# C-H-Chien/Trifocal_Pose_Estimation_using_Improved_GPUHC

Hardware: AMD Instinct MI355X
Metric: HC paths/sec (312 tracks x RANSAC samples) (higher is better)
Workload: dtype f32

## Files before the change

### trifocal_pose_estimation_using_improved_gpuhc_amd/_abi.py

```python
from __future__ import annotations

import ctypes as C
import os
from collections import namedtuple

import numpy as np

PKG_DIR = os.path.dirname(os.path.abspath(__file__))
LIB_PATH = os.environ.get("HC_TRIFOCAL_LIB") or os.path.join(PKG_DIR, "lib", "libhc_trifocal.so")

ABI_VERSION = 2

NUM_VARS, NUM_PARAMS, NUM_TRACKS = 30, 33, 312
NPP = NUM_PARAMS + 1
UNIFIED_INDEX_SIZE = 38880

HC_STATUS = {0: "HC_SUCCESS", 1: "HC_ERROR_INVALID_VALUE", 2: "HC_ERROR_WORKSPACE", 3: "HC_ERROR_LAUNCH",
             4: "HC_ERROR_DEVICE", 5: "HC_ERROR_TABLE"}


class HCError(RuntimeError):
    pass


# ... 138 lines not shown
                       "HC_THREEVIEW_NONE": HC_THREEVIEW_NONE, "HC_THREEVIEW_TOO_FEW": HC_THREEVIEW_TOO_FEW,
                       "HC_THREEVIEW_SINGULAR": HC_THREEVIEW_SINGULAR, "HC_THREEVIEW_SKIPPED": HC_THREEVIEW_SKIPPED}


class hcThreeViewReport(C.Structure):
    _fields_ = [("status", C.c_int32), ("iterations_run", C.c_int32), ("best_iteration", C.c_int32),
                ("transfer_history", C.c_int32 * (HC_REFINE_MAX_ITERATIONS + 1)),
                ("joint_history", C.c_int32 * (HC_REFINE_MAX_ITERATIONS + 1)),
                ("fit_set", C.c_int32), ("transfer_inliers", C.c_int32),
                ("scale_in", C.c_float), ("scale_out", C.c_float), ("pad", C.c_int32),
                ("rms_px_in", C.c_double * 2), ("rms_px_out", C.c_double * 2)]


class hcRefineThreeViewSettings(C.Structure):
    _fields_ = [("head", hcRefineSettings), ("scale_reports", C.c_void_p), ("reports", C.c_void_p),
                ("transfer_mask", C.c_void_p), ("iterations3", C.c_int32), ("pad", C.c_int32)]


THREEVIEW_REPORT_BYTES = C.sizeof(hcThreeViewReport)

HC_REFINE_STRUCTURE = 0x53543344
HC_STRUCTURE_ONLY = 1
HC_EDGEL3D_TANGENT, HC_EDGEL3D_ORIENTED = 1, 2
HC_STRUCTURE_NONE = 1
STRUCTURE_CONSTANTS = {"HC_REFINE_STRUCTURE": HC_REFINE_STRUCTURE, "HC_STRUCTURE_ONLY": HC_STRUCTURE_ONLY,
                       "HC_EDGEL3D_TANGENT": HC_EDGEL3D_TANGENT, "HC_EDGEL3D_ORIENTED": HC_EDGEL3D_ORIENTED,
                       "HC_STRUCTURE_NONE": HC_STRUCTURE_NONE}


class hcEdgel3D(C.Structure):
    _fields_ = [("X", C.c_float * 3), ("T", C.c_float * 3), ("err3_px", C.c_float), ("sin_plane", C.c_float),
                ("sin3", C.c_float), ("edgel", C.c_int32), ("flags", C.c_int32), ("pad", C.c_int32)]


class hcStructureReport(C.Structure):
    _fields_ = [("status", C.c_int32), ("count", C.c_int32), ("tangents", C.c_int32), ("oriented", C.c_int32),
                ("scale31", C.c_float), ("pad", C.c_int32 * 3)]


class hcRefineStructureSettings(C.Structure):
    _fields_ = [("tv", hcRefineThreeViewSettings), ("tangents", C.c_void_p), ("edgel_offsets", C.c_void_p),
                ("edgels3d", C.c_void_p), ("reports", C.c_void_p), ("min_sin_plane", C.c_float),
                ("max_sin3", C.c_float)]


EDGEL3D_BYTES = C.sizeof(hcEdgel3D)
STRUCTURE_REPORT_BYTES = C.sizeof(hcStructureReport)
EDGEL3D_DTYPE = np.dtype([("X", "<f4", (3,)), ("T", "<f4", (3,)), ("err3_px", "<f4"), ("sin_plane", "<f4"),
                          ("sin3", "<f4"), ("edgel", "<i4"), ("flags", "<i4"), ("pad", "<i4")])
assert EDGEL3D_DTYPE.itemsize == EDGEL3D_BYTES


Sig = namedtuple("Sig", "name restype argtypes optional", defaults=(False,))

_i, _u, _z, _p, _s, _ST = C.c_int, C.c_uint, C.c_size_t, C.c_void_p, C.c_char_p, C.c_int
_TA = C.POINTER(hcTrackArgs)
_GA = C.POINTER(hcGroupedAbortArgs)
_WS = (_p, _z, _p)
_SUPPORT = (_i, _p, _p, _i, _p, _p, _i, _p, _p, _p)

SIGNATURES = (
    Sig("hc_trifocal_workspace_size", _z, ()),
    Sig("hc_trifocal_workspace_size_for", _z, (_i,)),
    Sig("hc_trifocal_workspace_size_for_steps", _z, (_i, _i)),
    Sig("hc_trifocal_2op1p_30x30_track", _ST, (_TA, *_WS)),
    Sig("hc_trifocal_2op1p_30x30_track_abort", _ST, (_TA, C.POINTER(hcAbortArgs), *_WS)),
    Sig("hc_trifocal_2op1p_30x30_track_abort_grouped", _ST, (_TA, _GA, *_WS), True),
    Sig("hc_trifocal_2op1p_30x30_track_abort_gated", _ST, (_TA, _GA, C.POINTER(hcJointGate), *_WS), True),
    Sig("hc_shared_flag_create", _ST, (C.POINTER(_p), C.POINTER(hcIpcHandle)), True),
    Sig("hc_shared_flag_memory_kind", _i, (_p,), True),
    Sig("hc_shared_flag_open", _ST, (C.POINTER(hcIpcHandle), C.POINTER(_p)), True),
    Sig("hc_shared_flag_reset", _ST, (_p, _p), True),
    Sig("hc_shared_flag_close", _ST, (_p, _i), True),
    Sig("hc_trifocal_2op1p_30x30_track_ph_codeopt", _ST, (_TA, *_WS)),
    Sig("hc_trifocal_2op1p_30x30_track_ph", _ST, (_TA, *_WS)),
    Sig("hc_trifocal_workspace_status", _ST, (_p,)),
    Sig("hc_trifocal_read_timings", _ST, (_p, C.POINTER(C.c_double))),
    Sig("hc_trifocal_read_timestamps", _ST, (_p, C.POINTER(C.c_uint64), C.POINTER(C.c_uint64),
                                             C.POINTER(C.c_double))),
    Sig("hc_cgesv_30x30_batched", _ST, (_i, _p, _p, _p, _p)),
    Sig("hc_trifocal_eval_batched", _ST, (_i, _p, _p, _p, _p, _p, _p, _p, *_WS)),
    Sig("hc_last_error_string", _s, ()),
    Sig("hc_trifocal_version", _s, ()),
    Sig("hc_trifocal_abi_version", _i, ()),
    Sig("hc_trifocal_set_ring_test", None, (_i,)),
    Sig("hc_trifocal_set_small_launch", None, (_i,), True),
    Sig("hc_trifocal_set_retry_reuse", None, (_i,), True),
    Sig("hc_trifocal_ring_check_test", _ST, (_p, _z, _u, _u, _u, _p), True),
    Sig("hc_lu_struct_pattern", _u, (_i,), True),
    Sig("hc_lu_group_class", _i, (_i, _i), True),
    Sig("hc_lu_candidates", _u, (_i,), True),
    Sig("hc_lu_search_span", _i, (_i,), True),
    Sig("hc_trifocal_pose_support", _ST, _SUPPORT),
    Sig("hc_trifocal_pose_support_grouped", _ST, _SUPPORT, True),
    Sig("hc_pose_merge", None, (_i, _p, _p, _i, C.POINTER(hcPoseSelection))),
    Sig("hc_trifocal_pose_support_joint", _ST, _SUPPORT),
    Sig("hc_trifocal_pose_support_joint_grouped", _ST, _SUPPORT),
    Sig("hc_trifocal_pose_inlier_mask", _ST, (_p, _i, _p, _p, _p, _p)),
    Sig("hc_pose_merge_joint", None, (_i, _p, _p, C.POINTER(hcTrifocalSelection))),
    Sig("hc_pose_residuals", _i, (_p,) * 7),
    Sig("hc_read_start_sols", _i, (_s, _p)),
    Sig("hc_read_start_params", _i, (_s, _p)),
    Sig("hc_read_int_table", _i, (_s, _p, _i)),
    Sig("hc_read_float_table", _i, (_s, _p, _i)),
    Sig("hc_count_triplet_edgels", _i, (_s,)),
    Sig("hc_read_triplet_edgels", _i, (_s, _p, _p, _i)),
    Sig("hc_split_samples", None, (_i, _i, _p)),
    Sig("hc_prepare_target_params", None, (_u, _i, _p, _p, _p, _i, _p, _p, _p, _p)),
    Sig("hc_count_solutions", None, (_i, _p, _p, _p, _p)),
    Sig("hc_write_converged_sols", _i, (_s, _i, _p, _p)),
    Sig("hc_add_pixel_noise", None, (_i, _p, _p, C.c_double, C.c_uint64, _p)),
    Sig("hc_write_triplet_edgels", _i, (_s, _i, _p, _p)),
)
DECLARED_SYMBOLS = tuple(s.name for s in SIGNATURES)

P2C_SIGNATURES = (
    Sig("hc_trifocal_2op1p_30x30_track_p2c", _ST, (_TA, C.POINTER(hcP2cArgs), *_WS), True),
    Sig("hc_trifocal_p2c_eval_batched", _ST, (_i, _p, _p, _p, _p, _p, _p, _p, _p, _p, *_WS), True),
    Sig("hc_p2c_coefficients", _ST, (_i, _p, _p, _p, _p, _p), True),
)
P2C_DECLARED_SYMBOLS = tuple(s.name for s in P2C_SIGNATURES)

_RS = C.POINTER(hcRefineSettings)
REFINE_SIGNATURES = (
    Sig("hc_trifocal_pose_refine", _ST, (_p, _i, _p, _p, _RS, _p, _p, _p), True),
    Sig("hc_trifocal_pose_refine_grouped", _ST, (_i, _p, _p, _RS, _p, _p, _p), True),
)
REFINE_DECLARED_SYMBOLS = tuple(s.name for s in REFINE_SIGNATURES)

HC_TOPK_MAX = 32
TOPK_SIGNATURES = (
    Sig("hc_trifocal_pose_topk_joint", _ST, (_i, _p, _p, _i, _p, _p), True),
    Sig("hc_trifocal_pose_topk_joint_grouped", _ST, (_i, _p, _p, _i, _p, _i, _p, _p), True),
    Sig("hc_trifocal_pose_refine_topk", _ST, (_i, _p, _i, _p, _p, _RS, _p, _p, _p, _p, _p), True),
    Sig("hc_trifocal_pose_refine_topk_grouped", _ST, (_i, _p, _i, _p, _RS, _p, _p, _p, _p, _p), True),
    Sig("hc_pose_merge_topk", None, (_i, _i, _p, _p, _p), True),
)
TOPK_DECLARED_SYMBOLS = tuple(s.name for s in TOPK_SIGNATURES)

LU_SIGNATURES = (
    Sig("hc_lu_step_level", _i, (_i,), True),
    Sig("hc_cgesv_30x30_struct_batched", _ST, (_i, _p, _p, _p, _p), True),
    Sig("hc_cgesv_30x30_variant_batched", _ST, (_i, _i, _p, _p, _p, _p), True),
)
LU_VARIANTS = ("throughput", "throughput_twin", "abort", "abort_twin", "small", "small_twin", "archived",
               "archived_twin")
LU_DECLARED_SYMBOLS = tuple(s.name for s in LU_SIGNATURES)

LU_ROWTABLE_SIGNATURES = (
    Sig("hc_lu_row_field", _i, (_i, _i, _i), True),
)
LU_ROW_FIELDS = ("member", "bound", "window", "partner", "place", "chain")

EVAL_SIGNATURES = (
    Sig("hc_trifocal_eval_variant_batched", _ST, (_i, _u, _i, _p, _p, _p, _p, _p, _p, _p, _p, _p, _p, *_WS), True),
)
EVAL_VARIANTS = ("packed", "abs")
HC_EVAL_REDO = 1
EVAL_DECLARED_SYMBOLS = tuple(s.name for s in EVAL_SIGNATURES)

ADAPTIVE_SIGNATURES = (
    Sig("hc_ransac_need_table", _ST, (_i, C.c_double, _i, _i, _p), True),
)
ADAPTIVE_DECLARED_SYMBOLS = tuple(s.name for s in ADAPTIVE_SIGNATURES)

_lib = None


def lib() -> C.CDLL:
    global _lib
    if _lib is None:
        if not os.path.exists(LIB_PATH):
            raise HCError(f"native library missing: {LIB_PATH} (run `python -c 'import __graft_entry__ as g; g.build()'`)")
        import torch
        L = C.CDLL(LIB_PATH)
        for s in SIGNATURES + P2C_SIGNATURES + REFINE_SIGNATURES + TOPK_SIGNATURES + LU_SIGNATURES + \
                LU_ROWTABLE_SIGNATURES + EVAL_SIGNATURES + ADAPTIVE_SIGNATURES:
            fn = getattr(L, s.name, None)
            if fn is None:
                if s.optional:
                    continue
                raise HCError(f"{LIB_PATH} does not export {s.name}")
            fn.restype, fn.argtypes = s.restype, list(s.argtypes)
        if L.hc_trifocal_abi_version() != ABI_VERSION:
            raise HCError(f"{LIB_PATH}: ABI {L.hc_trifocal_abi_version()}, this binding expects {ABI_VERSION}")
        _lib = L
    return _lib


def check(status: int, what: str) -> None:
    if status != 0:
        detail = lib().hc_last_error_string().decode(errors="replace")
        raise HCError(f"{what} failed: {HC_STATUS.get(status, status)} ({detail})")


def call(name: str, *args) -> None:
    fn = getattr(lib(), name, None)
    if fn is None:
        raise HCError(f"{LIB_PATH} does not export {name}")
    check(fn(*args), name)


def ptr(x):
    if x is None:
        return C.c_void_p()
    if hasattr(x, "data_ptr"):
        return C.c_void_p(x.data_ptr())
    if hasattr(x, "cuda_stream"):
        return C.c_void_p(x.cuda_stream)
    return x.ctypes.data_as(C.c_void_p)


def _fatbin_digest(path: str) -> str | None:
    import hashlib
    import struct
    with open(path, "rb") as fh:
        elf = fh.read()
    if elf[:4] != b"\x7fELF" or elf[4] != 2:
        return None
    shoff, = struct.unpack_from("<Q", elf, 0x28)
    shentsize, shnum, shstrndx = struct.unpack_from("<HHH", elf, 0x3A)
    def sec(i):
        name, _typ, _flags, _addr, off, size = struct.unpack_from("<IIQQQQ", elf, shoff + i * shentsize)
        return name, off, size
    _, stroff, _ = sec(shstrndx)
    for i in range(shnum):
        name, off, size = sec(i)
        end = elf.index(b"\0", stroff + name)
        if elf[stroff + name:end] == b".hip_fatbin":
            return hashlib.sha256(elf[off:off + size]).hexdigest()
    return None


def build_id(path: str | None = None) -> str:
    import re
    path = path or LIB_PATH
    with open(path, "rb") as fh:
        m = re.search(rb"hc_trifocal gfx950 (v[0-9.]+)", fh.read())
    ver = m.group(1).decode() if m else "v?"
    d = _fatbin_digest(path)
    return f"{ver}+{d[:12] if d else 'nofatbin'}"


PRODUCT_LIB_PATH = os.path.join(PKG_DIR, "lib", "libhc_trifocal.so")
```

### trifocal_pose_estimation_using_improved_gpuhc_amd/csrc/hc_components.hpp

```cpp
#pragma once

#include "hc_layout.hpp"

namespace hc {


__global__ void __launch_bounds__(WG_THREADS) k_cgesv(int n, const cf *__restrict__ A, const cf *__restrict__ B,
                                                      cf *__restrict__ X) {
    __shared__ LUBuf s_lu[2 * WAVES_PER_WG];
    __shared__ __attribute__((aligned(16))) cf s_scr[2 * WAVES_PER_WG][LU_SCRATCH_CF];
    const int lane = lane_id();
    const int r = lane & 31;
    const int sys = (blockIdx.x * WAVES_PER_WG + threadIdx.x / WAVE) * 2 + (lane >> 5);
    const bool ok = sys < n && r < NV;
    cf rA[NV];
    uint32_t pat = 0;
#pragma unroll
    for (int c = 0; c < NV; c++) {
        rA[c] = ok ? A[((size_t)sys * NV + r) * NV + c] : cmk(0.0f, 0.0f);
        if (rA[c].x != 0.0f || rA[c].y != 0.0f) pat |= 1u << c;
    }
    const cf rB = ok ? B[(size_t)sys * NV + r] : cmk(0.0f, 0.0f);
    LUBuf &LB = s_lu[(threadIdx.x / WAVE) * 2 + (lane >> 5)];
    cf *scr = s_scr[(threadIdx.x / WAVE) * 2 + (lane >> 5)];
    bool redo;
    cf x = lu_solve<false>(rA, rB, lane, pat, LB, scr, redo, __ballot(sys < n));
    if (__builtin_expect(redo, 0)) {
#pragma unroll
        for (int c = 0; c < NV; c++) rA[c] = ok ? A[((size_t)sys * NV + r) * NV + c] : cmk(0.0f, 0.0f);
        x = lu_solve<true>(rA, rB, lane, pat, LB, scr, redo);
    }
    if (ok) X[(size_t)sys * NV + r] = x;
}

__global__ void __launch_bounds__(WG_THREADS) k_cgesv_struct_check(int n, const cf *__restrict__ A,
                                                                   unsigned *__restrict__ bad) {
    const size_t i = (size_t)blockIdx.x * WG_THREADS + threadIdx.x;
    if (i >= (size_t)n * NV) return;
    const uint32_t pat = LU_STRUCT_PAT[i % NV];
    bool out = false;
    for (int c = 0; c < NV; c++) {
        const cf a = A[i * NV + c];
        if (!((pat >> c) & 1u) && (a.x != 0.0f || a.y != 0.0f)) out = true;
    }
    if (out) *bad = 1u;
}
template <int LAT, bool STRUCT, bool ENTCHK, bool FUSE>
__global__ void __launch_bounds__(WG_THREADS) k_cgesv_variant(int n, const cf *__restrict__ A,
                                                              const cf *__restrict__ B, cf *__restrict__ X) {
    __shared__ LUBuf s_lu[2 * WAVES_PER_WG];
    __shared__ __attribute__((aligned(16))) cf s_scr[2 * WAVES_PER_WG][FUSE ? LU_SCRATCH_FUSED_CF : LU_SCRATCH_CF];
    if constexpr (FUSE) {
        lu_rowtab_fill(threadIdx.x);
        __syncthreads();
    }
    const int lane = lane_id();
    const int r = lane & 31;
    const int sys = (blockIdx.x * WAVES_PER_WG + threadIdx.x / WAVE) * 2 + (lane >> 5);
    const bool ok = sys < n && r < NV;
    cf rA[NV];
    uint32_t nz = 0;
    pf2 sq = {0.0f, 0.0f};
#pragma unroll
    for (int c = 0; c < NV; c++) {
        rA[c] = ok ? A[((size_t)sys * NV + r) * NV + c] : cmk(0.0f, 0.0f);
        if constexpr (!STRUCT) {
            if (rA[c].x != 0.0f || rA[c].y != 0.0f) nz |= 1u << c;
        }
        if constexpr (ENTCHK) {
            sq.x = __builtin_fmaf(rA[c].x, rA[c].x, sq.x);
            sq.y = __builtin_fmaf(rA[c].y, rA[c].y, sq.y);
        }
    }
    bool ent_bad = false;
    if constexpr (ENTCHK) ent_bad = __ballot(!(sq.x + sq.y < __builtin_inff())) != 0ull;
    const uint32_t pat = STRUCT ? (r < NV ? LU_STRUCT_PAT[r] : 0u) : nz;
    const cf rB = ok ? B[(size_t)sys * NV + r] : cmk(0.0f, 0.0f);
    LUBuf &LB = s_lu[(threadIdx.x / WAVE) * 2 + (lane >> 5)];
    cf *scr = s_scr[(threadIdx.x / WAVE) * 2 + (lane >> 5)];
    bool redo;
    cf x = lu_solve<false, LAT, STRUCT, ENTCHK, FUSE>(rA, rB, lane, pat, LB, scr, redo, __ballot(sys < n), ent_bad);
    if (__builtin_expect(redo, 0)) {
#pragma unroll
        for (int c = 0; c < NV; c++) rA[c] = ok ? A[((size_t)sys * NV + r) * NV + c] : cmk(0.0f, 0.0f);
        x = lu_solve<true>(rA, rB, lane, pat, LB, scr, redo);
    }
    if (ok) X[(size_t)sys * NV + r] = x;
}


__global__ void __launch_bounds__(WG_THREADS) k_eval(int n, const Workspace *ws, const cf *__restrict__ X,
                                                     const cf *__restrict__ P, const cf *__restrict__ D,
                                                     cf *__restrict__ HX, cf *__restrict__ HT, cf *__restrict__ H) {
    __shared__ uint32_t s_hx[HX_SLOT_CAP * 32];
    __shared__ uint2 s_ht[HT_TERMS * 32];
    __shared__ uint32_t s_hxd[HX_NSLOT / 2 * 32];
    __shared__ SlotLDS s_slot[2 * WAVES_PER_WG];
    const EvalTables *T = &ws->tab;
    if (ws->status != 0u) return;
    for (int i = threadIdx.x; i < HX_SLOT_CAP * 32; i += WG_THREADS) s_hx[i] = T->hx[i];
    for (int i = threadIdx.x; i < HT_TERMS * 32; i += WG_THREADS) s_ht[i] = T->ht[i];
    for (int i = threadIdx.x; i < HX_NSLOT / 2 * 32; i += WG_THREADS) s_hxd[i] = (&T->hxd[0][0])[i];
    {
        float *z = reinterpret_cast<float *>(s_slot);
        for (int i = threadIdx.x; i < (int)(sizeof(s_slot) / 4); i += WG_THREADS) z[i] = 0.0f;
    }
    __syncthreads();
    const int lane = lane_id();
    const int r = lane & 31;
    const int sys = (blockIdx.x * WAVES_PER_WG + threadIdx.x / WAVE) * 2 + (lane >> 5);
    SlotLDS &S = s_slot[(threadIdx.x / WAVE) * 2 + (lane >> 5)];
    const bool ok = sys < n;
    if (ok && r < 31) S.x[r] = X[(size_t)sys * 31 + r];
    if (ok) {
        S.ent[r] = P[(size_t)sys * NPP + r];
        S.ent[NPP + r] = D[(size_t)sys * NPP + r];
        if (r < NPP - 32) {
            S.ent[r + 32] = P[(size_t)sys * NPP + r + 32];
            S.ent[NPP + r + 32] = D[(size_t)sys * NPP + r + 32];
        }
    }
    __shared__ uint32_t s_gm[GM_WORDS][32];
    if (threadIdx.x < 32)
        for (int q = 0; q < GM_WORDS; q++) s_gm[q][threadIdx.x] = T->gm[q][threadIdx.x];
    __syncthreads();
    build_prefix_rounds(S, r, &T->pre[0][0]);
    cf rA[NV];
    eval_hx(rA, s_hx, s_hxd, &s_gm[0][0], S, r);
    const cf ht = eval_rhs<RHS_HT>(s_ht, S, r, true, rhs_masks(T));
    const cf h = eval_rhs<RHS_H>(s_ht, S, r, false, rhs_masks(T));
    if (ok && r < NV) {
#pragma unroll
        for (int c = 0; c < NV; c++) HX[((size_t)sys * NV + r) * NV + c] = rA[c];
        HT[(size_t)sys * NV + r] = ht;
        H[(size_t)sys * NV + r] = h;
    }
}

template <bool ABSTAB>
__global__ void __launch_bounds__(WG_THREADS) k_eval_variant(int n, int redo_vals, const Workspace *ws,
                                                             const cf *__restrict__ X, const cf *__restrict__ TGT,
                                                             const cf *__restrict__ DIF, const cf *__restrict__ SP,
                                                             const float *__restrict__ T0,
                                                             const uint8_t *__restrict__ KIND, cf *__restrict__ HX,
                                                             cf *__restrict__ RHS, uint8_t *__restrict__ ENT_OK) {
    __shared__ cf s_sp[NPP];
    __shared__ SlotLDS s_slot[2 * WAVES_PER_WG];
    const EvalTables *T = &ws->tab;
    if (ws->status != 0u) return;
    const uint2 *s_ht = T->ht;
    const uint32_t *s_hx = T->hx;
    const uint32_t *s_hxd = &T->hxd[0][0];
    if (threadIdx.x < NPP) s_sp[threadIdx.x] = SP[threadIdx.x];
    {
        float *z = reinterpret_cast<float *>(s_slot);
        for (int i = threadIdx.x; i < (int)(sizeof(s_slot) / 4); i += WG_THREADS) z[i] = 0.0f;
    }
    __syncthreads();
    const int lane = lane_id();
    const int r = lane & 31, hb = lane & 32;
    const int wid = threadIdx.x / WAVE;
    SlotLDS &S = s_slot[wid * 2 + (hb >> 5)];
    if (r == 30) S.x[30] = cmk(1.0f, 0.0f);
    __shared__ uint32_t s_rowc[GM_WORDS + 1][32];
    if (threadIdx.x < 32) {
        for (int q = 0; q < GM_WORDS; q++) s_rowc[q][threadIdx.x] = T->gm[q][threadIdx.x];
        s_rowc[GM_WORDS][threadIdx.x] = T->pat[threadIdx.x];
    }
    __syncthreads();
    const bool rl = r < NV;
    wave_lds_sync();
    const AbsTables *AT = &ws->abs;
    const int wv = ABSTAB ? __builtin_amdgcn_readfirstlane(wid) : 0;
    char *const l0 = reinterpret_cast<char *>(s_slot);

    const int pt = (blockIdx.x * WAVES_PER_WG + wid) * 2 + (hb >> 5);
    const size_t pi = (size_t)(pt < n ? pt : n - 1);
    const unsigned kd = KIND[pi];
    const bool act = pt < n && kd < 2u;
    const bool pred = act && kd == 0u;
    if (act && rl) S.x[r] = X[pi * (NV + 1) + r];
    build_prefixes(S, r, &T->pre[0][0], TGT + pi * NPP, DIF + pi * NPP, s_sp, T0[pi]);
    wave_lds_sync();
    const int lane_v = lane_fresh();
    const int r_v = lane_v & 31;
    const uint32_t l16 = (uint32_t)lane_v << 4;
    cf rB = cmk(0.0f, 0.0f);
    {
        const bool any_p = __ballot(pred) != 0ull, any_c = __ballot(act && !pred) != 0ull;
        const RhsMasks mk = rhs_masks(T);
        if (any_p && any_c) {
            if constexpr (ABSTAB) rB = eval_rhs_abs<RHS_MIXED>(AT->ht[wv], AT->htq[wv], l0, l16, pred, mk);
            else rB = eval_rhs<RHS_MIXED>(s_ht, S, r_v, pred, mk);
        } else if (any_p) {
            const cf t = ABSTAB ? eval_rhs_abs<RHS_HT>(AT->ht[wv], AT->htq[wv], l0, l16, true, mk)
                                : eval_rhs<RHS_HT>(s_ht, S, r_v, true, mk);
            if (pred) rB = t;
        } else if (any_c) {
            const cf t = ABSTAB ? eval_rhs_abs<RHS_H>(AT->ht[wv], AT->htq[wv], l0, l16, false, mk)
                                : eval_rhs<RHS_H>(s_ht, S, r_v, false, mk);
            if (!pred) rB = t;
        }
    }
    cf rA[NV];
    if constexpr (ABSTAB) {
        uint4 gmv[ABS_GM_Q];
        const bool ent_ok = eval_hx_terms_abs(AT->hx[wv], l0, l16, AT->gm[wv], gmv);
        if (act) ENT_OK[pi * 32 + r] = ent_ok ? 1 : 0;
        wave_lds_sync();
        gather_hx_abs(rA, l0, gmv);
    } else {
        eval_hx(rA, s_hx, s_hxd, &s_rowc[0][0], S, r_v);
    }
    wave_lds_sync();
    if (redo_vals) {
        for (int k = r; k < ENT_CAP - 1; k += 32) S.ent[k] = cmk(__builtin_nanf(""), __builtin_nanf(""));
        wave_lds_sync();
        const bool act_r = act, pred_r = pred;
        const int l_r = lane_fresh(), r_r = l_r & 31;
        const uint32_t l16_r = (uint32_t)l_r << 4;
        cf rb = cmk(0.0f, 0.0f);
        if (__ballot(pred_r) != 0ull) {
            const cf t = ABSTAB ? eval_rhs_abs<RHS_HT>(AT->ht[wv], AT->htq[wv], l0, l16_r, true, rhs_masks(T))
                                : eval_rhs<RHS_HT>(s_ht, S, r_r, true, rhs_masks(T));
            if (pred_r) rb = t;
        }
        if (__ballot(act_r && !pred_r) != 0ull) {
            const cf t = ABSTAB ? eval_rhs_abs<RHS_H>(AT->ht[wv], AT->htq[wv], l0, l16_r, false, rhs_masks(T))
                                : eval_rhs<RHS_H>(s_ht, S, r_r, false, rhs_masks(T));
            if (!pred_r) rb = t;
        }
        if constexpr (ABSTAB) {
            uint4 gmv[ABS_GM_Q];
            eval_hx_terms_abs(AT->hx[wv], l0, l16_r, AT->gm[wv], gmv);
            wave_lds_sync();
            gather_hx_abs(rA, l0, gmv);
        } else {
            eval_hx_terms(s_hx, s_hxd, reinterpret_cast<char *>(&S), r_r);
            wave_lds_sync();
            gather_hx(rA, &s_rowc[0][0], S, r_r);
        }
        wave_lds_sync();
        rB = rb;
    }
    if (act && rl) {
#pragma unroll
        for (int c = 0; c < NV; c++) HX[(pi * NV + r) * NV + c] = rA[c];
        RHS[pi * NV + r] = rB;
    }
}

}
```

### trifocal_pose_estimation_using_improved_gpuhc_amd/csrc/hc_eval.hpp

```cpp
#pragma once

#include <stddef.h>

#include "hc_slot.hpp"

namespace hc {

typedef float pf2 __attribute__((ext_vector_type(2)));

constexpr int HX_GCAP[6] = {8, 5, 3, 3, 1, 1};
constexpr int HX_SLOT_CAP = 21;
constexpr int HX_NSLOT = 6;
__host__ __device__ constexpr int hx_gend(int s) { return s < 0 ? 0 : hx_gend(s - 1) + HX_GCAP[s]; }
__host__ __device__ constexpr bool hx_is_gend(int k) {
    return k + 1 == hx_gend(0) || k + 1 == hx_gend(1) || k + 1 == hx_gend(2) || k + 1 == hx_gend(3) ||
           k + 1 == hx_gend(4) || k + 1 == hx_gend(5);
}
__host__ __device__ constexpr int hx_gslot(int k) {
    return k < hx_gend(0) ? 0 : k < hx_gend(1) ? 1 : k < hx_gend(2) ? 2 : k < hx_gend(3) ? 3 : k < hx_gend(4) ? 4 : 5;
}
static_assert(hx_gend(5) == HX_SLOT_CAP, "slot capacities");
constexpr int SLOT_OFF_X = (int)offsetof(SlotLDS, x);
constexpr int SLOT_OFF_ENT = (int)offsetof(SlotLDS, ent);
constexpr int SLOT_OFF_ENTZERO = SLOT_OFF_ENT + 8 * (ENT_CAP - 1);
constexpr int SLOT_OFF_STG = SLOT_OFF_ENT;
constexpr int SLOT_STG_DIF_DELTA = 8 * NPP;
constexpr int SLOT_OFF_TP = (int)offsetof(SlotLDS, tp);
constexpr int SLOT_OFF_QP = (int)offsetof(SlotLDS, qp);
constexpr int SLOT_OFF_HXDUMMY = (int)offsetof(SlotLDS, lu) + 8 * 31;
static_assert(SLOT_OFF_QP + 8 * QP_CAP < 65536 && SLOT_OFF_HXDUMMY < 65536, "slot offsets must fit 16 bits");
static_assert(SLOT_OFF_X + 8 * 31 < 256, "x offsets must fit a byte");
static_assert(2 * NPP <= ENT_CAP - 1, "the staging area lies below the structural zero");

constexpr int GM_WORDS = NV / 2;
constexpr int PRE_TP_ROUNDS = (TP_CAP + 31) / 32, PRE_ROUNDS = PRE_TP_ROUNDS + (QP_CAP + 31) / 32;
__device__ __forceinline__ float coef_b2(uint32_t w) {
    float co;
    asm("v_cvt_f32_i32_sdwa %0, sext(%1) dst_sel:DWORD dst_unused:UNUSED_PAD src0_sel:BYTE_2" : "=v"(co) : "v"(w));
    return co;
}
__device__ __forceinline__ float coef_ht(const uint2 &w) { return (float)((int)w.y >> 24); }
struct EvalTables {
    int hx_len;
    int status;
    unsigned magic;
    unsigned lu_struct;
    unsigned long long src_hash;
    unsigned long long pad2;
    uint32_t gm[GM_WORDS][32];
    uint32_t pat[32];
    uint32_t hxd[HX_NSLOT / 2][32];
    uint32_t ht_acc_mask[4];
    uint32_t ht_light_mask[4];
    uint2 pre[PRE_ROUNDS][32];
    uint32_t hx[HX_SLOT_CAP * 32];
    uint2 ht[HT_TERMS * 32];
};

__device__ __forceinline__ pf2 ldp(const char *base, uint32_t off) {
    return *reinterpret_cast<const pf2 *>(base + off);
}
__device__ __forceinline__ pf2 pcmul(pf2 a, pf2 b) {
    pf2 t, r;
    asm("v_pk_mul_f32 %0, %1, %2 op_sel:[1,1] op_sel_hi:[1,0] neg_lo:[1,0]" : "=v"(t) : "v"(a), "v"(b));
    asm("v_pk_fma_f32 %0, %1, %2, %3 op_sel_hi:[0,1,1]" : "=v"(r) : "v"(a), "v"(b), "v"(t));
    return r;
}
__device__ __forceinline__ pf2 pcmadd(pf2 acc, pf2 a, pf2 b) {
    pf2 s, r;
    asm("v_pk_fma_f32 %0, %1, %2, %3 op_sel_hi:[0,1,1]" : "=v"(s) : "v"(a), "v"(b), "v"(acc));
    asm("v_pk_fma_f32 %0, %1, %2, %3 op_sel:[1,1,0] op_sel_hi:[1,0,1] neg_lo:[1,0,0]" : "=v"(r) : "v"(a), "v"(b), "v"(s));
    return r;
}
__device__ __forceinline__ pf2 pcmsub(pf2 acc, pf2 a, pf2 b) {
    pf2 s, r;
    asm("v_pk_fma_f32 %0, %1, %2, %3 op_sel_hi:[0,1,1] neg_lo:[1,0,0] neg_hi:[1,0,0]" : "=v"(s) : "v"(a), "v"(b), "v"(acc));
    asm("v_pk_fma_f32 %0, %1, %2, %3 op_sel:[1,1,0] op_sel_hi:[1,0,1] neg_hi:[1,0,0]" : "=v"(r) : "v"(a), "v"(b), "v"(s));
    return r;
}

#ifndef HC_EV_AHEAD
#define HC_EV_AHEAD 2
#endif
constexpr int EV_AHEAD = HC_EV_AHEAD;
constexpr int EV_WAHEAD = EV_AHEAD + 2;

struct HxOps { pf2 t, xu, xv; };
__device__ __forceinline__ HxOps hx_ops(const char *sb, uint32_t w) {
    return HxOps{ldp(sb, w & 0xFFFFu), ldp(sb, (w >> 16) & 0xFFu), ldp(sb, w >> 24)};
}

__device__ __forceinline__ void eval_hx_terms(const uint32_t *s_hx, const uint32_t *s_hxd, char *sb, int r) {
    uint32_t w[HX_SLOT_CAP];
    uint32_t dst[HX_NSLOT / 2];
#pragma unroll
    for (int q = 0; q < HX_NSLOT / 2; q++) dst[q] = s_hxd[q * 32 + r];
#pragma unroll
    for (int k = 0; k < EV_WAHEAD; k++) w[k] = s_hx[k * 32 + r];
    HxOps o[EV_AHEAD + 1];
#pragma unroll
    for (int k = 0; k < EV_AHEAD; k++) o[k] = hx_ops(sb, w[k]);
    pf2 acc = {0.0f, 0.0f};
#pragma unroll
    for (int k = 0; k < HX_SLOT_CAP; k++) {
        if (k + EV_WAHEAD < HX_SLOT_CAP) w[k + EV_WAHEAD] = s_hx[(k + EV_WAHEAD) * 32 + r];
        if (k + EV_AHEAD < HX_SLOT_CAP) o[(k + EV_AHEAD) % (EV_AHEAD + 1)] = hx_ops(sb, w[k + EV_AHEAD]);
        const HxOps &q = o[k % (EV_AHEAD + 1)];
        const pf2 P = pcmul(q.t, q.xu);
        acc = pcmadd(acc, P, q.xv);
        if (hx_is_gend(k)) {
            const int sl = hx_gslot(k);
            const uint32_t off = (sl & 1) ? (dst[sl >> 1] >> 16) : (dst[sl >> 1] & 0xFFFFu);
            *reinterpret_cast<pf2 *>(sb + off) = acc;
            acc = pf2{0.0f, 0.0f};
        }
        __builtin_amdgcn_sched_barrier(0);
    }
}

__device__ __forceinline__ void gather_hx(cf (&rA)[NV], const uint32_t *gmw, const SlotLDS &S, int r) {
    const char *sb = reinterpret_cast<const char *>(&S);
    uint32_t g[GM_WORDS];
#pragma unroll
    for (int q = 0; q < GM_WORDS; q++) g[q] = gmw[q * 32 + r];
#pragma unroll
    for (int c = 0; c < NV; c++) {
        const pf2 v = ldp(sb, (c & 1) ? (g[c / 2] >> 16) : (g[c / 2] & 0xFFFFu));
        rA[c] = cmk(v.x, v.y);
    }
}

__device__ __forceinline__ void eval_hx(cf (&rA)[NV], const uint32_t *s_hx, const uint32_t *s_hxd,
                                        const uint32_t *gmw, SlotLDS &S, int r) {
    eval_hx_terms(s_hx, s_hxd, reinterpret_cast<char *>(&S), r);
    wave_lds_sync();
    HC_ISA_MARK("ev_gather");
    gather_hx(rA, gmw, S, r);
}

__device__ __forceinline__ void build_prefix_rounds(SlotLDS &S, int r, const uint2 *pre) {
    char *sb = reinterpret_cast<char *>(&S);
    wave_lds_sync();
#pragma unroll
    for (int k = 0; k < PRE_TP_ROUNDS; k++) {
        const uint2 w = pre[k * 32 + r];
        const pf2 pa = ldp(sb, w.x & 0xFFFFu), pb = ldp(sb, w.x >> 16);
        const float co = coef_b2(w.y);
        const pf2 t = pcmul(pa * pf2{co, co}, pb);
        *reinterpret_cast<pf2 *>(sb + (w.y & 0xFFFFu)) = t;
    }
#pragma unroll
    for (int k = PRE_TP_ROUNDS; k < PRE_ROUNDS; k++) {
        const uint2 w = pre[k * 32 + r];
        const uint32_t oa = w.x & 0xFFFFu, ob = w.x >> 16;
        const pf2 pa = ldp(sb, oa), pb = ldp(sb, ob);
        const pf2 da = ldp(sb + SLOT_STG_DIF_DELTA, oa), db = ldp(sb + SLOT_STG_DIF_DELTA, ob);
        const pf2 q = pcmadd(pcmul(da, pb), db, pa);
// ... 6 lines not shown
    cf *stg = S.ent;
    const float omt = (float)(1.0 - (double)t0);
    stg[r] = cadd(cscale(target[r], t0), cscale(sp[r], omt));
    stg[NPP + r] = diff[r];
    if (r == 0) {
        stg[32] = cadd(cscale(target[32], t0), cscale(sp[32], omt));
        stg[33] = cmk(1.0f, 0.0f);
        stg[NPP + 32] = diff[32];
        stg[NPP + 33] = diff[33];
    }
    build_prefix_rounds(S, r, pre);
}

constexpr int P2C_NK = 38;
constexpr int SLOT_STG_P2C_HT_DELTA = 8 * P2C_NK;
static_assert(2 * P2C_NK <= ENT_CAP - 1, "the P2C staging area lies below the structural zero");
__device__ __forceinline__ void p2c_stage(SlotLDS &S, int r, const cf *chx, const cf *cht, float t) {
    cf *stg = S.ent;
#pragma unroll
    for (int q = 0; q < 2; q++) {
        const int k = r + 32 * q;
        if (k < P2C_NK) {
            stg[k] = cadd(cadd(chx[3 * k], cscale(chx[3 * k + 1], t)), cscale(cscale(chx[3 * k + 2], t), t));
            stg[P2C_NK + k] = cadd(cht[2 * k], cscale(cht[2 * k + 1], t));
        }
    }
}
__device__ __forceinline__ void build_prefix_rounds_p2c(SlotLDS &S, int r, const uint2 *pre) {
    char *sb = reinterpret_cast<char *>(&S);
    wave_lds_sync();
#pragma unroll
    for (int k = 0; k < PRE_TP_ROUNDS; k++) {
        const uint2 w = pre[k * 32 + r];
        const pf2 c = ldp(sb, w.x & 0xFFFFu);
        const float co = coef_b2(w.y);
        *reinterpret_cast<pf2 *>(sb + (w.y & 0xFFFFu)) = c * pf2{co, co};
    }
#pragma unroll
    for (int k = PRE_TP_ROUNDS; k < PRE_ROUNDS; k++) {
        const uint2 w = pre[k * 32 + r];
        *reinterpret_cast<pf2 *>(sb + (w.y & 0xFFFFu)) = ldp(sb + SLOT_STG_P2C_HT_DELTA, w.x & 0xFFFFu);
    }
    wave_lds_sync();
}
__device__ __forceinline__ void build_prefixes_p2c(SlotLDS &S, int r, const uint2 *pre, const cf *chx, const cf *cht,
                                                   float t0) {
    p2c_stage(S, r, chx, cht, t0);
    build_prefix_rounds_p2c(S, r, pre);
}

enum : int { RHS_HT = 0, RHS_H = 1, RHS_MIXED = 2 };
constexpr int HT_FULL = 13, HT_HELP = HT_TERMS - HT_FULL;
constexpr int HT_HELP_FIRST = HT_FULL - HT_HELP;

template <bool SUB>
__device__ __forceinline__ pf2 pcmacc_masked(pf2 acc, pf2 a, pf2 b, unsigned long long m) {
    pf2 t;
    unsigned long long sv;
    if constexpr (SUB)
        asm("s_mov_b64 %2, exec\n\ts_mov_b64 exec, %3\n\t"
            "v_pk_fma_f32 %1, %4, %5, %0 op_sel_hi:[0,1,1] neg_lo:[1,0,0] neg_hi:[1,0,0]\n\t"
            "s_nop 0\n\t"
            "v_pk_fma_f32 %0, %4, %5, %1 op_sel:[1,1,0] op_sel_hi:[1,0,1] neg_hi:[1,0,0]\n\t"
            "s_mov_b64 exec, %2"
            : "+v"(acc), "=&v"(t), "=&s"(sv) : "s"(m), "v"(a), "v"(b));
    else
        asm("s_mov_b64 %2, exec\n\ts_mov_b64 exec, %3\n\t"
            "v_pk_fma_f32 %1, %4, %5, %0 op_sel_hi:[0,1,1]\n\t"
            "s_nop 0\n\t"
            "v_pk_fma_f32 %0, %4, %5, %1 op_sel:[1,1,0] op_sel_hi:[1,0,1] neg_lo:[1,0,0]\n\t"
            "s_mov_b64 exec, %2"
            : "+v"(acc), "=&v"(t), "=&s"(sv) : "s"(m), "v"(a), "v"(b));
    return acc;
}
__device__ __forceinline__ pf2 from_partner(pf2 v) {
    asm("v_permlane16_swap_b32 %0, %0\n\tv_permlane16_swap_b32 %1, %1" : "+v"(v.x), "+v"(v.y));
    return v;
}
struct RhsMasks { unsigned long long acc[HT_HELP], light[HT_HELP]; };

__device__ __forceinline__ RhsMasks rhs_masks(const EvalTables *T) {
    RhsMasks m;
#pragma unroll
    for (int q = 0; q < HT_HELP; q++) {
        const unsigned long long a = (uint32_t)__builtin_amdgcn_readfirstlane((int)T->ht_acc_mask[q]),
                                 l = (uint32_t)__builtin_amdgcn_readfirstlane((int)T->ht_light_mask[q]);
        m.acc[q] = a | (a << 32);
        m.light[q] = l | (l << 32);
    }
    return m;
}

template <int KIND>
struct RhsOps { pf2 t, q, xu, xv, xw; };
template <int KIND>
__device__ __forceinline__ RhsOps<KIND> rhs_ops(const char *sb, const uint2 &w) {
    RhsOps<KIND> o;
    if constexpr (KIND != RHS_HT) o.t = ldp(sb, w.x & 0xFFFFu);
    if constexpr (KIND != RHS_H) o.q = ldp(sb, w.x >> 16);
    o.xu = ldp(sb, w.y & 0xFFu);
    o.xv = ldp(sb, (w.y >> 8) & 0xFFu);
    o.xw = ldp(sb, (w.y >> 16) & 0xFFu);
    return o;
}

template <int KIND>
__device__ __forceinline__ cf eval_rhs(const uint2 *s_ht, const SlotLDS &S, int r, bool ht_half, const RhsMasks &mk) {
    const char *sb = reinterpret_cast<const char *>(&S);
    constexpr bool SUB = KIND == RHS_HT;
    uint2 w[HT_TERMS];
#pragma unroll
    for (int j = 0; j < EV_WAHEAD; j++) w[j] = s_ht[j * 32 + r];
    RhsOps<KIND> o[EV_AHEAD + 1];
#pragma unroll
    for (int j = 0; j < EV_AHEAD; j++) o[j] = rhs_ops<KIND>(sb, w[j]);
    pf2 acc = {0.0f, 0.0f};
    pf2 hp[HT_HELP];
#pragma unroll
    for (int j = 0; j < HT_FULL; j++) {
        if (j + EV_WAHEAD < HT_TERMS) w[j + EV_WAHEAD] = s_ht[(j + EV_WAHEAD) * 32 + r];
        if (j + EV_AHEAD < HT_FULL) o[(j + EV_AHEAD) % (EV_AHEAD + 1)] = rhs_ops<KIND>(sb, w[j + EV_AHEAD]);
        const RhsOps<KIND> &q = o[j % (EV_AHEAD + 1)];
        const float co = coef_ht(w[j]);
        pf2 P;
        if constexpr (KIND == RHS_HT) {
            const pf2 s = q.q * pf2{co, co};
            P = pcmul(pcmul(s, q.xu), q.xv);
        } else if constexpr (KIND == RHS_H) {
            P = pcmul(pcmul(q.t, q.xu), q.xv);
        } else {
            const pf2 s = q.q * pf2{-co, -co};
            const pf2 pre = {ht_half ? s.x : q.t.x, ht_half ? s.y : q.t.y};
            P = pcmul(pcmul(pre, q.xu), q.xv);
        }
        if (j < HT_HELP_FIRST) {
            acc = SUB ? pcmsub(acc, P, q.xw) : pcmadd(acc, P, q.xw);
        } else {
            hp[j - HT_HELP_FIRST] = P;
            acc = pcmacc_masked<SUB>(acc, P, q.xw, mk.acc[j - HT_HELP_FIRST]);
        }
        __builtin_amdgcn_sched_barrier(0);
    }
#pragma unroll
    for (int q = 0; q < HT_HELP; q++) {
        const pf2 P = from_partner(hp[q]);
        const pf2 xw = ldp(sb, (w[HT_FULL + q].y >> 16) & 0xFFu);
        acc = pcmacc_masked<SUB>(acc, P, xw, mk.light[q]);
    }
    return cmk(acc.x, acc.y);
}

constexpr int ABS_WAVES = 4;
constexpr int ABS_GM_Q = (NV + 3) / 4;
static_assert(HT_HELP <= 3, "the light terms' x[w] share one word group");
struct AbsTables {
    uint4 hx[ABS_WAVES][HX_SLOT_CAP][WAVE];
    uint4 ht[ABS_WAVES][HT_FULL + 1][WAVE];
    uint2 htq[ABS_WAVES][HT_FULL][WAVE];
    uint4 gm[ABS_WAVES][ABS_GM_Q][WAVE];
};
static_assert(2 * ABS_WAVES * sizeof(SlotLDS) < 65536, "absolute offsets stay in the DS offset range");
constexpr int EV_TAHEAD = 6;
static_assert(EV_TAHEAD > EV_AHEAD, "the words come before the operands they address");

template <typename W>
__device__ __forceinline__ W abs_ld(const W *row, uint32_t lane_off) {
    return *reinterpret_cast<const W *>(reinterpret_cast<const char *>(row) + (size_t)lane_off);
}

__device__ __forceinline__ HxOps hx_ops_abs(const char *l0, const uint4 &w) {
    return HxOps{ldp(l0, w.x), ldp(l0, w.y), ldp(l0, w.z)};
}
__device__ __forceinline__ bool eval_hx_terms_abs(const uint4 (*hxw)[WAVE], char *l0, uint32_t l16,
                                                  const uint4 (*gmw)[WAVE], uint4 (&g)[ABS_GM_Q]) {
    uint4 w[HX_SLOT_CAP];
#pragma unroll
    for (int k = 0; k < EV_TAHEAD; k++) w[k] = abs_ld(hxw[k], l16);
    HxOps o[EV_AHEAD + 1];
#pragma unroll
    for (int k = 0; k < EV_AHEAD; k++) o[k] = hx_ops_abs(l0, w[k]);
    pf2 acc = {0.0f, 0.0f}, sq = {0.0f, 0.0f};
#pragma unroll
    for (int k = 0; k < HX_SLOT_CAP; k++) {
        if (k + EV_TAHEAD < HX_SLOT_CAP) w[k + EV_TAHEAD] = abs_ld(hxw[k + EV_TAHEAD], l16);
        if (k == HX_SLOT_CAP - EV_TAHEAD) {
#pragma unroll
            for (int q = 0; q < ABS_GM_Q; q++) g[q] = abs_ld(gmw[q], l16);
        }
        if (k + EV_AHEAD < HX_SLOT_CAP) o[(k + EV_AHEAD) % (EV_AHEAD + 1)] = hx_ops_abs(l0, w[k + EV_AHEAD]);
        const HxOps &q = o[k % (EV_AHEAD + 1)];
        const pf2 P = pcmul(q.t, q.xu);
        acc = pcmadd(acc, P, q.xv);
        if (hx_is_gend(k)) {
            *reinterpret_cast<pf2 *>(l0 + w[k].w) = acc;
            asm("v_pk_fma_f32 %0, %1, %1, %0" : "+v"(sq) : "v"(acc));
            acc = pf2{0.0f, 0.0f};
        }
        __builtin_amdgcn_sched_barrier(0);
    }
    return sq.x + sq.y < __builtin_inff();
}

__device__ __forceinline__ void gather_hx_abs(cf (&rA)[NV], const char *l0, const uint4 (&g)[ABS_GM_Q]) {
#pragma unroll
    for (int c = 0; c < NV; c++) {
        const uint4 &gw = g[c / 4];
        const pf2 v = ldp(l0, c % 4 == 0 ? gw.x : c % 4 == 1 ? gw.y : c % 4 == 2 ? gw.z : gw.w);
        rA[c] = cmk(v.x, v.y);
    }
}

template <int KIND>
__device__ __forceinline__ RhsOps<KIND> rhs_ops_abs(const char *l0, const uint4 &w, const uint2 &wq) {
    RhsOps<KIND> o;
    if constexpr (KIND != RHS_HT) o.t = ldp(l0, w.w);
    if constexpr (KIND != RHS_H) o.q = ldp(l0, wq.x);
    o.xu = ldp(l0, w.x);
    o.xv = ldp(l0, w.y);
    o.xw = ldp(l0, w.z);
    return o;
}

template <int KIND>
__device__ __forceinline__ cf eval_rhs_abs(const uint4 (*htw)[WAVE], const uint2 (*htqw)[WAVE], const char *l0,
                                           uint32_t l16, bool ht_half, const RhsMasks &mk) {
    constexpr bool SUB = KIND == RHS_HT;
    constexpr bool Q = KIND != RHS_H;
    const uint32_t l8 = l16 >> 1;
    uint4 w[HT_FULL + 1];
    uint2 wq[HT_FULL];
#pragma unroll
    for (int j = 0; j < EV_TAHEAD; j++) {
        w[j] = abs_ld(htw[j], l16);
        if constexpr (Q) wq[j] = abs_ld(htqw[j], l8);
    }
    RhsOps<KIND> o[EV_AHEAD + 1];
#pragma unroll
    for (int j = 0; j < EV_AHEAD; j++) o[j] = rhs_ops_abs<KIND>(l0, w[j], wq[j]);
    pf2 acc = {0.0f, 0.0f};
    pf2 hp[HT_HELP];
#pragma unroll
    for (int j = 0; j < HT_FULL; j++) {
        if (j + EV_TAHEAD < HT_FULL + 1) w[j + EV_TAHEAD] = abs_ld(htw[j + EV_TAHEAD], l16);
        if constexpr (Q)
            if (j + EV_TAHEAD < HT_FULL) wq[j + EV_TAHEAD] = abs_ld(htqw[j + EV_TAHEAD], l8);
        if (j + EV_AHEAD < HT_FULL)
            o[(j + EV_AHEAD) % (EV_AHEAD + 1)] = rhs_ops_abs<KIND>(l0, w[j + EV_AHEAD], wq[j + EV_AHEAD]);
        const RhsOps<KIND> &q = o[j % (EV_AHEAD + 1)];
        pf2 P;
        if constexpr (KIND == RHS_HT) {
            const float co = __uint_as_float(wq[j].y);
            const pf2 s = q.q * pf2{co, co};
            P = pcmul(pcmul(s, q.xu), q.xv);
        } else if constexpr (KIND == RHS_H) {
            P = pcmul(pcmul(q.t, q.xu), q.xv);
        } else {
            const float co = __uint_as_float(wq[j].y);
            const pf2 s = q.q * pf2{-co, -co};
            const pf2 pre = {ht_half ? s.x : q.t.x, ht_half ? s.y : q.t.y};
            P = pcmul(pcmul(pre, q.xu), q.xv);
        }
        if (j < HT_HELP_FIRST) {
            acc = SUB ? pcmsub(acc, P, q.xw) : pcmadd(acc, P, q.xw);
        } else {
            hp[j - HT_HELP_FIRST] = P;
            acc = pcmacc_masked<SUB>(acc, P, q.xw, mk.acc[j - HT_HELP_FIRST]);
        }
        __builtin_amdgcn_sched_barrier(0);
    }
#pragma unroll
    for (int q = 0; q < HT_HELP; q++) {
        const pf2 P = from_partner(hp[q]);
        const uint4 &lw = w[HT_FULL];
        const pf2 xw = ldp(l0, q == 0 ? lw.x : q == 1 ? lw.y : lw.z);
        acc = pcmacc_masked<SUB>(acc, P, xw, mk.light[q]);
    }
    return cmk(acc.x, acc.y);
}

}
```

### trifocal_pose_estimation_using_improved_gpuhc_amd/csrc/hc_kernels.hip

```cpp
#include "hc_layout.hpp"
#include "hc_prep.hpp"
#include "hc_components.hpp"
#include "hc_ring.hpp"
#include "hc_score.hpp"
#include "hc_track.hpp"
#include "hc_p2c.hpp"
#include "../../include/hc_trifocal_testing.h"
#include "../../include/p2c/hc_trifocal_p2c.h"
#include "../../include/lu/hc_lu_testing.h"
#include "../../include/lu/hc_lu_rowtable_testing.h"
#include "../../include/eval/hc_eval_testing.h"
#include "../../include/adaptive/hc_trifocal_adaptive.h"

#include <atomic>
#include <climits>
#include <cstdlib>
#include <cstring>
#include <map>
#include <mutex>
#include <utility>

namespace hc {

thread_local hipError_t g_last_hip_error = hipSuccess;
static inline hcStatus launch_status(hcStatus on_fail) {
    const hipError_t e = hipGetLastError();
    if (e != hipSuccess) { g_last_hip_error = e; return on_fail; }
    return HC_SUCCESS;
}

static size_t ws_bytes_needed() { return (sizeof(Workspace) + 255) & ~(size_t)255; }
struct SliceLayout {
    size_t rq, ring, susp;
    size_t total;
    unsigned long long ring_cap;
    size_t susp_entry0, susp_entry1;
};
static SliceLayout slice_layout(long long paths, int max_steps) {
    if (paths < 0) paths = 0;
    if (max_steps < 0) max_steps = 0;
    SliceLayout a;
    a.ring_cap = ring_entries(paths, max_steps);
    const size_t ring_bytes = ((size_t)a.ring_cap * sizeof(unsigned long long) + 255) & ~(size_t)255;
    a.rq = ws_bytes_needed();
    a.ring = a.rq + RQ_WORDS * sizeof(unsigned);
    a.susp = a.ring + ring_bytes;
    a.total = a.susp + (size_t)paths * SUSP_WORDS * sizeof(unsigned long long);
    a.susp_entry0 = ring_bytes / 8;
    a.susp_entry1 = a.susp_entry0 + (size_t)paths * SUSP_WORDS;
    return a;
}
static bool sliced_launch(bool abort_mode, const hcTrackSettings &st, const SliceLayout &a, size_t wsb) {
    return !abort_mode && SLICE_Q > 0 && wsb >= a.total && a.ring_cap < 0xFFFFFF00ull &&
           a.susp_entry1 < (size_t)UINT_MAX && slice_fits(st.max_steps, st.max_corrections, st.delta_t_inc_steps);
}
static std::atomic<int> g_ring_test{0};
static std::atomic<int> g_small_launch{0};
static std::atomic<int> g_retry_reuse{1};

static int grid_for(int waves_needed, const void *kernel) {
    static std::mutex mu;
    static std::map<std::pair<int, const void *>, std::pair<int, int>> cache;
    int dev = 0;
    if (hipGetDevice(&dev) != hipSuccess) return -1;
    int cus = 0, per_cu = 0;
    {
        std::lock_guard<std::mutex> g(mu);
        auto it = cache.find({dev, kernel});
        if (it == cache.end()) {
            if (hipDeviceGetAttribute(&cus, hipDeviceAttributeMultiprocessorCount, dev) != hipSuccess) return -1;
            if (hipOccupancyMaxActiveBlocksPerMultiprocessor(&per_cu, kernel, WG_THREADS, 0) != hipSuccess) per_cu = 1;
            if (per_cu < 1) per_cu = 1;
            it = cache.emplace(std::make_pair(dev, kernel), std::make_pair(cus, per_cu)).first;
        }
        cus = it->second.first;
        per_cu = it->second.second;
    }
    const int want = waves_needed / WAVES_PER_WG + (waves_needed % WAVES_PER_WG != 0);
    const int cap = cus * per_cu;
    return want < cap ? want : cap;
}
static int resident_wgs(const void *kernel) { return grid_for(INT_MAX, kernel); }

enum class TrackMode { GatedAbort, GroupedAbort, Abort, Ph, PhCodeopt, Track, P2c };
struct TrackLaunch {
    TrackMode mode;
    const hcAbortArgs *ab = nullptr;
    const hcGroupedAbortArgs *gr = nullptr;
    const hcJointGate *jg = nullptr;
    const hcP2cArgs *p2c = nullptr;
};

struct TrackKernels { const void *lus, *any; };
static TrackKernels track_kernels(TrackMode mode, bool small, bool adaptive = false) {
    static const void *const by_mode[2][6] = {
        {(const void *)k_track_gated<true>, (const void *)k_track_grouped<true>,
         (const void *)k_track<true, HC_ABORT_MINW, true>, (const void *)k_track<false, 5, true, true>,
         (const void *)k_track<false, 5, true, true>, (const void *)k_track<false, 5, true>},
        {(const void *)k_track_gated<false>, (const void *)k_track_grouped<false>,
         (const void *)k_track<true, HC_ABORT_MINW, true, false, false>,
         (const void *)k_track<false, 5, true, true, false>, (const void *)k_track<false, 5, true, true, false>,
         (const void *)k_track<false, 5, true, false, false>}};
    if (small) return {(const void *)k_track_small<true>, (const void *)k_track_small<false>};
    if (mode == TrackMode::P2c) return {(const void *)k_track_p2c<true>, (const void *)k_track_p2c<false>};
    if (mode == TrackMode::GatedAbort && adaptive)
        return {(const void *)k_track_adaptive<true>, (const void *)k_track_adaptive<false>};
    return {by_mode[0][(int)mode], by_mode[1][(int)mode]};
}

static bool small_launch(TrackMode mode, long long paths) {
    const int small_mode = g_small_launch.load(std::memory_order_relaxed);
    if (mode != TrackMode::Track || small_mode < 0) return false;
    const long long slots = 2ll * WAVES_PER_WG * resident_wgs(track_kernels(mode, false).lus);
    const long long small_slots = 2ll * WAVES_PER_WG * resident_wgs(track_kernels(mode, true).lus);
    return small_mode > 0 || (slots > 0 && 2 * paths <= slots && paths <= small_slots);
}

static hcStatus enqueue_track(const void *kern, int grid, KArgs &k, hipStream_t s) {
    void *kargs[] = {&k};
    g_last_hip_error = hipLaunchKernel(kern, dim3(grid), dim3(WG_THREADS), kargs, 0, s);
    if (g_last_hip_error != hipSuccess) return HC_ERROR_LAUNCH;
    return launch_status(HC_ERROR_LAUNCH);
}

static hcStatus launch_track(const hcTrackArgs *t, const TrackLaunch &l, void *workspace, size_t wsb,
                             hcStream stream) {
    const bool gated = l.mode == TrackMode::GatedAbort;
    const bool grouped = gated || l.mode == TrackMode::GroupedAbort;
    const bool abort_mode = grouped || l.mode == TrackMode::Abort;
    const hcAbortArgs *ab = l.mode == TrackMode::Abort ? l.ab : nullptr;
    const hcGroupedAbortArgs *gr = grouped ? l.gr : nullptr;
    const hcP2cArgs *pc = l.mode == TrackMode::P2c ? l.p2c : nullptr;
    const hcAdaptiveGate *ag =
        gated && l.jg->pad == (int32_t)HC_GATE_ADAPTIVE ? reinterpret_cast<const hcAdaptiveGate *>(l.jg) : nullptr;
    if (!t || t->sub_ransac_iters < 0) return HC_ERROR_INVALID_VALUE;
    if (grouped && (gr->num_groups < 1 || !gr->groups || !gr->sample_group || !gr->group_found ||
                    !gr->trifocal_sols_batch_index))
        return HC_ERROR_INVALID_VALUE;
    if (ag && (!ag->need || !ag->need_offset || !ag->sample_ordinal || !ag->group_limit)) return HC_ERROR_INVALID_VALUE;
    if (!workspace || wsb < ws_bytes_needed()) return HC_ERROR_WORKSPACE;
    if (t->sub_ransac_iters == 0) return HC_SUCCESS;
    if ((!t->start_sols && !t->start_sols_array) || (!t->tracks && !t->track_array) || !t->converge || !t->infinity)
        return HC_ERROR_INVALID_VALUE;
    if (!pc && (!t->start_params || !t->target_params || !t->diff_params || !t->unified_index))
        return HC_ERROR_INVALID_VALUE;
    if (t->settings.max_steps < 0 || t->settings.max_corrections < 0 || t->settings.delta_t_inc_steps < 0)
        return HC_ERROR_INVALID_VALUE;
    if (l.mode == TrackMode::Abort && (!ab || ab->num_triplet_edgels <= 0 || !ab->triplet_edge_locations ||
                                       !ab->intrinsic_matrix || !ab->found_trifocal_sols ||
                                       !ab->trifocal_sols_batch_index))
        return HC_ERROR_INVALID_VALUE;
    const long long paths = (long long)t->sub_ransac_iters * NTRK;
    if (paths > 0x7FFFFFFFll) return HC_ERROR_INVALID_VALUE;
    hipStream_t s = (hipStream_t)stream;
    Workspace *ws = (Workspace *)workspace;
    (void)hipGetLastError();
    KArgs k{};
    k.num_paths = (int)paths;
    k.ordered = abort_mode ? 0 : 1;
    k.truncate = (l.mode == TrackMode::PhCodeopt || l.mode == TrackMode::Ph || pc) ? 0 : 1;
    k.explicit_rk = (l.mode == TrackMode::Ph || pc) ? 1 : 0;
    k.max_steps = t->settings.max_steps;
    k.max_corr = t->settings.max_corrections;
// ... 124 lines not shown
int hc_diag_phases(unsigned long long *out, int reset) { return hc::diag_read(hc::g_diag_phase, out, reset); }
#endif
#ifdef HC_DIAG_LUWORK
int hc_diag_luwork(unsigned long long *out, int reset) { return hc::diag_read(hc::g_diag_luwork, out, reset); }
#endif
#ifdef HC_DIAG_LIVE
int hc_diag_live(unsigned long long *out, int reset) { return hc::diag_read(hc::g_diag_live, out, reset); }
#endif
#ifdef HC_DIAG_TIMES
int hc_diag_span(unsigned long long *out, int reset) {
    static const unsigned long long init[4] = {~0ull, 0ull, 0ull, 0ull};
    return hc::diag_read(hc::g_diag_span, out, reset, &init);
}
#endif
#ifdef HC_DIAG_UTIL
int hc_diag_util(unsigned long long *out, int reset) { return hc::diag_read(hc::g_diag_util, out, reset); }
#endif

size_t hc_trifocal_workspace_size(void) { return hc::ws_bytes_needed(); }

size_t hc_trifocal_workspace_size_for(int sub_ransac_iters) {
    return hc_trifocal_workspace_size_for_steps(sub_ransac_iters, 80);
}

size_t hc_trifocal_workspace_size_for_steps(int sub_ransac_iters, int max_steps) {
    return hc::slice_layout(sub_ransac_iters > 0 ? (long long)sub_ransac_iters * hc::NTRK : 0, max_steps).total;
}

hcStatus hc_trifocal_2op1p_30x30_track(const hcTrackArgs *args, void *workspace, size_t workspace_bytes,
                                       hcStream stream) {
    return hc::launch_track(args, {hc::TrackMode::Track}, workspace, workspace_bytes, stream);
}

hcStatus hc_trifocal_2op1p_30x30_track_abort(const hcTrackArgs *args, const hcAbortArgs *abort_args,
                                             void *workspace, size_t workspace_bytes, hcStream stream) {
    return hc::launch_track(args, {hc::TrackMode::Abort, abort_args}, workspace, workspace_bytes, stream);
}

hcStatus hc_trifocal_2op1p_30x30_track_abort_grouped(const hcTrackArgs *args, const hcGroupedAbortArgs *g,
                                                     void *workspace, size_t workspace_bytes, hcStream stream) {
    if (!g) return HC_ERROR_INVALID_VALUE;
    return hc::launch_track(args, {hc::TrackMode::GroupedAbort, nullptr, g}, workspace, workspace_bytes, stream);
}

hcStatus hc_trifocal_2op1p_30x30_track_abort_gated(const hcTrackArgs *args, const hcGroupedAbortArgs *g,
                                                   const hcJointGate *gate, void *workspace,
                                                   size_t workspace_bytes, hcStream stream) {
    if (!g || !gate) return HC_ERROR_INVALID_VALUE;
    if (!(gate->min_joint_ratio > 0.0f) || gate->min_joint_ratio > 3.402823466e+38f) return HC_ERROR_INVALID_VALUE;
    return hc::launch_track(args, {hc::TrackMode::GatedAbort, nullptr, g, gate}, workspace, workspace_bytes, stream);
}

hcStatus hc_trifocal_2op1p_30x30_track_ph_codeopt(const hcTrackArgs *args, void *workspace, size_t workspace_bytes,
                                                  hcStream stream) {
    return hc::launch_track(args, {hc::TrackMode::PhCodeopt}, workspace, workspace_bytes, stream);
}

hcStatus hc_trifocal_2op1p_30x30_track_ph(const hcTrackArgs *args, void *workspace, size_t workspace_bytes,
                                          hcStream stream) {
    return hc::launch_track(args, {hc::TrackMode::Ph}, workspace, workspace_bytes, stream);
}

hcStatus hc_trifocal_2op1p_30x30_track_p2c(const hcTrackArgs *args, const hcP2cArgs *p2c, void *workspace,
                                           size_t workspace_bytes, hcStream stream) {
    if (!p2c || !p2c->hx_index || !p2c->ht_index || !p2c->coeffs_hx || !p2c->coeffs_ht) return HC_ERROR_INVALID_VALUE;
    hc::TrackLaunch l{hc::TrackMode::P2c};
    l.p2c = p2c;
    return hc::launch_track(args, l, workspace, workspace_bytes, stream);
}

hcStatus hc_trifocal_workspace_status(const void *workspace) {
    if (!workspace) return HC_ERROR_INVALID_VALUE;
    hc::Workspace h;
    const hcStatus st = hc::read_control(workspace, h);
    if (st != HC_SUCCESS) return st;
    if (h.status == 0u) return HC_SUCCESS;
    return h.status == (unsigned)HC_ERROR_TABLE ? HC_ERROR_TABLE : HC_ERROR_DEVICE;
}

hcStatus hc_trifocal_read_timings(const void *workspace, double *first_found_seconds) {
    if (!workspace || !first_found_seconds) return HC_ERROR_INVALID_VALUE;
    hc::Workspace h;
    const hcStatus st = hc::read_control(workspace, h);
    if (st != HC_SUCCESS) return st;
    *first_found_seconds = (h.t_found && h.t_start) ? (double)(long long)(h.t_found - h.t_start) / hc::wall_clock_hz() : -1.0;
    return HC_SUCCESS;
}

hcStatus hc_trifocal_read_timestamps(const void *workspace, uint64_t *start_ticks, uint64_t *found_ticks,
                                     double *tick_hz) {
    if (!workspace || !start_ticks || !found_ticks || !tick_hz) return HC_ERROR_INVALID_VALUE;
    hc::Workspace h;
    const hcStatus st = hc::read_control(workspace, h);
    if (st != HC_SUCCESS) return st;
    *start_ticks = h.t_start;
    *found_ticks = h.t_found;
    *tick_hz = hc::wall_clock_hz();
    return HC_SUCCESS;
}

hcStatus hc_cgesv_30x30_batched(int n, const hcComplex *A, const hcComplex *b, hcComplex *x, hcStream stream) {
    if (n < 0 || (n > 0 && (!A || !b || !x))) return HC_ERROR_INVALID_VALUE;
    if (n == 0) return HC_SUCCESS;
    (void)hipGetLastError();
    const int per = 2 * hc::WAVES_PER_WG;
    hipLaunchKernelGGL(hc::k_cgesv, dim3((n + per - 1) / per), dim3(hc::WG_THREADS), 0, (hipStream_t)stream, n,
                       (const hc::cf *)A, (const hc::cf *)b, (hc::cf *)x);
    return hc::launch_status(HC_ERROR_LAUNCH);
}

hcStatus hc_cgesv_30x30_variant_batched(int variant, int n, const hcComplex *A, const hcComplex *b, hcComplex *x,
                                        hcStream stream) {
    if (variant < 0 || variant >= HC_LU_VARIANT_COUNT) return HC_ERROR_INVALID_VALUE;
    if (n < 0 || (n > 0 && (!A || !b || !x))) return HC_ERROR_INVALID_VALUE;
    if (n == 0) return HC_SUCCESS;
    hipStream_t s = (hipStream_t)stream;
    (void)hipGetLastError();
    switch (variant) {
    case HC_LU_VARIANT_THROUGHPUT:      return hc::launch_cgesv_variant<false, false, 0, true>(n, A, b, x, s);
    case HC_LU_VARIANT_THROUGHPUT_TWIN: return hc::launch_cgesv_variant<false, false, 0, false>(n, A, b, x, s);
    case HC_LU_VARIANT_ABORT:           return hc::launch_cgesv_variant<true, false, HC_LU_LATB_COLS, true>(n, A, b, x, s);
    case HC_LU_VARIANT_ABORT_TWIN:      return hc::launch_cgesv_variant<true, false, HC_LU_LATB_COLS, false>(n, A, b, x, s);
    case HC_LU_VARIANT_SMALL:           return hc::launch_cgesv_variant<false, false, HC_SMALL_LAT, true>(n, A, b, x, s);
    case HC_LU_VARIANT_SMALL_TWIN:      return hc::launch_cgesv_variant<false, false, HC_SMALL_LAT, false>(n, A, b, x, s);
    case HC_LU_VARIANT_ARCHIVED:        return hc::launch_cgesv_variant<false, true, 0, true>(n, A, b, x, s);
    case HC_LU_VARIANT_ARCHIVED_TWIN:   return hc::launch_cgesv_variant<false, true, 0, false>(n, A, b, x, s);
    }
    return HC_ERROR_INVALID_VALUE;
}

hcStatus hc_cgesv_30x30_struct_batched(int n, const hcComplex *A, const hcComplex *b, hcComplex *x, hcStream stream) {
    return hc_cgesv_30x30_variant_batched(HC_LU_VARIANT_THROUGHPUT, n, A, b, x, stream);
}

hcStatus hc_trifocal_eval_batched(int n, const int32_t *unified_index, const hcComplex *x, const hcComplex *p,
                                  const hcComplex *d, hcComplex *Hx, hcComplex *Ht, hcComplex *H, void *workspace,
                                  size_t workspace_bytes, hcStream stream) {
    if (n < 0 || !unified_index || (n > 0 && (!x || !p || !d || !Hx || !Ht || !H))) return HC_ERROR_INVALID_VALUE;
    if (!workspace || workspace_bytes < hc::ws_bytes_needed()) return HC_ERROR_WORKSPACE;
    if (n == 0) return HC_SUCCESS;
    hipStream_t s = (hipStream_t)stream;
    hc::Workspace *ws = (hc::Workspace *)workspace;
    (void)hipGetLastError();
    hc::PrepArgs pa{unified_index, ws, nullptr, nullptr, nullptr, nullptr, 0u, 0u, 0u};
    hipLaunchKernelGGL(hc::k_prep_tables, dim3(1), dim3(hc::PREP_THREADS), 0, s, pa);
    if (hc::launch_status(HC_ERROR_LAUNCH) != HC_SUCCESS) return HC_ERROR_LAUNCH;
    const int per = 2 * hc::WAVES_PER_WG;
    hipLaunchKernelGGL(hc::k_eval, dim3((n + per - 1) / per), dim3(hc::WG_THREADS), 0, s, n, ws,
                       (const hc::cf *)x, (const hc::cf *)p, (const hc::cf *)d, (hc::cf *)Hx, (hc::cf *)Ht,
                       (hc::cf *)H);
    return hc::launch_status(HC_ERROR_LAUNCH);
}

hcStatus hc_trifocal_eval_variant_batched(int variant, unsigned flags, int n, const int32_t *unified_index,
                                          const hcComplex *x, const hcComplex *target, const hcComplex *diff,
                                          const hcComplex *start_params, const float *t, const uint8_t *kind,
                                          hcComplex *Hx, hcComplex *rhs, uint8_t *ent_ok, void *workspace,
                                          size_t workspace_bytes, hcStream stream) {
    if (variant < 0 || variant >= HC_EVAL_VARIANT_COUNT || (flags & ~HC_EVAL_REDO) != 0u) return HC_ERROR_INVALID_VALUE;
    const bool abs_tables = variant == HC_EVAL_VARIANT_ABS;
    if (n < 0 || (n > 0 && (!unified_index || !x || !target || !diff || !start_params || !t || !kind || !Hx || !rhs ||
                            (abs_tables && !ent_ok))))
        return HC_ERROR_INVALID_VALUE;
    if (!workspace || workspace_bytes < hc::ws_bytes_needed()) return HC_ERROR_WORKSPACE;
    if (n == 0) return HC_SUCCESS;
    hipStream_t s = (hipStream_t)stream;
    hc::Workspace *ws = (hc::Workspace *)workspace;
    (void)hipGetLastError();
    hc::PrepArgs pa{unified_index, ws, nullptr, nullptr, nullptr, nullptr, 0u, 0u, 0u};
    hipLaunchKernelGGL(hc::k_prep_tables, dim3(1), dim3(hc::PREP_THREADS), 0, s, pa);
    if (hc::launch_status(HC_ERROR_LAUNCH) != HC_SUCCESS) return HC_ERROR_LAUNCH;
    const int per = 2 * hc::WAVES_PER_WG;
    const dim3 grid((n + per - 1) / per), block(hc::WG_THREADS);
    const int redo = (flags & HC_EVAL_REDO) ? 1 : 0;
    if (abs_tables)
        hipLaunchKernelGGL(hc::k_eval_variant<true>, grid, block, 0, s, n, redo, ws, (const hc::cf *)x,
                           (const hc::cf *)target, (const hc::cf *)diff, (const hc::cf *)start_params, t, kind,
                           (hc::cf *)Hx, (hc::cf *)rhs, ent_ok);
    else
        hipLaunchKernelGGL(hc::k_eval_variant<false>, grid, block, 0, s, n, redo, ws, (const hc::cf *)x,
                           (const hc::cf *)target, (const hc::cf *)diff, (const hc::cf *)start_params, t, kind,
                           (hc::cf *)Hx, (hc::cf *)rhs, ent_ok);
    if (hc::launch_status(HC_ERROR_LAUNCH) != HC_SUCCESS) return HC_ERROR_LAUNCH;
    unsigned ctl[16];
    hipError_t e = hipMemcpyAsync(ctl, workspace, sizeof(ctl), hipMemcpyDeviceToHost, s);
    if (e == hipSuccess) e = hipStreamSynchronize(s);
    if (e != hipSuccess) {
        hc::g_last_hip_error = e;
        return HC_ERROR_DEVICE;
    }
    const unsigned status = ctl[offsetof(hc::Workspace, status) / sizeof(unsigned)];
    if (status == 0u) return HC_SUCCESS;
    return status == (unsigned)HC_ERROR_TABLE ? HC_ERROR_TABLE : HC_ERROR_DEVICE;
}

hcStatus hc_trifocal_p2c_eval_batched(int n, const int32_t *hx_index, const int32_t *ht_index, const hcComplex *x,
                                      const hcComplex *coeffs_hx, const hcComplex *coeffs_ht, const float *t,
                                      hcComplex *Hx, hcComplex *Ht, hcComplex *H, void *workspace,
                                      size_t workspace_bytes, hcStream stream) {
    if (n < 0 || !hx_index || !ht_index || (n > 0 && (!x || !coeffs_hx || !coeffs_ht || !t || !Hx || !Ht || !H)))
        return HC_ERROR_INVALID_VALUE;
    if (!workspace || workspace_bytes < hc::ws_bytes_needed()) return HC_ERROR_WORKSPACE;
    if (n == 0) return HC_SUCCESS;
    hipStream_t s = (hipStream_t)stream;
    hc::Workspace *ws = (hc::Workspace *)workspace;
    (void)hipGetLastError();
    hc::PrepArgs pa{hx_index, ws, nullptr, nullptr, nullptr, nullptr, 0u, 0u, 0u};
    hipLaunchKernelGGL(hc::k_prep_tables_p2c<true>, dim3(1), dim3(hc::PREP_THREADS), 0, s, pa, ht_index);
    if (hc::launch_status(HC_ERROR_LAUNCH) != HC_SUCCESS) return HC_ERROR_LAUNCH;
    const int per = 2 * hc::WAVES_PER_WG;
    hipLaunchKernelGGL(hc::k_eval_p2c<true>, dim3((n + per - 1) / per), dim3(hc::WG_THREADS), 0, s, n, ws,
                       (const hc::cf *)x, (const hc::cf *)coeffs_hx, (const hc::cf *)coeffs_ht, t, (hc::cf *)Hx,
                       (hc::cf *)Ht, (hc::cf *)H);
    return hc::launch_status(HC_ERROR_LAUNCH);
}

const char *hc_last_error_string(void) { return hipGetErrorString(hc::g_last_hip_error); }

static_assert(sizeof(hcIpcHandle) == sizeof(hipIpcMemHandle_t), "hcIpcHandle mirrors hipIpcMemHandle_t");

namespace hc {
static std::mutex g_flag_mu;
static std::map<const void *, int> g_flag_kind;
}

hcStatus hc_shared_flag_create(uint32_t **flag, hcIpcHandle *handle) {
    if (!flag || !handle) return HC_ERROR_INVALID_VALUE;
    static const unsigned kinds[3] = {hipDeviceMallocUncached, hipDeviceMallocFinegrained, hipDeviceMallocDefault};
    hipError_t last = hipSuccess;
    for (int k = 0; k < 3; k++) {
        void *p = nullptr;
        last = (kinds[k] == hipDeviceMallocDefault) ? hipMalloc(&p, 256) : hipExtMallocWithFlags(&p, 256, kinds[k]);
        if (last != hipSuccess) { (void)hipGetLastError(); continue; }
        hipIpcMemHandle_t h;
        if ((last = hipMemset(p, 0, 256)) != hipSuccess || (last = hipDeviceSynchronize()) != hipSuccess ||
            (last = hipIpcGetMemHandle(&h, p)) != hipSuccess) {
            (void)hipGetLastError();
            (void)hipFree(p);
            continue;
        }
        memcpy(handle, &h, sizeof(h));
        *flag = (uint32_t *)p;
        std::lock_guard<std::mutex> g(hc::g_flag_mu);
        hc::g_flag_kind[p] = 2 - k;
        return HC_SUCCESS;
    }
    hc::g_last_hip_error = last;
    return HC_ERROR_DEVICE;
}

int hc_shared_flag_memory_kind(const uint32_t *flag) {
    std::lock_guard<std::mutex> g(hc::g_flag_mu);
    const auto it = hc::g_flag_kind.find(flag);
    return it == hc::g_flag_kind.end() ? -1 : it->second;
}

hcStatus hc_shared_flag_open(const hcIpcHandle *handle, uint32_t **flag) {
    if (!flag || !handle) return HC_ERROR_INVALID_VALUE;
    hipIpcMemHandle_t h;
    memcpy(&h, handle, sizeof(h));
    void *p = nullptr;
    if ((hc::g_last_hip_error = hipIpcOpenMemHandle(&p, h, hipIpcMemLazyEnablePeerAccess)) != hipSuccess)
        return HC_ERROR_DEVICE;
    *flag = (uint32_t *)p;
    return HC_SUCCESS;
}

hcStatus hc_shared_flag_reset(uint32_t *flag, hcStream stream) {
    if (!flag) return HC_ERROR_INVALID_VALUE;
    if ((hc::g_last_hip_error = hipMemsetAsync(flag, 0, sizeof(uint32_t), (hipStream_t)stream)) != hipSuccess)
        return HC_ERROR_LAUNCH;
    return HC_SUCCESS;
}

hcStatus hc_shared_flag_close(uint32_t *flag, int opened) {
    if (!flag) return HC_ERROR_INVALID_VALUE;
    if (!opened) {
        std::lock_guard<std::mutex> g(hc::g_flag_mu);
        hc::g_flag_kind.erase(flag);
    }
    hc::g_last_hip_error = opened ? hipIpcCloseMemHandle(flag) : hipFree(flag);
    return hc::g_last_hip_error == hipSuccess ? HC_SUCCESS : HC_ERROR_DEVICE;
}

int hc_trifocal_abi_version(void) { return HC_TRIFOCAL_ABI_VERSION; }

unsigned hc_lu_struct_pattern(int row) { return row >= 0 && row < hc::NV ? hc::LU_STRUCT_PAT[row] : 0u; }
unsigned hc_lu_candidates(int step) { return step >= 0 && step < hc::NV ? hc::LU_BOUND.cand[step] : 0u; }
int hc_lu_search_span(int step) { return step >= 0 && step < hc::NV ? hc::lu_search_span(step) : -1; }
int hc_lu_step_level(int step) { return step >= 0 && step < hc::NV ? hc::LU_LEVELS.level[step] : -1; }
int hc_lu_group_class(int step, int group) {
    if (step < 0 || step >= hc::NV - 1 || group < 0 || group >= hc::LuChunks::count(step)) return -1;
    return hc::lu_group_class(step, group);
}
int hc_lu_row_field(int level, int row, int field) {
    if (level < 0 || level >= hc::LU_REC_LEVELS || row < 0 || row >= hc::LU_REC_ROWS) return -2;
    hc::LuRowRec rec{0u, hc::LU_ROWTAB.w[level * hc::LU_REC_ROWS + row]};
    rec.bound = hc::LU_ROWTAB.w[hc::LU_REC_BOUND0 + ((rec.word >> hc::LU_REC_MEMBER_AT) & 31u)];
    const int mem = (int)((rec.word >> hc::LU_REC_MEMBER_AT) & 31u), k = (int)((rec.word >> hc::LU_REC_CHAIN_AT) & 15u);
    switch (field) {
    case HC_LU_ROW_MEMBER: return mem == hc::LU_REC_NO_MEMBER ? -1 : mem;
    case HC_LU_ROW_BOUND: return (int)rec.bound;
    case HC_LU_ROW_WINDOW: return (int)(rec.word & ((1u << hc::LU_REC_WIN_BITS) - 1u)) / 8 + 2 * row;
    case HC_LU_ROW_PARTNER: return (int)((rec.word >> hc::LU_REC_PARTNER_AT) & 31u);
    case HC_LU_ROW_PLACE: return (rec.word & hc::LU_REC_FIRST) ? 0 : (rec.word & hc::LU_REC_UP) ? 1 : 2;
    case HC_LU_ROW_CHAIN: return k == hc::LU_REC_NO_CHAIN ? -1 : k;
    default: return -2;
    }
}

hcStatus hc_trifocal_ring_check_test(void *workspace, size_t workspace_bytes, unsigned head, unsigned tail,
                                     unsigned avail, hcStream stream) {
    const hc::SliceLayout area = hc::slice_layout(0, 0);
    if (!workspace || workspace_bytes < area.ring) return HC_ERROR_WORKSPACE;
    hipStream_t s = (hipStream_t)stream;
    unsigned *rq = (unsigned *)((char *)workspace + area.rq);
    const unsigned v[3] = {head, tail, avail};
    const int at[3] = {hc::RQ_HEAD, hc::RQ_TAIL, hc::RQ_AVAIL};
    (void)hipGetLastError();
    for (int i = 0; i < 3; i++)
        if ((hc::g_last_hip_error = hipMemcpyAsync(rq + at[i], &v[i], sizeof(unsigned), hipMemcpyHostToDevice, s)) !=
            hipSuccess)
            return HC_ERROR_LAUNCH;
    if ((hc::g_last_hip_error = hipStreamSynchronize(s)) != hipSuccess) return HC_ERROR_DEVICE;
    hipLaunchKernelGGL(hc::k_ring_check, dim3(1), dim3(64), 0, s, (hc::Workspace *)workspace, (const unsigned *)rq);
    return hc::launch_status(HC_ERROR_LAUNCH);
}

void hc_trifocal_set_ring_test(int delay_ticks) {
    hc::g_ring_test.store(delay_ticks > 0 ? (delay_ticks < HC_RING_TEST_MIN_TICKS ? HC_RING_TEST_MIN_TICKS : delay_ticks)
                                          : 0,
                          std::memory_order_relaxed);
}

void hc_trifocal_set_small_launch(int mode) {
    hc::g_small_launch.store(mode < 0 ? -1 : mode > 0 ? 1 : 0, std::memory_order_relaxed);
}

void hc_trifocal_set_retry_reuse(int on) { hc::g_retry_reuse.store(on ? 1 : 0, std::memory_order_relaxed); }

const char *hc_trifocal_version(void) {
    return "hc_trifocal gfx950 v10.12 (2 paths/wave, structurally sparse LDS-broadcast LU with lean pivot steps fused by level, the levels' per-row constants and row labels read from LDS tables, "
           "one exec region per pivot step for the eligible rows with the column groups through scratch windows, "
           "column groups by structural class (never-fillable groups untested, always-live groups unconditional), "
           "pivot search narrowed to the candidate rows' DPP group "
           "(abort kernel and tracking launches filling at most half of the path slots -- the latter at 3 waves/SIMD, "
           "16 columns per batch: batched latency mode, one LDS round trip per pivot step, every live-able column "
           "group untested), "
           "structure-agnostic twin kernels for other dH/dx structures, readlane back substitution (the throughput "
           "kernel's fused positions level by level through LDS), pipelined evals over "
           "per-slot prefix tables, 5 waves/SIMD, time slicing at step boundaries with least-attained-service "
           "issue priority, a rejected step's retry reuses its first RK4 slope, the throughput kernel's operand "
           "addresses read complete from per-slot tables and its finiteness check made on the dH/dx entries)";
}

}
```

### trifocal_pose_estimation_using_improved_gpuhc_amd/csrc/hc_lu.hpp

```cpp
#pragma once

#include "hc_eval.hpp"
#include "hc_lu_struct.hpp"
#include "hc_lu_diag.hpp"

namespace hc {

typedef float f4v __attribute__((ext_vector_type(4)));

struct alignas(16) LUBuf {
    cf row[32];
};
static_assert(sizeof(LUBuf) == sizeof(SlotLDS::lu), "LUBuf is SlotLDS::lu");
static_assert(offsetof(SlotLDS, lu) % 16 == 0, "SlotLDS::lu must be 16-B aligned");

__device__ __forceinline__ float rcp_rn(float s) {
    const float r0 = __builtin_amdgcn_rcpf(s);
    const float e0 = __builtin_fmaf(-s, r0, 1.0f);
    return __builtin_fmaf(e0, r0, r0);
}
__device__ __forceinline__ bool rcp_fast_bits(int bits) {
    return (uint32_t)(bits - 0x12800000) < (uint32_t)(0x7B800000 - 0x12800000);
}

__device__ __forceinline__ void st4(cf *p, cf a, cf b) {
    f4v v = {a.x, a.y, b.x, b.y};
    *reinterpret_cast<f4v *>(p) = v;
}
__device__ __forceinline__ void ld4(const cf *p, cf &a, cf &b) {
    const f4v v = *reinterpret_cast<const f4v *>(p);
    a = cmk(v.x, v.y);
    b = cmk(v.z, v.w);
}

__device__ __forceinline__ int half_max_int_p16(int v) {
    v = max(v, dpp_i<DPP_QP_1032>(v));
    v = max(v, dpp_i<DPP_QP_2301>(v));
    v = max(v, dpp_i<DPP_ROW_HALF_MIRROR>(v));
    v = max(v, dpp_i<DPP_ROW_MIRROR>(v));
    const auto sw = __builtin_amdgcn_permlane16_swap((unsigned)v, (unsigned)v, false, false);
    return max((int)sw[0], (int)sw[1]);
}

template <uint32_t C>
__device__ __forceinline__ unsigned long long and_halves(unsigned long long x) {
    uint32_t lo = (uint32_t)x, hi = (uint32_t)(x >> 32);
    asm("s_and_b32 %0, %0, %2\n\ts_and_b32 %1, %1, %2" : "+s"(lo), "+s"(hi) : "i"(C) : "scc");
    return (unsigned long long)lo | ((unsigned long long)hi << 32);
}
template <int SPAN>
__device__ __forceinline__ int half_max_int_span(int v) {
    if constexpr (SPAN >= 4) {
        return half_max_int_p16(v);
    } else {
        v = max(v, dpp_i<DPP_QP_1032>(v));
        v = max(v, dpp_i<DPP_QP_2301>(v));
        if constexpr (SPAN >= 2) v = max(v, dpp_i<DPP_ROW_HALF_MIRROR>(v));
        if constexpr (SPAN >= 3) v = max(v, dpp_i<DPP_ROW_MIRROR>(v));
        return v;
    }
}

__device__ __forceinline__ int half_min_int_p16(int v) {
    v = min(v, dpp_i<DPP_QP_1032>(v));
    v = min(v, dpp_i<DPP_QP_2301>(v));
    v = min(v, dpp_i<DPP_ROW_HALF_MIRROR>(v));
    v = min(v, dpp_i<DPP_ROW_MIRROR>(v));
    const auto sw = __builtin_amdgcn_permlane16_swap((unsigned)v, (unsigned)v, false, false);
    return min((int)sw[0], (int)sw[1]);
}

struct PivF { pf2 oo; };

__device__ __forceinline__ pf2 recip_fast(pf2 y, float s, pf2 &oo) {
    pf2 o1p, o2p, bb, sq, q, r;
    o1p.x = rcp_rn(s);
    asm("v_pk_mul_f32 %0, %1, %2 op_sel_hi:[1,0]" : "=v"(bb) : "v"(y), "v"(o1p));
    asm("v_pk_mul_f32 %0, %1, %1" : "=v"(sq) : "v"(bb));
    o2p.x = rcp_rn(sq.x + sq.y);
    asm("v_pk_mul_f32 %0, %1, %2 op_sel_hi:[0,1] neg_hi:[0,1]" : "=v"(q) : "v"(o1p), "v"(bb));
    asm("v_pk_mul_f32 %0, %1, %2 op_sel_hi:[1,0]" : "=v"(r) : "v"(q), "v"(o2p));
    oo.x = o1p.x;
    oo.y = o2p.x;
    return r;
}

__device__ __forceinline__ pf2 pcdiv_apply(pf2 b, pf2 piv, const PivF &f) {
    pf2 bb, a, t1, t2, s, q;
    asm("v_pk_mul_f32 %0, %1, %2 op_sel_hi:[1,0]" : "=v"(bb) : "v"(piv), "v"(f.oo));
    asm("v_pk_mul_f32 %0, %1, %2 op_sel_hi:[1,0]" : "=v"(a) : "v"(b), "v"(f.oo));
    asm("v_pk_mul_f32 %0, %1, %2 op_sel_hi:[1,0]" : "=v"(t1) : "v"(a), "v"(bb));
    asm("v_pk_mul_f32 %0, %1, %2 op_sel:[1,1] op_sel_hi:[0,1]" : "=v"(t2) : "v"(a), "v"(bb));
    asm("v_pk_add_f32 %0, %1, %2 neg_hi:[0,1]" : "=v"(s) : "v"(t1), "v"(t2));
    asm("v_pk_mul_f32 %0, %1, %2 op_sel:[0,1] op_sel_hi:[1,1]" : "=v"(q) : "v"(s), "v"(f.oo));
    return q;
}

__device__ __forceinline__ uint32_t group_bits(uint32_t pmw) {
    uint32_t t = pmw;
#pragma unroll
    for (int k = 1; k < LU_CHUNK; k++) t |= pmw >> k;
    return t;
}
template <int I, int K>
__device__ __forceinline__ bool group_live(uint32_t pmw, uint32_t gb) {
    using C = LuChunks;
    constexpr int J = C::start(I, K), N = C::len(I, K);
    if constexpr (N == 1) return (pmw >> J) & 1u;
    else return (gb >> J) & 1u;
}

template <int J, int N>
__device__ __forceinline__ void grp_store(cf *w, const cf (&rA)[NV]) {
    if constexpr (N == 1) w[J] = rA[J];
    else st4(&w[J], rA[J], rA[J + 1]);
}
template <int J, int N>
__device__ __forceinline__ void grp_load(const cf *p, cf *u) {
    if constexpr (N == 1) u[0] = p[J];
    else ld4(&p[J], u[0], u[1]);
}
template <int J, int N>
__device__ __forceinline__ void grp_update(cf (&rA)[NV], const pf2 &l, const cf *u) {
#pragma unroll
    for (int q = 0; q < N; q++) {
        const pf2 v = pcmsub(pf2{rA[J + q].x, rA[J + q].y}, l, pf2{u[q].x, u[q].y});
        rA[J + q] = cmk(v.x, v.y);
    }
}

template <int I>
__device__ __forceinline__ int lu_read_pivot(const LUBuf &L, cf &reg, cf &sB0) {
    reg = L.row[I];
    cf pr;
    ld4(&L.row[30], sB0, pr);
    return __float_as_int(pr.x);
}

struct LatCols {
    static constexpr int off(int I, int K) {
        int n = 0;
        for (int k = 0; k < K; k++)
            if (lu_group_class(I, k) != GRP_DEAD) n += LuChunks::len(I, k);
        return n;
    }
    static constexpr int total(int I) { return off(I, LuChunks::count(I)); }
};
template <int I, int K>
__device__ __forceinline__ void lat_store(const cf (&rA)[NV], cf *wrow) {
    using C = LuChunks;
    if constexpr (K < C::count(I)) {
        if constexpr (lu_group_class(I, K) != GRP_DEAD) grp_store<C::start(I, K), C::len(I, K)>(wrow, rA);
        lat_store<I, K + 1>(rA, wrow);
    }
}
template <int I, int K, int LO, int HI, int M>
__device__ __forceinline__ void lat_load(cf (&u)[M], const LUBuf &L) {
    using C = LuChunks;
    if constexpr (K < C::count(I)) {
        constexpr int O = LatCols::off(I, K);
        if constexpr (lu_group_class(I, K) != GRP_DEAD && O >= LO && O < HI)
            grp_load<C::start(I, K), C::len(I, K)>(L.row, &u[O - LO]);
        lat_load<I, K + 1, LO, HI>(u, L);
    }
}
template <int I, int K, int LO, int HI, int M>
__device__ __forceinline__ void lat_fma(cf (&rA)[NV], const pf2 &l, const cf (&u)[M]) {
    using C = LuChunks;
    if constexpr (K < C::count(I)) {
        constexpr int O = LatCols::off(I, K);
        if constexpr (lu_group_class(I, K) != GRP_DEAD && O >= LO && O < HI)
            grp_update<C::start(I, K), C::len(I, K)>(rA, l, &u[O - LO]);
        lat_fma<I, K + 1, LO, HI>(rA, l, u);
    }
}
#ifndef HC_LU_LATB_COLS
#define HC_LU_LATB_COLS 8
#endif
template <int I, int LO, int B>
__device__ __forceinline__ void lat_batches(cf (&rA)[NV], const pf2 &l, const LUBuf &L) {
    constexpr int T = LatCols::total(I);
    if constexpr (LO < T) {
        constexpr int HI = LO + B;
        cf u[B + 1];
        lat_load<I, 0, LO, HI>(u, L);
        lat_fma<I, 0, LO, HI>(rA, l, u);
        lat_batches<I, HI, B>(rA, l, L);
    }
}
template <int I, int LAT>
__device__ __forceinline__ void lu_step_batched(cf (&rA)[NV], cf &rB, int &rowid, PivF &my, LUBuf &L, cf *scr,
                                                bool is_piv, pf2 reg_s, pf2 oo_s, bool elig) {
    HC_ISA_MARK_I("lu_store", I);
    cf *wrow = is_piv ? L.row : scr;
    wrow[I] = cmk(reg_s.x, reg_s.y);
    st4(&wrow[30], rB, cmk(__int_as_float(rowid), 0.0f));
    lat_store<I, 0>(rA, wrow);
    wave_lds_sync();
    HC_ISA_MARK_I("lu_rcp", I);
    cf reg, sB0;
    const int piv_pos = lu_read_pivot<I>(L, reg, sB0);
    cf u[LAT + 1];
    lat_load<I, 0, 0, LAT>(u, L);
    rowid = is_piv ? I : (rowid == I ? piv_pos : rowid);
    my.oo.x = is_piv ? oo_s.x : my.oo.x;
    my.oo.y = is_piv ? oo_s.y : my.oo.y;
    asm volatile("" : "+v"(my.oo));
    HC_ISA_MARK_I("lu_update", I);
    if (elig) {
        HC_ISA_MARK_I("lu_mult", I);
        const pf2 lq = pcmul(pf2{rA[I].x, rA[I].y}, pf2{reg.x, reg.y});
        const pf2 lp = {is_piv ? 0.0f : lq.x, is_piv ? 0.0f : lq.y};
        const pf2 bp = pcmsub(pf2{rB.x, rB.y}, lp, pf2{sB0.x, sB0.y});
        rB = cmk(bp.x, bp.y);
        lat_fma<I, 0, 0, LAT>(rA, lp, u);
        lat_batches<I, LAT, LAT>(rA, lp, L);
    }
}

template <int I, int K, bool STRUCT>
__device__ __forceinline__ void lu_group_elig(cf (&rA)[NV], const pf2 &l, uint32_t pmw, uint32_t gb, cf *wrow,
                                              const LUBuf &L HC_LU_WORK_ARG) {
    using C = LuChunks;
    if constexpr (K < C::count(I)) {
        constexpr int J = C::start(I, K), N = C::len(I, K);
        constexpr int CLS = STRUCT ? lu_group_class(I, K) : GRP_TESTED;
        if (CLS != GRP_DEAD && (CLS == GRP_ALWAYS || __builtin_expect(group_live<I, K>(pmw, gb), 1))) {
            grp_store<J, N>(wrow, rA);
            wave_lds_sync();
            HC_LU_WORK(N);
            HC_DIAG_LIVE_HIT(I, K);
            HC_LU_WORK_GROUP();
            cf u[N];
            grp_load<J, N>(L.row, u);
            grp_update<J, N>(rA, l, u);
        }
        __builtin_amdgcn_sched_barrier(0);
        lu_group_elig<I, K + 1, STRUCT>(rA, l, pmw, gb, wrow, L HC_LU_WORK_PASS);
    }
}
template <int I, bool X1, bool STRUCT>
__device__ __forceinline__ void lu_step_tested(cf (&rA)[NV], cf &rB, int &rowid, uint32_t &pat, PivF &my, LUBuf &L,
                                               cf *scr, bool is_piv, int pl0, int pl1, pf2 reg_s, pf2 oo_s,
                                               bool elig HC_LU_WORK_ARG) {
    const uint32_t pp0 = (uint32_t)__builtin_amdgcn_readlane((int)pat, pl0);
    const uint32_t pp1 = (uint32_t)__builtin_amdgcn_readlane((int)pat, pl1);
    const uint32_t pmw = (pp0 | pp1) & (0xFFFFFFFFu << (I + 1));
    const uint32_t gb = group_bits(pmw);
    HC_ISA_MARK_I("lu_store", I);
    cf *wrow;
    if constexpr (X1) {
        wrow = is_piv ? L.row : scr;
        wrow[I] = cmk(reg_s.x, reg_s.y);
        st4(&wrow[30], rB, cmk(__int_as_float(rowid), 0.0f));
    } else if (is_piv) {
        L.row[I] = cmk(reg_s.x, reg_s.y);
        L.row[30] = rB;
        L.row[31].x = __int_as_float(rowid);
    }
    wave_lds_sync();
    HC_ISA_MARK_I("lu_rcp", I);
    cf reg, sB0;
    const int piv_pos = lu_read_pivot<I>(L, reg, sB0);
    if constexpr (X1) {
        rowid = is_piv ? I : (rowid == I ? piv_pos : rowid);
        my.oo.x = is_piv ? oo_s.x : my.oo.x;
        my.oo.y = is_piv ? oo_s.y : my.oo.y;
    } else {
        if (is_piv) rowid = I;
        else if (rowid == I) rowid = piv_pos;
        if (is_piv) my.oo = oo_s;
    }
    asm volatile("" : "+v"(my.oo));
    HC_ISA_MARK_I("lu_update", I);
    if constexpr (!X1) wrow = is_piv ? L.row : scr;
#ifdef HC_DIAG_LUWORK
    lu_work_acc.excl = __builtin_amdgcn_ballot_w64(is_piv);
#endif
    HC_DIAG_LIVE_HIT(I, LIVE_SOLVES);
    if (elig) {
        HC_ISA_MARK_I("lu_mult", I);
        const pf2 lq = pcmul(pf2{rA[I].x, rA[I].y}, pf2{reg.x, reg.y});
        const pf2 lp = {is_piv ? 0.0f : lq.x, is_piv ? 0.0f : lq.y};
        const pf2 bp = pcmsub(pf2{rB.x, rB.y}, lp, pf2{sB0.x, sB0.y});
        rB = cmk(bp.x, bp.y);
        pat |= (uint32_t)__builtin_amdgcn_sbfe((int)pat, I, 1) & pmw;
        lu_group_elig<I, 0, STRUCT>(rA, lp, pmw, gb, wrow, L HC_LU_WORK_PASS);
    }
}

template <int I, int K>
__device__ __forceinline__ void lu_group_dense(cf (&rA)[NV], const pf2 &l, LUBuf &L, bool is_piv,
                                               bool below HC_LU_WORK_ARG) {
    using C = LuChunks;
    if constexpr (K < C::count(I)) {
        constexpr int J = C::start(I, K), N = C::len(I, K);
        if (is_piv) grp_store<J, N>(L.row, rA);
        wave_lds_sync();
        if (below) {
            HC_LU_WORK(N);
            HC_LU_WORK_GROUP();
            cf u[N];
            grp_load<J, N>(L.row, u);
            grp_update<J, N>(rA, l, u);
        }
        __builtin_amdgcn_sched_barrier(0);
        lu_group_dense<I, K + 1>(rA, l, L, is_piv, below HC_LU_WORK_PASS);
    }
}
template <int I>
__device__ __forceinline__ void lu_step_dense(cf (&rA)[NV], cf &rB, int &rowid, PivF &my, LUBuf &L, bool is_piv,
                                              pf2 reg_s, pf2 oo_s, bool elig HC_LU_WORK_ARG) {
    HC_ISA_MARK_I("lu_store", I);
    if (is_piv) {
        L.row[I] = cmk(reg_s.x, reg_s.y);
        L.row[30] = rB;
        L.row[31].x = __int_as_float(rowid);
    }
    wave_lds_sync();
    HC_ISA_MARK_I("lu_rcp", I);
    cf reg, sB0;
    const int piv_pos = lu_read_pivot<I>(L, reg, sB0);
    if (is_piv) rowid = I;
    else if (rowid == I) rowid = piv_pos;
    if (is_piv) my.oo = oo_s;
    asm volatile("" : "+v"(my.oo));
    const bool below = elig && !is_piv;
    pf2 lp = {0.0f, 0.0f};
    if (below) {
        HC_ISA_MARK_I("lu_mult", I);
        lp = pcmul(pf2{rA[I].x, rA[I].y}, pf2{reg.x, reg.y});
        const pf2 bp = pcmsub(pf2{rB.x, rB.y}, lp, pf2{sB0.x, sB0.y});
        rB = cmk(bp.x, bp.y);
    }
    HC_ISA_MARK_I("lu_update", I);
    lu_group_dense<I, 0>(rA, lp, L, is_piv, below HC_LU_WORK_PASS);
}

}

#include "hc_lu_levels.hpp"

namespace hc {

template <int I, bool DENSE, int LAT, bool STRUCT>
__device__ __forceinline__ void lu_forward(cf (&rA)[NV], cf &rB, int &rowid, uint32_t &pat, int lane, int r, int hb,
                                           bool row_lane, PivF &my, LUBuf &L, cf *scr, bool &redo,
                                           unsigned long long elig_m HC_LU_WORK_ARG) {
    if constexpr (I < NV) {
        HC_ISA_MARK_I("lu_search", I);
        const float v = __builtin_fabsf(rA[I].x) + __builtin_fabsf(rA[I].y);
        pf2 reg_s, oo_s;
        if constexpr (!DENSE) {
            reg_s = recip_fast(pf2{rA[I].x, rA[I].y}, v, oo_s);
        } else {
            const divf f = cdiv_factors(rA[I]);
            const cf rg = (v == 0.0f) ? cmk(1.0f, 0.0f) : cdiv_apply(cmk(1.0f, 0.0f), f);
            reg_s = pf2{rg.x, rg.y};
            oo_s = pf2{f.o1, f.o2};
        }
        const bool elig = __builtin_amdgcn_inverse_ballot_w64(elig_m);
        bool is_piv;
        float piv_abs;
        int pl0, pl1;
        unsigned long long piv_m;
        constexpr int SPAN = (STRUCT && !DENSE) ? lu_search_span(I) : 4;
        const int key = elig ? __float_as_int(v) : -1;
        const int mx = half_max_int_span<SPAN>(key);
        unsigned long long m = __builtin_amdgcn_ballot_w64(key == mx);
        unsigned long long bad = __builtin_amdgcn_ballot_w64(!rcp_fast_bits(mx));
        if constexpr (SPAN < 4) {
            m = and_halves<LU_BOUND.cand[I]>(m);
            bad = and_halves<LU_BOUND.cand[I]>(bad);
        }
        const unsigned mlo = (unsigned)m, mhi = (unsigned)(m >> 32);
        constexpr bool TIE = I == 18 || I == 19 || I == 21 || I == 22;
        const bool rare = DENSE || (TIE ? (bad != 0ull) : ((__builtin_popcountll(m) != 2) | (bad != 0ull)));
        if (__builtin_expect(rare, 0)) {
            HC_ISA_MARK_I("lu_rare", I);
#ifdef HC_DIAG_LUWORK
            lu_work_acc.rare++;
            if constexpr (!DENSE) {
                if (lane == 0) atomicAdd(&g_diag_luwork[DIAG_LUWORK_RARE_AT + I], 1ull);
                if (lu_step_fusable(I)) lu_work_acc.rare_fusable = 1ull;
            }
#endif
            const bool isn = v != v;
            const unsigned long long nanb = __builtin_amdgcn_ballot_w64(isn);
            int mx2 = mx;
            unsigned long long m2 = m;
            if constexpr (SPAN < 4) {
                mx2 = half_max_int_p16(key);
                m2 = __builtin_amdgcn_ballot_w64(key == mx2);
            }
            if (__builtin_expect(nanb != 0ull, 0)) {
                const int key2 = (elig && !isn) ? __float_as_int(v) : -1;
                mx2 = half_max_int_p16(key2);
                m2 = __builtin_amdgcn_ballot_w64(key2 == mx2);
            }
            const unsigned long long nanm = nanb & __builtin_amdgcn_ballot_w64(rowid == I);
            const unsigned nlo = (unsigned)nanm, nhi = (unsigned)(nanm >> 32);
            const unsigned mine_m = hb ? (unsigned)(m2 >> 32) : (unsigned)m2, mine_n = hb ? nhi : nlo;
            const int c2 = ((mine_m >> r) & 1u) ? rowid : (1 << 20);
            const int mn = half_min_int_p16(c2);
            const unsigned long long w = __builtin_amdgcn_ballot_w64(row_lane && rowid == mn);
            const unsigned wm = hb ? (unsigned)(w >> 32) : (unsigned)w;
            const int pl = mine_n ? hb + __builtin_ctz(mine_n) : hb + (wm ? __builtin_ctz(wm) : 0);
            is_piv = lane == pl;
            piv_abs = mine_n ? __builtin_nanf("") : __int_as_float(mx2);
            const unsigned long long pm = __builtin_amdgcn_ballot_w64(is_piv);
            piv_m = pm;
            pl0 = __builtin_ctz((unsigned)pm | 0x80000000u);
            pl1 = 32 + __builtin_ctz((unsigned)(pm >> 32) | 0x80000000u);
            if constexpr (!DENSE)
                redo = redo || __builtin_amdgcn_ballot_w64(!rcp_fast_bits(__float_as_int(piv_abs))) != 0ull;
        } else if constexpr (TIE) {
            const int c2 = key == mx ? rowid : (1 << 20);
            const int mn = half_min_int_p16(c2);
            is_piv = key == mx && rowid == mn;
            piv_abs = __int_as_float(mx);
            const unsigned long long w = __builtin_amdgcn_ballot_w64(is_piv);
            piv_m = w;
            pl0 = __builtin_ctz((unsigned)w);
            pl1 = 32 + __builtin_ctz((unsigned)(w >> 32));
        } else {
            is_piv = __builtin_amdgcn_inverse_ballot_w64(m);
            piv_m = m;
            piv_abs = __int_as_float(mx);
            pl0 = __builtin_ctz(mlo);
            pl1 = 32 + __builtin_ctz(mhi);
        }
        HC_ISA_MARK_I("lu_pattern", I);
        if constexpr (DENSE) lu_step_dense<I>(rA, rB, rowid, my, L, is_piv, reg_s, oo_s, elig HC_LU_WORK_PASS);
        else if constexpr (LAT > 0 && STRUCT) lu_step_batched<I, LAT>(rA, rB, rowid, my, L, scr, is_piv, reg_s, oo_s, elig);
        else lu_step_tested<I, (LAT > 0), STRUCT>(rA, rB, rowid, pat, my, L, scr, is_piv, pl0, pl1, reg_s, oo_s,
                                                  elig HC_LU_WORK_PASS);
        lu_forward<I + 1, DENSE, LAT, STRUCT>(rA, rB, rowid, pat, lane, r, hb, row_lane, my, L, scr, redo,
                                              elig_m & ~piv_m HC_LU_WORK_PASS);
    }
}
template <int LV>
__device__ __forceinline__ void lu_forward_fused(cf (&rA)[NV], cf &rB, int &rowid, uint32_t &pat, int lane, int r, int hb,
                                                 bool row_lane, PivF &my, LUBuf &L, cf *scr, bool &redo,
                                                 unsigned long long elig_m HC_LU_WORK_ARG) {
    if constexpr (LV < LU_LEVELS.nlevels) {
        if (!lu_level<LV>(rA, rB, rowid, pat, r, hb, my, L, scr, elig_m HC_LU_WORK_PASS)) {
#ifdef HC_DIAG_LUWORK
            lu_work_acc.rare++;
            lu_work_acc.rare_fusable = 1ull;
#endif
            redo = true;
            return;
        }
        lu_forward_fused<LV + 1>(rA, rB, rowid, pat, lane, r, hb, row_lane, my, L, scr, redo, elig_m HC_LU_WORK_PASS);
    } else {
        lu_forward<lu_first_unfused_step(), false, 0, true>(rA, rB, rowid, pat, lane, r, hb, row_lane, my, L, scr, redo,
                                                           elig_m HC_LU_WORK_PASS);
    }
}

template <int I, int LAST = 0>
__device__ __forceinline__ void lu_backward(const cf (&rA)[NV], cf &rB, int rowid, const PivF &my, pf2 &res) {
    if constexpr (I >= LAST) {
        HC_ISA_MARK_I("lu_back", I);
        const unsigned long long own = __builtin_amdgcn_ballot_w64(rowid == I);
        const int o0 = __builtin_ctz((unsigned)own);
        const int o1 = 32 + __builtin_ctz((unsigned)(own >> 32));
        const pf2 q = pcdiv_apply(pf2{rB.x, rB.y}, pf2{rA[I].x, rA[I].y}, my);
        const float x0 = __int_as_float(__builtin_amdgcn_readlane(__float_as_int(q.x), o0));
        const float y0 = __int_as_float(__builtin_amdgcn_readlane(__float_as_int(q.y), o0));
        const float x1 = __int_as_float(__builtin_amdgcn_readlane(__float_as_int(q.x), o1));
        const float y1 = __int_as_float(__builtin_amdgcn_readlane(__float_as_int(q.y), o1));
        const pf2 xs0 = {x0, y0}, xs1 = {x1, y1};
        pf2 xv;
        unsigned long long tmp;
        asm volatile("s_nop 1\n\ts_mov_b64 %2, exec\n\tv_mov_b64 %0, %3\n\ts_mov_b32 exec_lo, 0\n\t"
                     "v_mov_b64 %0, %4\n\ts_mov_b32 exec_lo, %5\n\ts_mov_b32 exec_hi, %5\n\t"
                     "v_mov_b64 %1, %0\n\ts_mov_b64 exec, %2"
                     : "=&v"(xv), "+v"(res), "=&s"(tmp) : "s"(xs0), "s"(xs1), "i"(1u << I));
        if constexpr (I > 0) {
            const pf2 w = pcmsub(pf2{rB.x, rB.y}, xv, pf2{rA[I].x, rA[I].y});
            rB = cmk(w.x, w.y);
        }
        lu_backward<I - 1, LAST>(rA, rB, rowid, my, res);
    }
}

struct LuMode { int lat; bool strct, entchk, fuse; };
constexpr LuMode lu_mode(bool ABORT, bool ARCH, int LULAT, bool LUS) {
    const bool entchk = !ABORT && !ARCH && LULAT == 0;
    return LuMode{LULAT, LUS, entchk, entchk && LUS};
}

template <bool DENSE, int LAT = 0, bool STRUCT = false, bool ENTCHK = false, bool FUSE = false>
__device__ __forceinline__ cf lu_solve(cf (&rA)[NV], cf rB, int lane, uint32_t pattern, LUBuf &L, cf *scratch,
                                      bool &redo, unsigned long long count_mask = ~0ull, bool ent_bad = false) {
    static_assert(!FUSE || (!DENSE && LAT == 0 && STRUCT && ENTCHK), "the fused levels belong to the throughput tracker's solve");
    (void)count_mask;
    const int r = lane & 31, hb = lane & 32;
    const bool row_lane = r < NV;
    redo = false;
    if constexpr (DENSE) HC_ISA_MARK("lu_dense");
    else HC_ISA_MARK("lu_sparse");
    HC_ISA_MARK("lu_finite");
    if constexpr (!DENSE && ENTCHK) {
        if (__builtin_expect(ent_bad, 0)) {
            redo = true;
            return cmk(0.0f, 0.0f);
        }
    } else if constexpr (!DENSE) {
        pf2 sq = {0.0f, 0.0f};
#pragma unroll
        for (int c = 0; c < NV; c++) {
            const pf2 e = {rA[c].x, rA[c].y};
            asm("v_pk_fma_f32 %0, %1, %1, %0" : "+v"(sq) : "v"(e));
        }
        const bool ok = sq.x + sq.y < __builtin_inff();
        if (__builtin_expect(__builtin_amdgcn_ballot_w64(!ok) != 0ull, 0)) {
            redo = true;
            return cmk(0.0f, 0.0f);
        }
    }
    int rowid = row_lane ? r : FUSE ? NV : 99;
    uint32_t pat = row_lane ? pattern : 0u;
    PivF my{pf2{0.0f, 0.0f}};
#ifdef HC_DIAG_LUWORK
    LuWork lu_work_acc{0ull, count_mask, 0ull, 0ull, 0ull, 0ull};
#endif
    if constexpr (FUSE)
        lu_forward_fused<0>(rA, rB, rowid, pat, lane, r, hb, row_lane, my, L, scratch + 2 * r, redo,
                            __builtin_amdgcn_ballot_w64(row_lane) HC_LU_WORK_PASS);
    else
        lu_forward<0, DENSE, LAT, STRUCT>(rA, rB, rowid, pat, lane, r, hb, row_lane, my, L, scratch + 2 * r, redo,
                                          __builtin_amdgcn_ballot_w64(row_lane) HC_LU_WORK_PASS);
#ifdef HC_DIAG_LUWORK
    const unsigned long long solves = (unsigned long long)__builtin_popcountll(count_mask & __builtin_amdgcn_ballot_w64(row_lane)) / NV;
    if (lane == 0 && !DENSE && !redo) {
        atomicAdd(&g_diag_luwork[0], lu_work_acc.acc);
        atomicAdd(&g_diag_luwork[1], solves);
        atomicAdd(&g_diag_luwork[3], 1ull);
        atomicAdd(&g_diag_luwork[4], lu_work_acc.groups);
        atomicAdd(&g_diag_luwork[5], lu_work_acc.rare);
    }
    if (lane == 0 && DENSE) atomicAdd(&g_diag_luwork[2], solves);
    if (lane == 0 && !DENSE) atomicAdd(&g_diag_luwork[DIAG_LUWORK_RARE_FUSABLE], lu_work_acc.rare_fusable);
#endif
    if constexpr (FUSE) {
        if (__builtin_expect(redo, 0)) return cmk(0.0f, 0.0f);
    }
#ifdef HC_DIAG_PHASES
    if ((lane & 63) == 0 && blockIdx.x < 16384u) g_diag_lu_mid[blockIdx.x * 4 + (threadIdx.x >> 6)] = __builtin_amdgcn_s_memtime();
#endif
    HC_ISA_MARK("lu_back_init");
    pf2 res = {0.0f, 0.0f};
    if constexpr (FUSE) {
        lu_backward<NV - 1, lu_first_unfused_step()>(rA, rB, rowid, my, res);
        lu_backward_fused<LU_LEVELS.nlevels - 1>(rA, rB, rowid, my, L, r, res);
        const float nf = __builtin_fmaf(res.y, 0.0f, res.x * 0.0f);
        redo = __builtin_amdgcn_ballot_w64(nf != nf) != 0ull;
#ifdef HC_DIAG_LUWORK
        if (lane == 0 && redo) {
            atomicAdd(&g_diag_luwork[0], 0ull - lu_work_acc.acc);
            atomicAdd(&g_diag_luwork[1], 0ull - solves);
            atomicAdd(&g_diag_luwork[3], 0ull - 1ull);
            atomicAdd(&g_diag_luwork[4], 0ull - lu_work_acc.groups);
            atomicAdd(&g_diag_luwork[5], 0ull - lu_work_acc.rare);
        }
#endif
    } else {
        lu_backward<NV - 1>(rA, rB, rowid, my, res);
    }
    return cmk(res.x, res.y);
}

}
```

### trifocal_pose_estimation_using_improved_gpuhc_amd/csrc/hc_lu_levels.hpp

```cpp
#pragma once

namespace hc {

constexpr int DPP_WAVE_SHL1 = 0x130, DPP_WAVE_SHR1 = 0x138;

__device__ __forceinline__ uint32_t *lu_rowtab_lds() {
    __shared__ uint32_t t[LU_REC_WORDS];
    return t;
}
__device__ __forceinline__ void lu_rowtab_fill(int tid) {
    if (tid < LU_REC_WORDS) lu_rowtab_lds()[tid] = LU_ROWTAB.w[tid];
}
template <int LV, int K>
__device__ __forceinline__ void lvl_pick(const cf (&rA)[NV], pf2 &c, int kk) {
    if constexpr (K < lu_level_count(LV)) {
        constexpr int I = lu_level_member(LV, K);
        const bool in = kk == K;
        c.x = in ? rA[I].x : c.x;
        c.y = in ? rA[I].y : c.y;
        lvl_pick<LV, K + 1>(rA, c, kk);
    }
}

template <int LV>
__device__ __forceinline__ void lvl_relabel(int &rowid, int mem, bool is_piv, unsigned long long live_m, const LUBuf &L) {
    const bool live = __builtin_amdgcn_inverse_ballot_w64(live_m);
    for (;;) {
        const int t = __float_as_int(L.row[rowid].x);
        rowid = live ? t : rowid;
        const bool again = live && ((lu_member_cols(LV) >> rowid) & 1u) != 0u;
        if (__builtin_expect(__builtin_amdgcn_ballot_w64(again) == 0ull, 1)) break;
    }
    rowid = is_piv ? mem : rowid;
}
template <int LV, int J>
__device__ __forceinline__ void lvl_groups(cf (&rA)[NV], const pf2 &l, cf *wrow, const cf *cw) {
    if constexpr (J < NV) {
        if constexpr (((LU_LEVELS.cols[LV] >> J) & 3u) != 0u) {
            grp_store<J, 2>(wrow, rA);
            wave_lds_sync();
            cf u[2];
            grp_load<J, 2>(cw, u);
            grp_update<J, 2>(rA, l, u);
            __builtin_amdgcn_sched_barrier(0);
        }
        lvl_groups<LV, J + 2>(rA, l, wrow, cw);
    }
}
template <int LV>
__device__ __forceinline__ bool lu_level(cf (&rA)[NV], cf &rB, int &rowid, uint32_t &pat, int r, int hb, PivF &my,
                                         LUBuf &L, cf *scr, unsigned long long &elig_m HC_LU_WORK_ARG) {
    constexpr int CNT = lu_level_count(LV), I0 = lu_level_member(LV, 0);
    constexpr uint32_t ROWS = LU_LEVELS.rows[LV];
    HC_ISA_MARK_I("lu_search", I0);
    pf2 c = {0.0f, 0.0f};
    const uint32_t rec = lu_rowtab_lds()[LV * LU_REC_ROWS + r];
    lvl_pick<LV, 0>(rA, c, (int)((rec >> LU_REC_CHAIN_AT) & 15u));
    const float v = __builtin_fabsf(c.x) + __builtin_fabsf(c.y);
    pf2 oo_s;
    const pf2 reg_s = recip_fast(c, v, oo_s);
    const unsigned long long lv_elig = and_halves<ROWS>(elig_m);
    const bool elig = __builtin_amdgcn_inverse_ballot_w64(lv_elig);
    const int key = elig ? __float_as_int(v) : -1;
    int mx;
    {
        const int u1 = dpp_i<DPP_WAVE_SHL1>(key), u2 = dpp_i<DPP_WAVE_SHL1>(u1);
        const int d1 = dpp_i<DPP_WAVE_SHR1>(key), d2 = dpp_i<DPP_WAVE_SHR1>(d1);
        const int a = rec >= LU_REC_UP ? u1 : d2;
        const int b = (int)rec < 0 ? u2 : d1;
        mx = max(key, max(a, b));
    }
    if constexpr (lu_partner_rows(LV, 0) != (1u << NV) - 1u) {
        const int pl = (int)((rec >> LU_REC_PARTNER_AT) & 31u) + hb;
        mx = max(mx, __builtin_amdgcn_ds_bpermute(pl << 2, mx));
    }
    const unsigned long long m = and_halves<ROWS>(__builtin_amdgcn_ballot_w64(key == mx));
    const unsigned long long bad = and_halves<ROWS>(__builtin_amdgcn_ballot_w64(!rcp_fast_bits(mx)));
    if (__builtin_expect((__builtin_popcountll(m) != 2 * CNT) | (bad != 0ull), 0)) return false;
    const bool is_piv = __builtin_amdgcn_inverse_ballot_w64(m);
    HC_ISA_MARK_I("lu_store", I0);
    const cf *cw = reinterpret_cast<const cf *>(reinterpret_cast<const char *>(scr) + (rec & ((1u << LU_REC_WIN_BITS) - 1u)));
    cf *wrow = is_piv ? const_cast<cf *>(cw) : scr;
    st4(&wrow[0], cmk(reg_s.x, reg_s.y), rB);
    const int mem = (int)((rec >> LU_REC_MEMBER_AT) & 31u);
    const uint32_t bnd = lu_rowtab_lds()[LU_REC_BOUND0 + mem];
    if constexpr (LV == 0) L.row[r].x = __int_as_float(r);
    if (is_piv) L.row[mem].x = __int_as_float(rowid);
    wave_lds_sync();
    HC_ISA_MARK_I("lu_rcp", I0);
    cf reg, sB0;
    ld4(&cw[0], reg, sB0);
    if (is_piv) my.oo = oo_s;
    asm volatile("" : "+v"(my.oo));
    lvl_relabel<LV>(rowid, mem, is_piv, elig_m & ~m, L);
    HC_ISA_MARK_I("lu_update", I0);
#ifdef HC_DIAG_LUWORK
    {
        int pairs = 0;
        for (int j = 0; j < NV; j += 2) pairs += ((LU_LEVELS.cols[LV] >> j) & 3u) != 0u;
        lu_work_acc.acc += 2ull * (unsigned long long)pairs *
                           (unsigned long long)__builtin_popcountll(lv_elig & lu_work_acc.mask & ~m);
        lu_work_acc.groups += (unsigned long long)pairs;
    }
#endif
    if (elig) {
        HC_ISA_MARK_I("lu_mult", I0);
        const pf2 lq = pcmul(c, pf2{reg.x, reg.y});
        const pf2 lp = {is_piv ? 0.0f : lq.x, is_piv ? 0.0f : lq.y};
        const pf2 bp = pcmsub(pf2{rB.x, rB.y}, lp, pf2{sB0.x, sB0.y});
        rB = cmk(bp.x, bp.y);
        pat |= (pat & lu_member_cols(LV)) != 0u ? bnd : 0u;
        lvl_groups<LV, 0>(rA, lp, wrow, cw);
    }
    elig_m &= ~m;
    return true;
}

template <int LV>
__device__ __forceinline__ void lu_back_level(const cf (&rA)[NV], cf &rB, int rowid, const PivF &my, LUBuf &L, int r) {
    HC_ISA_MARK_I("lu_back_level", LV);
    pf2 c = {0.0f, 0.0f};
    const uint32_t rec = lu_rowtab_lds()[LV * LU_REC_ROWS + r];
    lvl_pick<LV, 0>(rA, c, (int)((rec >> LU_REC_CHAIN_AT) & 15u));
    const int mem = (int)((rec >> LU_REC_MEMBER_AT) & 31u);
    const pf2 q = pcdiv_apply(pf2{rB.x, rB.y}, c, my);
    if (rowid == mem) L.row[mem] = cmk(q.x, q.y);
    wave_lds_sync();
    if constexpr (LV > 0) {
        if (__builtin_amdgcn_inverse_ballot_w64(lu_both(LU_LEVELS.rows[LV]))) {
            const cf x = L.row[mem];
            const pf2 w = pcmsub(pf2{rB.x, rB.y}, pf2{x.x, x.y}, c);
            rB = cmk(w.x, w.y);
        }
    }
}
template <int LV>
__device__ __forceinline__ void lu_backward_fused(const cf (&rA)[NV], cf &rB, int rowid, const PivF &my, LUBuf &L, int r,
                                                  pf2 &res) {
    if constexpr (LV >= 0) {
        lu_back_level<LV>(rA, rB, rowid, my, L, r);
        lu_backward_fused<LV - 1>(rA, rB, rowid, my, L, r, res);
    } else {
        if (__builtin_amdgcn_inverse_ballot_w64(lu_both(lu_fused_steps()))) {
            const cf x = L.row[r];
            res = pf2{x.x, x.y};
        }
    }
}

}
```

### trifocal_pose_estimation_using_improved_gpuhc_amd/csrc/hc_lu_struct.hpp

```cpp
#pragma once

#include <initializer_list>

#include "hc_device.hpp"

namespace hc {

constexpr int LU_CHUNK = 2;

struct LuChunks {
    static constexpr int single(int I) { return ((I + 1) & 1) && (I + 1 < NV) ? 1 : 0; }
    static constexpr int start(int I, int k) { return k < single(I) ? I + 1 : I + 1 + single(I) + (k - single(I)) * LU_CHUNK; }
    static constexpr int len(int I, int k) {
        return k < single(I) ? 1 : ((NV - start(I, k)) < LU_CHUNK ? (NV - start(I, k)) : LU_CHUNK);
    }
    static constexpr int count(int I) { return single(I) + (NV - (I + 1 + single(I)) + LU_CHUNK - 1) / LU_CHUNK; }
    static constexpr uint32_t mask(int I, int k) { return ((1u << len(I, k)) - 1u) << start(I, k); }
};

constexpr uint32_t LU_STRUCT_PAT[NV] = {
    0x7040004u, 0x7080004u, 0x7100004u, 0x7040009u, 0x7080009u, 0x7100009u, 0x7040012u, 0x7080012u,
    0x7100012u, 0x38200020u, 0x38400020u, 0x38800020u, 0x38200041u, 0x38400041u, 0x38800041u, 0x38200082u,
    0x38400082u, 0x38800082u, 0x7003100u, 0x7003100u, 0x7001100u, 0x7018400u, 0x7018400u, 0x7008400u,
    0x38005200u, 0x38005200u, 0x38001200u, 0x38028800u, 0x38028800u, 0x38008800u};
// ... 78 lines not shown
constexpr bool lu_levels_ordered() {
    for (int j = 0; j < NV; j++)
        for (int i = 0; i < j; i++)
            if (lu_step_fusable(j) && (LU_BOUND.cand[i] & LU_BOUND.cand[j]) != 0u &&
                !(lu_step_fusable(i) && LU_LEVELS.level[i] < LU_LEVELS.level[j])) return false;
    return true;
}
constexpr bool lu_back_chains_nested() {
    for (int i = 0; i < NV; i++)
        for (int j = i + 1; j < NV; j++)
            if (lu_step_fusable(i) && lu_step_fusable(j) && ((LU_BOUND.s[i] >> j) & 1u) &&
                !((LU_BOUND.cand[i] & ~LU_BOUND.cand[j]) == 0u && LU_LEVELS.level[i] < LU_LEVELS.level[j])) return false;
    return true;
}
constexpr bool lu_back_order_kept() {
    for (int r = 0; r < NV; r++) {
        int last = -1;
        for (int l = 0; l < NV; l++)
            for (int i = 0; i < NV; i++)
                if (lu_step_fusable(i) && LU_LEVELS.level[i] == l && ((LU_BOUND.cand[i] >> r) & 1u)) {
                    if (i <= last) return false;
                    last = i;
                }
    }
    return true;
}
constexpr uint32_t lu_fused_steps() {
    uint32_t m = 0u;
    for (int l = 0; l < LU_LEVELS.nlevels; l++) m |= LU_LEVELS.fused[l];
    return m;
}
constexpr int lu_first_unfused_step() {
    int i = 0;
    while (i < NV && ((lu_fused_steps() >> i) & 1u)) i++;
    return i;
}
constexpr uint32_t lu_bits(std::initializer_list<int> v) {
    uint32_t m = 0u;
    for (int b : v) m |= 1u << b;
    return m;
}
static_assert(lu_levels_disjoint(), "two steps of one level share a candidate row");
static_assert(lu_levels_ordered(), "a fused step depends on a step outside the lower fused levels");
static_assert(lu_back_chains_nested(), "a fused pivot row can hold a fused column outside its chain's ancestors");
static_assert(lu_back_order_kept(), "a row's ancestors do not rise in column with the level");
static_assert(lu_fused_steps() == (1u << 18) - 1u, "the fused levels cover exactly steps 0..17");
static_assert(LU_LEVELS.nlevels == 4 && LU_LEVELS.fused[0] == lu_bits({0, 1, 2, 5, 8, 9, 10, 11}) &&
              LU_LEVELS.fused[1] == lu_bits({3, 4, 12, 15}) && LU_LEVELS.fused[2] == lu_bits({6, 7, 13, 16}) &&
              LU_LEVELS.fused[3] == lu_bits({14, 17}), "the levels of DESIGN.md §3.5");
static_assert(LU_LEVELS.rows[0] == (1u << NV) - 1u && LU_LEVELS.rows[1] == (LU_LEVELS.rows[0] & ~lu_bits({0, 1, 2, 9, 10, 11})) &&
              LU_LEVELS.rows[2] == LU_LEVELS.rows[1] && LU_LEVELS.rows[3] == (0x3FFC0000u & LU_LEVELS.rows[0]),
              "the rows the levels work on");

constexpr int lu_level_count(int lv) { return lu_popcount(LU_LEVELS.fused[lv]); }
constexpr int lu_level_member(int lv, int k) {
    for (int i = 0; i < NV; i++)
        if ((LU_LEVELS.fused[lv] >> i) & 1u) {
            if (k == 0) return i;
            k--;
        }
    return -1;
}
constexpr int lu_max_level_count() {
    int n = 0;
    for (int l = 0; l < LU_LEVELS.nlevels; l++)
        if (lu_level_count(l) > n) n = lu_level_count(l);
    return n;
}
constexpr int lu_partner_off(int lv, int row) {
    for (int k = 0; k < lu_level_count(lv); k++) {
        const uint32_t c = LU_BOUND.cand[lu_level_member(lv, k)];
        if (!((c >> row) & 1u) || lu_popcount(c) <= 3) continue;
        int lo = 0, hi = 31;
        while (!((c >> lo) & 1u)) lo++;
        while (!((c >> hi) & 1u)) hi--;
        return row < lo + 3 ? (hi - 2) - lo : lo - (hi - 2);
    }
    return 0;
}
constexpr uint32_t lu_partner_rows(int lv, int off) {
    uint32_t m = 0u;
    for (int r = 0; r < NV; r++)
        if (lu_partner_off(lv, r) == off) m |= 1u << r;
    return m;
}
constexpr bool lu_chains_are_triples() {
    for (int i = 0; i < NV; i++) {
        if (!lu_step_fusable(i)) continue;
        uint32_t c = LU_BOUND.cand[i], t = 0u;
        for (int q = 0; q < NV; q += 3)
            if (((c >> q) & 7u) == 7u) t |= 7u << q;
        if (t != c) return false;
    }
    return true;
}
static_assert(lu_chains_are_triples(), "a fusable step's candidates are not whole lane triples");
constexpr uint32_t lu_member_cols(int lv) { return LU_LEVELS.fused[lv]; }
constexpr unsigned long long lu_both(uint32_t m) { return (unsigned long long)m | ((unsigned long long)m << 32); }
constexpr uint32_t LU_TRI0 = 0x09249249u, LU_TRI1 = LU_TRI0 << 1, LU_TRI2 = LU_TRI0 << 2;

constexpr int LU_SCRATCH_CF = 2 * 31 + 32;
constexpr int LU_CHAIN_WIN0 = LU_SCRATCH_CF;
constexpr int LU_SCRATCH_FUSED_CF = LU_CHAIN_WIN0 + 2 * (lu_max_level_count() - 1) + 32;

struct LuRowRec { uint32_t bound, word; };
constexpr int LU_REC_WIN_BITS = 10, LU_REC_MEMBER_AT = 10, LU_REC_PARTNER_AT = 15, LU_REC_CHAIN_AT = 20;
constexpr uint32_t LU_REC_UP = 1u << 30, LU_REC_FIRST = 1u << 31;
constexpr int LU_REC_NO_MEMBER = 31, LU_REC_NO_CHAIN = 15;
constexpr int LU_REC_ROWS = 32, LU_REC_LEVELS = 4;
constexpr int lu_row_chain(int lv, int row) {
    if (row >= NV) return -1;
    for (int k = 0; k < lu_level_count(lv); k++)
        if ((LU_BOUND.cand[lu_level_member(lv, k)] >> row) & 1u) return k;
    return -1;
}
constexpr LuRowRec lu_row_record(int lv, int row) {
    const int k = lu_row_chain(lv, row);
    const uint32_t place = (row % 3 == 0 ? LU_REC_FIRST : 0u) | (row % 3 != 2 ? LU_REC_UP : 0u);
    if (k < 0)
        return LuRowRec{0u, place | (uint32_t)LU_REC_NO_CHAIN << LU_REC_CHAIN_AT | (uint32_t)row << LU_REC_PARTNER_AT |
                                (uint32_t)LU_REC_NO_MEMBER << LU_REC_MEMBER_AT};
    const int I = lu_level_member(lv, k);
    return LuRowRec{LU_BOUND.s[I], place | (uint32_t)k << LU_REC_CHAIN_AT |
                                       (uint32_t)(row + lu_partner_off(lv, row)) << LU_REC_PARTNER_AT |
                                       (uint32_t)I << LU_REC_MEMBER_AT | (uint32_t)(8 * (LU_CHAIN_WIN0 + 2 * k - 2 * row))};
}
constexpr int LU_REC_BOUND0 = LU_REC_LEVELS * LU_REC_ROWS, LU_REC_WORDS = LU_REC_BOUND0 + LU_REC_NO_MEMBER + 1;
struct LuRowTab { uint32_t w[LU_REC_WORDS]; };
constexpr LuRowTab lu_row_table() {
    LuRowTab t{};
    for (int lv = 0; lv < LU_REC_LEVELS; lv++)
        for (int r = 0; r < LU_REC_ROWS; r++) {
            const LuRowRec rec = lu_row_record(lv, r);
            t.w[lv * LU_REC_ROWS + r] = rec.word;
            t.w[LU_REC_BOUND0 + (int)((rec.word >> LU_REC_MEMBER_AT) & 31u)] = rec.bound;
        }
    return t;
}
constexpr LuRowTab LU_ROWTAB = lu_row_table();
constexpr bool lu_row_fields_fit() {
    for (int lv = 0; lv < LU_REC_LEVELS; lv++)
        for (int r = 0; r < NV; r++) {
            const int k = lu_row_chain(lv, r), p = r + lu_partner_off(lv, r);
            if (k < 0) continue;
            const int win = 8 * (LU_CHAIN_WIN0 + 2 * k - 2 * r);
            if (win <= 0 || win >= (1 << LU_REC_WIN_BITS) || k >= LU_REC_NO_CHAIN || p < 0 || p >= NV) return false;
            if (lu_level_member(lv, k) >= LU_REC_NO_MEMBER || (LU_BOUND.s[lu_level_member(lv, k)] >> NV) != 0u) return false;
        }
    return true;
}
static_assert(LU_LEVELS.nlevels == LU_REC_LEVELS && lu_row_fields_fit(), "a field of the row records overflows");
static_assert(LU_REC_WORDS * sizeof(uint32_t) <= 640, "a larger row table may cost the headline kernel its fifth workgroup per CU: measure");

}
```

### trifocal_pose_estimation_using_improved_gpuhc_amd/csrc/hc_prep_body.inc

```
    const int32_t *__restrict__ U = pa.U;
    Workspace *ws = pa.ws;
    EvalTables *T = &ws->tab;
    __shared__ int s_len[32];
    __shared__ int s_bad;
    __shared__ int s_nostruct;
    __shared__ unsigned long long s_h[PREP_THREADS];
    __shared__ unsigned s_cleared, s_dlo, s_dhi;
    __shared__ int s_valid;
    const int tid = threadIdx.x;
    {
        unsigned long long h = 0;
        if constexpr (P2C) {
            for (int i = tid; i < P2C_HX_SIZE; i += PREP_THREADS)
                h += mix64(((unsigned long long)i << 32) | (unsigned)U[i]);
            for (int i = tid; i < P2C_HT_SIZE; i += PREP_THREADS)
                h += mix64(((unsigned long long)(P2C_HX_SIZE + i) << 32) | (unsigned)D_in[i]);
        } else if (((uintptr_t)U & 15u) == 0u) {
            const int4 *U4 = reinterpret_cast<const int4 *>(U);
            static_assert((HX_SIZE + HT_SIZE) % 4 == 0, "whole int4 words");
#pragma unroll 4
            for (int i = tid; i < (HX_SIZE + HT_SIZE) / 4; i += PREP_THREADS) {
                const int4 v = U4[i];
                const unsigned long long b = (unsigned long long)(4 * i) << 32;
                h += mix64(b | (unsigned)v.x) + mix64((b + (1ull << 32)) | (unsigned)v.y) +
// ... 256 lines not shown
                                        x30 | x30 << 8 | x30 << 16);
        int k = 0;
        if (r < NV) {
            for (int j = 0; j < HT_TERMS; j++) {
                const int base = j * HT_PARTS * NV + r;
                const int co = P2C ? htp(j, 0, r) : D[base], a = P2C ? htp(j, 1, r) : D[base + NV],
                          b = P2C ? htp(j, 2, r) : D[base + 2 * NV], u = P2C ? htp(j, 3, r) : D[base + 3 * NV],
                          v = P2C ? htp(j, 4, r) : D[base + 4 * NV], x3 = P2C ? htp(j, 5, r) : D[base + 5 * NV];
                if (co == 0) continue;
                bad |= co < -128 || co > 127 || a < 0 || a >= NPP || b < 0 || b >= NPP || u < 0 || u > NV ||
                       v < 0 || v > NV || x3 < 0 || x3 > NV;
                if (!bad) {
                    const uint2 tw = make_uint2(tp_off(co, a, b) | qp_off(a, b) << 16,
                                                (uint32_t)(SLOT_OFF_X + 8 * u) | ((uint32_t)(SLOT_OFF_X + 8 * v) << 8) |
                                                    ((uint32_t)(SLOT_OFF_X + 8 * x3) << 16) |
                                                    (((uint32_t)co & 0xFFu) << 24));
                    T->ht[k * 32 + r] = tw;
                    if (k >= HT_FULL) T->ht[(HT_HELP_FIRST + k - HT_FULL) * 32 + (r ^ 16)] = tw;
                }
                k++;
            }
        }
        for (int q = k; q < HT_TERMS; q++)
            if (!(q >= HT_HELP_FIRST && q < HT_HELP_FIRST + need_h)) T->ht[q * 32 + r] = pad_ht;
        if (bad) atomicOr(&s_bad, 1);
    }
    __shared__ uint32_t s_adj[TP_CAP][3];
    __shared__ uint8_t s_pidx[HX_SLOT_CAP + HT_FULL][32];
    __shared__ uint8_t s_tslot[TP_CAP], s_tinv[TP_CAP], s_order[TP_CAP];
    __shared__ int s_deg[TP_CAP];
    for (int i = tid; i < TP_CAP * 3; i += PREP_THREADS) (&s_adj[0][0])[i] = 0u;
    for (int i = tid; i < TP_CAP; i += PREP_THREADS) { s_tinv[i] = 0xFFu; s_tslot[i] = 0u; }
    __syncthreads();
    const int ntri = s_ntri;
    auto tp_index = [&](uint32_t w) -> uint32_t {
        const uint32_t o = w & 0xFFFFu;
        const uint32_t i = (o - (uint32_t)SLOT_OFF_TP) / 8u;
        return o >= (uint32_t)SLOT_OFF_TP && i < (uint32_t)ntri ? i : (uint32_t)TP_CAP;
    };
    for (int i = tid; i < (HX_SLOT_CAP + HT_FULL) * 32; i += PREP_THREADS) {
        const int p = i >> 5, l = i & 31;
        const uint32_t w = p < HX_SLOT_CAP ? T->hx[p * 32 + l] : T->ht[(p - HX_SLOT_CAP) * 32 + l].x;
        s_pidx[p][l] = (uint8_t)min(tp_index(w), (uint32_t)0xFFu);
    }
    __syncthreads();
    for (int i = tid; i < (HX_SLOT_CAP + HT_FULL) * 32; i += PREP_THREADS) {
        const int p = i >> 5, l = i & 31;
        const uint32_t t = s_pidx[p][l];
        if (t >= (uint32_t)ntri) continue;
        for (int l2 = 0; l2 < 32; l2++) {
            const uint32_t u = s_pidx[p][l2];
            if (u != t && u < (uint32_t)ntri) atomicOr(&s_adj[t][u >> 5], 1u << (u & 31));
        }
    }
    __syncthreads();
    if (tid < ntri)
        s_deg[tid] = tid == 0 ? (1 << 20) : __popc(s_adj[tid][0]) + __popc(s_adj[tid][1]) + __popc(s_adj[tid][2]);
    __syncthreads();
    if (tid < ntri) {
        int rk = 0;
        const int d = s_deg[tid];
        for (int u = 0; u < ntri; u++) rk += (s_deg[u] > d || (s_deg[u] == d && u < tid)) ? 1 : 0;
        s_order[rk] = (uint8_t)tid;
    }
    __syncthreads();
    if (tid < 64) {
        uint32_t m0 = 0u, m1 = 0u, m2 = 0u;
        int fill = 0;
        for (int k2 = 0; k2 < ntri; k2++) {
            const int t = s_order[k2];
            const int conf = __popc(s_adj[t][0] & m0) + __popc(s_adj[t][1] & m1) + __popc(s_adj[t][2] & m2);
            int key = (tid < 32 && fill < 3) ? ((conf * 4 + fill) << 5 | tid) : 0x7FFFFFFF;
            for (int s2 = 32; s2 > 0; s2 >>= 1) key = min(key, __shfl_xor(key, s2, 64));
            if (tid == (key & 31)) {
                const int slot = tid + 32 * fill++;
                s_tslot[t] = (uint8_t)slot;
                s_tinv[slot] = (uint8_t)t;
                if (t < 32) m0 |= 1u << t; else if (t < 64) m1 |= 1u << (t - 32); else m2 |= 1u << (t - 64);
            }
        }
    }
    __syncthreads();
    for (int i = tid; i < HX_SLOT_CAP * 32; i += PREP_THREADS) {
        const uint32_t w = T->hx[i], t = tp_index(w);
        if (t < (uint32_t)TP_CAP) T->hx[i] = (w & ~0xFFFFu) | (uint32_t)(SLOT_OFF_TP + 8 * s_tslot[t]);
    }
    for (int i = tid; i < HT_TERMS * 32; i += PREP_THREADS) {
        const uint32_t w = T->ht[i].x, t = tp_index(w);
        if (t < (uint32_t)TP_CAP) T->ht[i].x = (w & ~0xFFFFu) | (uint32_t)(SLOT_OFF_TP + 8 * s_tslot[t]);
    }
    if (r < 32) {
        const uint32_t p33 = (uint32_t)(SLOT_OFF_STG + 8 * 33);
        for (int q = 0; q < PRE_ROUNDS; q++) {
            const bool tpr = q < PRE_TP_ROUNDS;
            const int i = (tpr ? q : q - PRE_TP_ROUNDS) * 32 + r;
            uint2 job = make_uint2(p33 | p33 << 16, (uint32_t)SLOT_OFF_HXDUMMY);
            if (tpr && i < TP_CAP && s_tinv[i] != 0xFFu) {
                const uint32_t key = s_tri[s_tinv[i]];
                const uint32_t a = (key >> 8) & 0xFFu, b = key >> 16;
                job = make_uint2((uint32_t)(SLOT_OFF_STG + 8 * a) | (uint32_t)(SLOT_OFF_STG + 8 * b) << 16,
                                 (uint32_t)(SLOT_OFF_TP + 8 * i) | (key & 0xFFu) << 16);
                if constexpr (P2C)
                    job.x = (uint32_t)(SLOT_OFF_STG + 8 * (b > 1u ? (uint32_t)(P2C_NK - 1) : a + 32u * b));
            } else if (!tpr && i < s_npair) {
                const uint32_t a = s_pair[i] & 0xFFu, b = s_pair[i] >> 8;
                job = make_uint2((uint32_t)(SLOT_OFF_STG + 8 * a) | (uint32_t)(SLOT_OFF_STG + 8 * b) << 16,
                                 (uint32_t)(SLOT_OFF_QP + 8 * i));
                if constexpr (P2C)
                    job.x = (uint32_t)(SLOT_OFF_STG + 8 * (b > 1u ? (uint32_t)(P2C_NK - 1) : a + 32u * b));
            }
            T->pre[q][r] = job;
        }
    }
    __syncthreads();
    {
        AbsTables *A = &ws->abs;
        auto slot_base = [](int i) -> uint32_t {
            return (uint32_t)(((i >> 6) * 2 + ((i >> 5) & 1)) * (int)sizeof(SlotLDS));
        };
        for (int i = tid; i < ABS_WAVES * HX_SLOT_CAP * WAVE; i += PREP_THREADS) {
            const int l = i & 63, k = (i >> 6) % HX_SLOT_CAP, wv = (i >> 6) / HX_SLOT_CAP;
            const uint32_t sb = slot_base(wv * 64 + l);
            const uint32_t w = T->hx[k * 32 + (l & 31)];
            const int sl = hx_gslot(k);
            const uint32_t d = T->hxd[sl >> 1][l & 31];
            A->hx[wv][k][l] = make_uint4(sb + (w & 0xFFFFu), sb + ((w >> 16) & 0xFFu), sb + (w >> 24),
                                         sb + ((sl & 1) ? d >> 16 : d & 0xFFFFu));
        }
        for (int i = tid; i < ABS_WAVES * (HT_FULL + 1) * WAVE; i += PREP_THREADS) {
            const int l = i & 63, j = (i >> 6) % (HT_FULL + 1), wv = (i >> 6) / (HT_FULL + 1);
            const uint32_t sb = slot_base(wv * 64 + l);
            if (j < HT_FULL) {
                const uint2 w = T->ht[j * 32 + (l & 31)];
                A->ht[wv][j][l] = make_uint4(sb + (w.y & 0xFFu), sb + ((w.y >> 8) & 0xFFu), sb + ((w.y >> 16) & 0xFFu),
                                             sb + (w.x & 0xFFFFu));
                A->htq[wv][j][l] = make_uint2(sb + (w.x >> 16), __float_as_uint(coef_ht(w)));
            } else {
                uint32_t xw[3] = {sb + x30, sb + x30, sb + x30};
                for (int q = 0; q < HT_HELP; q++) xw[q] = sb + ((T->ht[(HT_FULL + q) * 32 + (l & 31)].y >> 16) & 0xFFu);
                A->ht[wv][j][l] = make_uint4(xw[0], xw[1], xw[2], sb + x30);
            }
        }
        for (int i = tid; i < ABS_WAVES * ABS_GM_Q * WAVE; i += PREP_THREADS) {
            const int l = i & 63, q = (i >> 6) % ABS_GM_Q, wv = (i >> 6) / ABS_GM_Q;
            const uint32_t sb = slot_base(wv * 64 + l);
            uint32_t g[4];
            for (int e = 0; e < 4; e++) {
                const int c = 4 * q + e;
                const uint32_t w = T->gm[min(c, NV - 1) >> 1][l & 31];
                g[e] = sb + ((c & 1) ? w >> 16 : w & 0xFFFFu);
            }
            A->gm[wv][q][l] = make_uint4(g[0], g[1], g[2], g[3]);
        }
    }
    if (r == 0) {
        for (int q = 0; q < 4; q++) {
            uint32_t am = 0xFFFFFFFFu, lm = 0u;
            for (int l = 0; l < 32; l++)
                if (s_htn[l] - HT_FULL > q) { am &= ~(1u << (l ^ 16)); lm |= 1u << l; }
            T->ht_acc_mask[q] = am;
            T->ht_light_mask[q] = lm;
        }
        int mx = 0;
        for (int q = 0; q < 32; q++) mx = max(mx, s_len[q]);
        T->hx_len = mx;
        T->status = s_bad ? HC_ERROR_TABLE : 0;
        T->lu_struct = s_nostruct ? 0u : 1u;
        T->src_hash = src_hash;
        T->magic = TAB_MAGIC;
        if (s_bad) ws->status = HC_ERROR_TABLE;
    }
```

### trifocal_pose_estimation_using_improved_gpuhc_amd/csrc/hc_track_body.inc

```
    constexpr LuMode LUM = lu_mode(ABORT, ARCH, LULAT, LUS);
    constexpr bool LUSTRUCT = LUM.strct;
    constexpr bool ABSTAB = LUM.entchk;
    constexpr bool LUFUSE = LUM.fuse;
    __shared__ cf s_sp[NPP];
    __shared__ SlotLDS s_slot[2 * WAVES_PER_WG];
    Workspace *ws = a.ws;
    const EvalTables *T = &ws->tab;
    if (ws->status != 0u) return;
    if ((T->lu_struct == 1u) != LUSTRUCT) return;
    const unsigned epoch = (!ABORT && a.slice_q > 0) ? ld_rlx(&a.rq[RQ_EPOCH]) : 0u;
    const uint2 *s_ht = T->ht;
    const uint32_t *s_hx = T->hx;
    const uint32_t *s_hxd = &T->hxd[0][0];
    if (!P2C && threadIdx.x < NPP) s_sp[threadIdx.x] = a.start_params[threadIdx.x];
    {
        float *z = reinterpret_cast<float *>(s_slot);
        for (int i = threadIdx.x; i < (int)(sizeof(s_slot) / 4); i += WG_THREADS) z[i] = 0.0f;
    }
    __syncthreads();
    if (ABORT && threadIdx.x == 0) atomicCAS(&ws->t_start, 0ull, (unsigned long long)__builtin_amdgcn_s_memrealtime());
    const int lane = lane_id();
    const int r = lane & 31, hb = lane & 32;
    const int wid = threadIdx.x / WAVE;
    SlotLDS &S = s_slot[wid * 2 + (hb >> 5)];
// ... 269 lines not shown
                    }
                    t_step = t0;
                    h2 = (float)(0.5 * (double)dt);
                    scale = 0.0f;
                    coef = 1;
                    s = 0;
                    nsteps++;
                    piece++;
                    if constexpr (REUSE) {
                        if (k1v) {
                            drain_stores();
                            const cf k1 = rl ? ld_cf_rlx(reinterpret_cast<const cf *>(a.susp + (size_t)b * SUSP_WORDS + r))
                                             : cmk(0.0f, 0.0f);
                            sols = cadd(sols, cscale(cscale(k1, dt), (float)(1.0 / 6.0)));
                            scale += h2;
                            coef <<= 1;
                            x = cadd(x, cscale(k1, scale));
                            t0 += h2;
                            s = 1;
#ifdef HC_DIAG_LUWORK
                            if (r == 0) atomicAdd(&g_diag_luwork[10], 1ull);
#endif
                        }
                    }
                }
                k1v = false;
                ph = suspend ? PH_DEQ : done ? PH_FINISH : PH_STAGE;
            }
            if (__ballot(ph == PH_FINISH || ph == PH_DEQ || ph == PH_BEGIN) == 0ull) break;
        }
        if (__ballot(ph == PH_STAGE) == 0ull) break;
#ifdef HC_DIAG_UTIL
        {
            const unsigned long long bs = __ballot(ph == PH_STAGE);
            if (lane == 0) {
                const unsigned bin = (unsigned)(__builtin_amdgcn_s_memrealtime() >> 10) & (UTIL_BINS - 1);
                unsigned long long *u = g_diag_util[blockIdx.x % UTIL_COPIES][bin];
                atomicAdd(&u[0], (unsigned long long)((bs & 1ull) + ((bs >> 32) & 1ull)));
                atomicAdd(&u[1], 1ull);
            }
        }
#endif
        if (ABORT) {
            const int qp = (ph == PH_STAGE) ? qpos : 0x7FFFFFFF;
            const int m = min(__builtin_amdgcn_readlane(qp, 0), __builtin_amdgcn_readlane(qp, 32));
            const int lvl = (int)((long long)m * HC_ABORT_PRIO_DIV / a.num_paths);
            if (lvl <= 0) __builtin_amdgcn_s_setprio(3);
            else if (lvl == 1) __builtin_amdgcn_s_setprio(2);
            else if (lvl == 2) __builtin_amdgcn_s_setprio(1);
            else __builtin_amdgcn_s_setprio(0);
        }
        if (!ABORT && a.ordered && a.slice_q == 0) {
            const int qp = (ph == PH_STAGE) ? qpos : 0;
            const int m = max(__builtin_amdgcn_readlane(qp, 0), __builtin_amdgcn_readlane(qp, 32));
            const int lvl = (int)((long long)m * PRIO_TENTHS / a.num_paths);
            if (lvl >= PRIO_TENTHS - 1) __builtin_amdgcn_s_setprio(3);
            else if (lvl >= PRIO_TENTHS - 2) __builtin_amdgcn_s_setprio(2);
            else if (lvl >= PRIO_TENTHS - 3) __builtin_amdgcn_s_setprio(1);
            else __builtin_amdgcn_s_setprio(0);
        }
        if (!ABORT && a.slice_q > 0) {
            const int si = (ph == PH_STAGE) ? stepidx : (1 << 20);
            const int m = min(__builtin_amdgcn_readlane(si, 0), __builtin_amdgcn_readlane(si, 32));
            const int q4 = (int)((long long)m * 4 / (a.max_steps + 1));
            if (q4 <= 0) __builtin_amdgcn_s_setprio(3);
            else if (q4 == 1) __builtin_amdgcn_s_setprio(2);
            else if (q4 == 2) __builtin_amdgcn_s_setprio(1);
            else __builtin_amdgcn_s_setprio(0);
        }
        HC_DIAG_MARK(0);
        if constexpr (GROUPED) {
            if (a.inflight_stop)
                found_seen = ph == PH_STAGE ? __hip_atomic_load(&a.group_found[a.sample_group[smp_loaded]],
                                                                __ATOMIC_RELAXED, __HIP_MEMORY_SCOPE_AGENT)
                                            : 0u;
            if constexpr (ADAPT) {
                if (a.inflight_stop && ph == PH_STAGE)
                    found_seen |= (unsigned)a.sample_ordinal[smp_loaded] >=
                                          __hip_atomic_load(&a.group_limit[a.sample_group[smp_loaded]], __ATOMIC_RELAXED,
                                                            __HIP_MEMORY_SCOPE_AGENT)
                                      ? 1u : 0u;
            }
        } else if (ABORT && a.inflight_stop) {
            found_seen = __hip_atomic_load(&ws->found, __ATOMIC_RELAXED, __HIP_MEMORY_SCOPE_AGENT);
            if (a.peer_found) found_seen |= __hip_atomic_load(a.peer_found, __ATOMIC_RELAXED, __HIP_MEMORY_SCOPE_SYSTEM);
        }

        HC_ISA_MARK("ctl_park");
        const float pre_t = S.st.pre_t;
        const int pre_smp = S.st.pre_smp;
        const bool rebuild = __ballot(ph == PH_STAGE && (__float_as_uint(t0) != __float_as_uint(pre_t) ||
                                                         smp_loaded != pre_smp)) != 0ull;
        if (r == 0) {
            SlotState q;
            q.t0 = t0; q.t_step = t_step; q.dt = dt; q.h2 = h2; q.scale = scale;
            q.s = s; q.stepidx = stepidx; q.coef = coef; q.succ = succ; q.nsteps = nsteps; q.ncorr = ncorr;
            q.b = b; q.smp = smp_loaded; q.ph = ph;
            q.flags = (end_zone ? 1 : 0) | (check ? 2 : 0) | (isSucc ? 4 : 0) | (isInf ? 8 : 0) | (piece << 4);
            q.pad = qpos;
            q.pre_t = rebuild ? t0 : pre_t;
            q.pre_smp = rebuild ? smp_loaded : pre_smp;
            S.st = q;
        }
        if (rl) { S.x[r] = x; S.xl[r] = xl; S.sols[r] = sols; }
        if (rebuild) {
            HC_ISA_MARK("ctl_prefix");
#ifdef HC_DIAG_LUWORK
            if (lane_fresh() == 0) atomicAdd(&g_diag_luwork[9], 1ull);
#endif
            const int rs = lane_fresh() & 31;
            const size_t so = (size_t)(smp_loaded > 0 ? smp_loaded : 0) * NPP;
            if constexpr (P2C) {
                const size_t sk = (size_t)(smp_loaded > 0 ? smp_loaded : 0) * P2C_NK;
                build_prefixes_p2c(S, rs, &T->pre[0][0], a.target_params + sk * 3, a.diff_params + sk * 2, t0);
            } else {
                build_prefixes(S, rs, &T->pre[0][0], a.target_params + so, a.diff_params + so, s_sp, t0);
            }
        }
        wave_lds_sync();
        const int s_in = s, ph_in = ph;
        asm volatile("" :: "v"(s_in), "v"(ph_in));
        const int lane_v = lane_fresh();
        const int r_v = lane_v & 31;
        const uint32_t l16 = (uint32_t)lane_v << 4;
        const uint32_t row_pat = s_rowc[GM_WORDS][r_v];
        const bool act = ph_in == PH_STAGE;
        const bool pred = act && s_in < 4;
        HC_DIAG_MARK(1);
        cf rB = cmk(0.0f, 0.0f);
        HC_ISA_MARK("ev_rhs");
        {
            const bool any_p = __ballot(pred) != 0ull, any_c = __ballot(act && !pred) != 0ull;
            const RhsMasks mk = rhs_masks(T);
#ifdef HC_DIAG_LUWORK
            if (lane_v == 0) atomicAdd(&g_diag_luwork[any_p && any_c ? 6 : any_p ? 7 : 8], 1ull);
#endif
            if (any_p && any_c) {
                HC_ISA_MARK("ev_rhs_mixed");
                if constexpr (ABSTAB) rB = eval_rhs_abs<RHS_MIXED>(AT->ht[wv], AT->htq[wv], l0, l16, pred, mk);
                else rB = eval_rhs<RHS_MIXED>(s_ht, S, r_v, pred, mk);
            } else if (any_p) {
                HC_ISA_MARK("ev_rhs_ht");
                const cf t = ABSTAB ? eval_rhs_abs<RHS_HT>(AT->ht[wv], AT->htq[wv], l0, l16, true, mk)
                                    : eval_rhs<RHS_HT>(s_ht, S, r_v, true, mk);
                if (pred) rB = t;
            } else if (any_c) {
                HC_ISA_MARK("ev_rhs_h");
                const cf t = ABSTAB ? eval_rhs_abs<RHS_H>(AT->ht[wv], AT->htq[wv], l0, l16, false, mk)
                                    : eval_rhs<RHS_H>(s_ht, S, r_v, false, mk);
                if (!pred) rB = t;
            }
        }
        HC_DIAG_MARK(3);
        cf rA[NV];
        HC_ISA_MARK("ev_hx");
        bool ent_ok = true;
        if constexpr (ABSTAB) {
            uint4 gmv[ABS_GM_Q];
            ent_ok = eval_hx_terms_abs(AT->hx[wv], l0, l16, AT->gm[wv], gmv);
            wave_lds_sync();
            HC_ISA_MARK("ev_gather");
            gather_hx_abs(rA, l0, gmv);
        } else {
            eval_hx(rA, s_hx, s_hxd, &s_rowc[0][0], S, r_v);
        }
        wave_lds_sync();
        const bool ent_bad = ABSTAB && __ballot(!ent_ok) != 0ull;
        HC_DIAG_MARK(2);
        bool redo;
        LUBuf &LB = *reinterpret_cast<LUBuf *>(S.lu);
        static_assert(ENT_CAP - 1 >= LU_SCRATCH_FUSED_CF && offsetof(SlotLDS, ent) % 16 == 0, "LU scratch in SlotLDS::ent");
        cf k = lu_solve<false, LUM.lat, LUSTRUCT, ABSTAB, LUFUSE>(rA, rB, lane_v, row_pat, LB, S.ent, redo,
                                                                  HC_LU_COUNT(__ballot(act)), ent_bad);
        HC_ISA_MARK("ctl_redo");
        if (__builtin_expect(redo, 0)) {
            HC_ISA_MARK("redo_evals");
            const bool act_r = S.st.ph == PH_STAGE, pred_r = act_r && S.st.s < 4;
            const int l_r = lane_fresh(), r_r = l_r & 31;
            const uint32_t l16_r = (uint32_t)l_r << 4;
            cf rb = cmk(0.0f, 0.0f);
            if (__ballot(pred_r) != 0ull) {
                const cf t = ABSTAB ? eval_rhs_abs<RHS_HT>(AT->ht[wv], AT->htq[wv], l0, l16_r, true, rhs_masks(T))
                                    : eval_rhs<RHS_HT>(s_ht, S, r_r, true, rhs_masks(T));
                if (pred_r) rb = t;
            }
            if (__ballot(act_r && !pred_r) != 0ull) {
                const cf t = ABSTAB ? eval_rhs_abs<RHS_H>(AT->ht[wv], AT->htq[wv], l0, l16_r, false, rhs_masks(T))
                                    : eval_rhs<RHS_H>(s_ht, S, r_r, false, rhs_masks(T));
                if (!pred_r) rb = t;
            }
            if constexpr (ABSTAB) {
                uint4 gmv[ABS_GM_Q];
                eval_hx_terms_abs(AT->hx[wv], l0, l16_r, AT->gm[wv], gmv);
                wave_lds_sync();
                gather_hx_abs(rA, l0, gmv);
            } else {
                eval_hx_terms(s_hx, s_hxd, reinterpret_cast<char *>(&S), r_r);
                wave_lds_sync();
                gather_hx(rA, &s_rowc[0][0], S, r_r);
            }
            wave_lds_sync();
            k = lu_solve<true>(rA, rb, lane_v, row_pat, LB, S.ent, redo, HC_LU_COUNT(__ballot(act_r)));
        }
        wave_lds_sync();
#ifdef HC_DIAG_PHASES
        {
            const uint64_t mid = g_diag_lu_mid[blockIdx.x * 4 + wid];
            const uint64_t n_ = __builtin_amdgcn_s_memtime();
            if (mid > dt_ && mid < n_) { dg[4] += mid - dt_; dt_ = mid; }
        }
#endif
        HC_DIAG_MARK(5);
        HC_ISA_MARK("ctl_update");
        {
            const SlotState q = S.st;
            t0 = q.t0; t_step = q.t_step; dt = q.dt; h2 = q.h2; scale = q.scale;
            s = q.s; stepidx = q.stepidx; coef = q.coef; succ = q.succ; nsteps = q.nsteps; ncorr = q.ncorr;
            b = q.b; smp_loaded = q.smp; ph = q.ph;
            end_zone = q.flags & 1; check = q.flags & 2; isSucc = q.flags & 4; isInf = q.flags & 8;
            piece = q.flags >> 4;
            qpos = q.pad;
            k1v = false;
            x = rl ? S.x[r] : cmk(0.0f, 0.0f);
            xl = rl ? S.xl[r] : cmk(0.0f, 0.0f);
            sols = rl ? S.sols[r] : cmk(0.0f, 0.0f);
        }
        const bool act_q = ph == PH_STAGE, pred_q = act_q && s < 4;
        if (act_q) {
            bool step_end = false;
            if (pred_q) {
                if (ARCH && s < 3 && a.explicit_rk) {
                    const cf kd = cmul(cscale(k, dt), cmk(1.0f, 0.0f));
                    sols = cadd(sols, cdivs(cscale(kd, 1.0f), s == 0 ? 6.0f : 3.0f));
                    if (s > 0) x = xl;
                    x = cadd(x, cmul(k, cmk(s == 2 ? dt : h2, 0.0f)));
                    if (s != 1) t0 += h2;
                } else if (s < 3) {
                    const float w = coef == 1   ? (float)(1.0 / 6.0)
                                    : coef == 2 ? (float)(2.0 / 6.0)
                                                : (float)((double)coef * 1.0 / 6.0);
                    sols = cadd(sols, cscale(cscale(k, dt), w));
                    if (coef > 1) x = xl;
                    const int sc = (s == 1) ? 0 : 1;
                    scale += (float)sc * h2;
                    coef <<= sc;
                    x = cadd(x, cscale(k, scale));
                    t0 += (float)sc * h2;
                    if constexpr (REUSE) {
                        if (s == 0 && rl && a.slice_q > 0 && a.retry_reuse)
                            st_cf_rlx(reinterpret_cast<cf *>(a.susp + (size_t)b * SUSP_WORDS + r), k);
                    }
                } else {
                    sols = cadd(sols, cdivs(cscale(cscale(k, dt), 1.0f), 6.0f));
                    x = sols;
                }
                s++;
                if (s == 4 && a.max_corr <= 0) step_end = true;
            } else {
                x = csub(x, k);
                ncorr++;
                const float vs = rl ? k.x * k.x + k.y * k.y : 0.0f;
                const float vc = rl ? x.x * x.x + x.y * x.y : 0.0f;
                const float ns = tree_sum_half(vs), nc = tree_sum_half(vc);
                isSucc = (double)ns < 0.000001 * (double)nc;
                isInf = (double)nc > 1e14;
                if (isInf || isSucc || (s - 4) + 1 >= a.max_corr) step_end = true;
                else s++;
            }
            if (step_end) {
                if (isInf) {
                    ph = PH_FINISH;
                } else {
                    if (!isSucc) {
                        dt = (float)((double)dt * 0.5);
                        x = xl;
                        sols = xl;
                        succ = 0;
                        t0 = t_step;
                        if constexpr (REUSE) k1v = a.slice_q > 0 && a.retry_reuse;
                    } else {
                        succ++;
                        xl = x;
                        sols = x;
                        if (succ >= a.inc_steps) { succ = 0; dt *= 2.0f; }
                    }
                    stepidx++;
                    ph = PH_BEGIN;
                }
            }
        }
    }
#ifdef HC_DIAG_TIMES
    if (lane == 0) {
        const unsigned long long w1 = __builtin_amdgcn_s_memrealtime();
        atomicMax(&g_diag_span[1], w1);
        atomicAdd(&g_diag_span[2], w1 - diag_w0);
        atomicAdd(&g_diag_span[3], 1ull);
    }
#endif
#ifdef HC_DIAG_PHASES
    HC_DIAG_MARK(0);
    if (lane == 0) {
        dg[7] = __builtin_amdgcn_s_memtime() - dt0_;
        for (int q = 0; q < 8; q++) atomicAdd(&g_diag_phase[q], (unsigned long long)dg[q]);
        atomicAdd(&g_diag_phase[8], 1ull);
    }
#endif
#undef HC_DIAG_MARK
```

### trifocal_pose_estimation_using_improved_gpuhc_amd/tracker.py

```python
from __future__ import annotations

import ctypes as C
from dataclasses import dataclass

import numpy as np
import torch

from . import _abi
from .problem import Problem, RansacData

PATH_STATS_DTYPE = np.dtype([("steps", "<i4"), ("corrections", "<i4"), ("inliers21", "<i4"), ("inliers31", "<i4")])


_TRACK_ENTRY = {(True, True, False): "hc_trifocal_2op1p_30x30_track_abort",
                (False, True, False): "hc_trifocal_2op1p_30x30_track",
                (False, False, False): "hc_trifocal_2op1p_30x30_track_ph_codeopt",
                (False, False, True): "hc_trifocal_2op1p_30x30_track_ph"}


def _require_gpu(device) -> torch.device:
    dev = torch.device(device)
    if dev.type != "cuda" or not torch.cuda.is_available():
        raise _abi.HCError("the GPU-HC tracker needs a ROCm GPU (no CPU fallback exists)")
    return dev
# ... 336 lines not shown
        self.launch(tgt, dif, r, abort=abort, inflight_stop=inflight_stop, truncate=truncate, explicit_rk=explicit_rk,
                    time_slicing=time_slicing)
        torch.cuda.synchronize(self.device)
        self.workspace_status()
        return r

    def launch_p2c(self, tables, coeffs_hx: torch.Tensor, coeffs_ht: torch.Tensor, r: TrackResult,
                   stream: torch.cuda.Stream | None = None, workspace: torch.Tensor | None = None,
                   num_samples: int | None = None) -> None:
        hx, ht = tables
        if num_samples is None:
            num_samples = coeffs_hx.shape[0]
        if num_samples < 0 or num_samples > coeffs_hx.shape[0] or num_samples > coeffs_ht.shape[0] or \
                num_samples * 312 > r.tracks.shape[0]:
            raise _abi.HCError("sample range outside the buffers")
        if hx.numel() != 28800 or ht.numel() != 2400 or hx.dtype != torch.int32 or ht.dtype != torch.int32:
            raise _abi.HCError("P2C tables: 28800 and 2400 int32 values")
        if tuple(coeffs_hx.shape[1:]) != (38, 3, 2) or tuple(coeffs_ht.shape[1:]) != (38, 2, 2) or \
                coeffs_hx.dtype != torch.float32 or coeffs_ht.dtype != torch.float32 or \
                not coeffs_hx.is_contiguous() or not coeffs_ht.is_contiguous():
            raise _abi.HCError("P2C coefficient blocks: contiguous float32 (N, 38, 3, 2) and (N, 38, 2, 2)")
        ws_t = self._workspace(workspace)
        a = _abi.hcTrackArgs()
        a.sub_ransac_iters = num_samples
        a.settings = self.settings
        a.start_sols = self.start_sols.data_ptr()
        a.tracks = r.tracks.data_ptr()
        a.converge = r.converge.data_ptr()
        a.infinity = r.infinity.data_ptr()
        a.stats = r.stats.data_ptr() if r.stats is not None else None
        pa = _abi.hcP2cArgs(hx.data_ptr(), ht.data_ptr(), coeffs_hx.data_ptr(), coeffs_ht.data_ptr())
        s = stream if stream is not None else torch.cuda.current_stream(self.device)
        _abi.call("hc_trifocal_2op1p_30x30_track_p2c", C.byref(a), C.byref(pa), _abi.ptr(ws_t), self.ws_bytes,
                  _abi.ptr(s))

    def p2c_tables(self, tables):
        hx, ht = tables
        return (torch.from_numpy(np.ascontiguousarray(hx, np.int32).reshape(-1)).to(self.device),
                torch.from_numpy(np.ascontiguousarray(ht, np.int32).reshape(-1)).to(self.device))

    def track_p2c(self, target: np.ndarray, diff: np.ndarray, tables=None, coeff_map=None,
                  stats: bool = True) -> TrackResult:
        from . import p2c
        if tables is None:
            if self._p2c_default is None:
                hx, ht, m = p2c.tables_from_ph(self._problem)
                self._p2c_default = (self.p2c_tables((hx, ht)), m)
            dev_tables, default_map = self._p2c_default
            if coeff_map is None:
                coeff_map = default_map
        else:
            if coeff_map is None:
                coeff_map = p2c.derive_coeff_map(self._problem, tables[0], tables[1])
            dev_tables = self.p2c_tables(tables)
        chx, cht = p2c.coefficients(coeff_map, self._problem.start_params, diff)
        chx_t, cht_t = torch.from_numpy(chx).to(self.device), torch.from_numpy(cht).to(self.device)
        r = self.allocate(chx.shape[0], stats=stats)
        self.reset_tracks(r)
        self.launch_p2c(dev_tables, chx_t, cht_t, r)
        torch.cuda.synchronize(self.device)
        self.workspace_status()
        return r

    def first_found_seconds(self) -> float:
        v = C.c_double(0.0)
        _abi.call("hc_trifocal_read_timings", _abi.ptr(self.workspace), C.byref(v))
        return v.value


def cgesv_batched(A: np.ndarray, b: np.ndarray, device="cuda:0") -> np.ndarray:
    dev = _require_gpu(device)
    At = torch.from_numpy(np.ascontiguousarray(A, np.float32)).to(dev)
    bt = torch.from_numpy(np.ascontiguousarray(b, np.float32)).to(dev)
    xt = torch.empty_like(bt)
    n = At.shape[0]
    _abi.call("hc_cgesv_30x30_batched", n, _abi.ptr(At), _abi.ptr(bt), _abi.ptr(xt),
              _abi.ptr(torch.cuda.current_stream(dev)))
    torch.cuda.synchronize(dev)
    return xt.cpu().numpy()


def cgesv_struct_batched(A: np.ndarray, b: np.ndarray, device="cuda:0") -> np.ndarray:
    dev = _require_gpu(device)
    At = torch.from_numpy(np.ascontiguousarray(A, np.float32)).to(dev)
    bt = torch.from_numpy(np.ascontiguousarray(b, np.float32)).to(dev)
    xt = torch.empty_like(bt)
    _abi.call("hc_cgesv_30x30_struct_batched", At.shape[0], _abi.ptr(At), _abi.ptr(bt), _abi.ptr(xt),
              _abi.ptr(torch.cuda.current_stream(dev)))
    torch.cuda.synchronize(dev)
    return xt.cpu().numpy()


def cgesv_variant_batched(variant, A: np.ndarray, b: np.ndarray, device="cuda:0") -> np.ndarray:
    dev = _require_gpu(device)
    if isinstance(variant, str):
        variant = _abi.LU_VARIANTS.index(variant)
    At = torch.from_numpy(np.ascontiguousarray(A, np.float32)).to(dev)
    bt = torch.from_numpy(np.ascontiguousarray(b, np.float32)).to(dev)
    xt = torch.empty_like(bt)
    _abi.call("hc_cgesv_30x30_variant_batched", int(variant), At.shape[0], _abi.ptr(At), _abi.ptr(bt), _abi.ptr(xt),
              _abi.ptr(torch.cuda.current_stream(dev)))
    torch.cuda.synchronize(dev)
    return xt.cpu().numpy()


def eval_batched(unified: np.ndarray, x: np.ndarray, p: np.ndarray, d: np.ndarray, device="cuda:0"):
    dev = _require_gpu(device)
    n = x.shape[0]
    U = torch.from_numpy(np.ascontiguousarray(unified, np.int32)).to(dev)
    X = torch.from_numpy(np.ascontiguousarray(x, np.float32)).to(dev)
    P = torch.from_numpy(np.ascontiguousarray(p, np.float32)).to(dev)
    D = torch.from_numpy(np.ascontiguousarray(d, np.float32)).to(dev)
    HX = torch.empty((n, 30, 30, 2), dtype=torch.float32, device=dev)
    HT = torch.empty((n, 30, 2), dtype=torch.float32, device=dev)
    H = torch.empty((n, 30, 2), dtype=torch.float32, device=dev)
    wsb = int(_abi.lib().hc_trifocal_workspace_size())
    ws = torch.zeros(wsb, dtype=torch.uint8, device=dev)
    _abi.call("hc_trifocal_eval_batched", n, *(_abi.ptr(t) for t in (U, X, P, D, HX, HT, H, ws)), wsb,
              _abi.ptr(torch.cuda.current_stream(dev)))
    torch.cuda.synchronize(dev)
    return HX.cpu().numpy(), HT.cpu().numpy(), H.cpu().numpy()


def eval_variant_batched(variant, unified: np.ndarray, x: np.ndarray, target: np.ndarray, diff: np.ndarray,
                         start_params: np.ndarray, t: np.ndarray, kind: np.ndarray, redo: bool = False,
                         device="cuda:0", workspace: torch.Tensor | None = None):
    dev = _require_gpu(device)
    if isinstance(variant, str):
        variant = _abi.EVAL_VARIANTS.index(variant)
    n = x.shape[0]
    U = torch.from_numpy(np.ascontiguousarray(unified, np.int32)).to(dev)
    X = torch.from_numpy(np.ascontiguousarray(x, np.float32)).to(dev)
    TG = torch.from_numpy(np.ascontiguousarray(target, np.float32)).to(dev)
    DF = torch.from_numpy(np.ascontiguousarray(diff, np.float32)).to(dev)
    SP = torch.from_numpy(np.ascontiguousarray(start_params, np.float32)).to(dev)
    T = torch.from_numpy(np.ascontiguousarray(t, np.float32)).to(dev)
    K = torch.from_numpy(np.ascontiguousarray(kind, np.uint8)).to(dev)
    if tuple(X.shape) != (n, 31, 2) or tuple(TG.shape) != (n, 34, 2) or tuple(DF.shape) != (n, 34, 2) or \
            tuple(SP.shape) != (34, 2) or tuple(T.shape) != (n,) or tuple(K.shape) != (n,) or U.numel() != 38880:
        raise _abi.HCError("eval_variant_batched: x (n, 31, 2), target and diff (n, 34, 2), start_params (34, 2), "
                           "t and kind (n,), a unified index of 38880 values")
    HX = torch.empty((n, 30, 30, 2), dtype=torch.float32, device=dev)
    RHS = torch.empty((n, 30, 2), dtype=torch.float32, device=dev)
    OK = torch.full((n, 32), 255, dtype=torch.uint8, device=dev)
    wsb = int(_abi.lib().hc_trifocal_workspace_size())
    ws = workspace if workspace is not None else torch.zeros(wsb, dtype=torch.uint8, device=dev)
    if ws.numel() * ws.element_size() < wsb:
        raise _abi.HCError("eval_variant_batched: workspace too small")
    _abi.call("hc_trifocal_eval_variant_batched", int(variant), _abi.HC_EVAL_REDO if redo else 0, n,
              *(_abi.ptr(v) for v in (U, X, TG, DF, SP, T, K, HX, RHS, OK, ws)), ws.numel() * ws.element_size(),
              _abi.ptr(torch.cuda.current_stream(dev)))
    torch.cuda.synchronize(dev)
    return HX.cpu().numpy(), RHS.cpu().numpy(), OK.cpu().numpy()
```

Before: 1.645 million.

## Keep fused LU solve row in 16 compact positions instead of 30 columns

```diff
diff --git a/include/lu/hc_lu_compact_testing.h b/include/lu/hc_lu_compact_testing.h
--- /dev/null
+++ b/include/lu/hc_lu_compact_testing.h
@@ -0,0 +1,23 @@
+#ifndef HC_LU_COMPACT_TESTING_H
+#define HC_LU_COMPACT_TESTING_H
+
+#include "../hc_trifocal.h"
+
+#ifdef __cplusplus
+extern "C" {
+#endif
+
+#define HC_LU_COMPACT_WIDTH 16
+
+int hc_lu_compact_column(int row, int position);
+
+hcStatus hc_trifocal_compact_rows_batched(int n, const int32_t *unified_index, const hcComplex *x,
+                                          const hcComplex *target, const hcComplex *diff,
+                                          const hcComplex *start_params, const float *t, const uint8_t *kind,
+                                          hcComplex *rows, hcComplex *rhs, uint8_t *ent_ok, void *workspace,
+                                          size_t workspace_bytes);
+
+#ifdef __cplusplus
+}
+#endif
+#endif
diff --git a/trifocal_pose_estimation_using_improved_gpuhc_amd/_abi.py b/trifocal_pose_estimation_using_improved_gpuhc_amd/_abi.py
--- a/trifocal_pose_estimation_using_improved_gpuhc_amd/_abi.py
+++ b/trifocal_pose_estimation_using_improved_gpuhc_amd/_abi.py
@@ -314,6 +314,12 @@
 )
 LU_ROW_FIELDS = ("member", "bound", "window", "partner", "place", "chain")
 
+LU_COMPACT_SIGNATURES = (
+    Sig("hc_lu_compact_column", _i, (_i, _i), True),
+    Sig("hc_trifocal_compact_rows_batched", _ST, (_i, _p, _p, _p, _p, _p, _p, _p, _p, _p, _p, _p, C.c_size_t), True),
+)
+LU_COMPACT_WIDTH = 16
+
 EVAL_SIGNATURES = (
     Sig("hc_trifocal_eval_variant_batched", _ST, (_i, _u, _i, _p, _p, _p, _p, _p, _p, _p, _p, _p, _p, *_WS), True),
 )
@@ -337,7 +343,7 @@
         import torch
         L = C.CDLL(LIB_PATH)
         for s in SIGNATURES + P2C_SIGNATURES + REFINE_SIGNATURES + TOPK_SIGNATURES + LU_SIGNATURES + \
-                LU_ROWTABLE_SIGNATURES + EVAL_SIGNATURES + ADAPTIVE_SIGNATURES:
+                LU_ROWTABLE_SIGNATURES + LU_COMPACT_SIGNATURES + EVAL_SIGNATURES + ADAPTIVE_SIGNATURES:
             fn = getattr(L, s.name, None)
             if fn is None:
                 if s.optional:
diff --git a/trifocal_pose_estimation_using_improved_gpuhc_amd/csrc/hc_components.hpp b/trifocal_pose_estimation_using_improved_gpuhc_amd/csrc/hc_components.hpp
--- a/trifocal_pose_estimation_using_improved_gpuhc_amd/csrc/hc_components.hpp
+++ b/trifocal_pose_estimation_using_improved_gpuhc_amd/csrc/hc_components.hpp
@@ -58,18 +58,34 @@
     const int r = lane & 31;
     const int sys = (blockIdx.x * WAVES_PER_WG + threadIdx.x / WAVE) * 2 + (lane >> 5);
     const bool ok = sys < n && r < NV;
-    cf rA[NV];
+    cf rA[LuRowForm<FUSE>::W];
     uint32_t nz = 0;
     pf2 sq = {0.0f, 0.0f};
-#pragma unroll
-    for (int c = 0; c < NV; c++) {
-        rA[c] = ok ? A[((size_t)sys * NV + r) * NV + c] : cmk(0.0f, 0.0f);
-        if constexpr (!STRUCT) {
-            if (rA[c].x != 0.0f || rA[c].y != 0.0f) nz |= 1u << c;
-        }
-        if constexpr (ENTCHK) {
-            sq.x = __builtin_fmaf(rA[c].x, rA[c].x, sq.x);
-            sq.y = __builtin_fmaf(rA[c].y, rA[c].y, sq.y);
+    if constexpr (!FUSE) {
+#pragma unroll
+        for (int c = 0; c < NV; c++) {
+            rA[c] = ok ? A[((size_t)sys * NV + r) * NV + c] : cmk(0.0f, 0.0f);
+            if constexpr (!STRUCT) {
+                if (rA[c].x != 0.0f || rA[c].y != 0.0f) nz |= 1u << c;
+            }
+            if constexpr (ENTCHK) {
+                sq.x = __builtin_fmaf(rA[c].x, rA[c].x, sq.x);
+                sq.y = __builtin_fmaf(rA[c].y, rA[c].y, sq.y);
+            }
+        }
+    } else {
+        static_assert(STRUCT && ENTCHK, "the fused solve's mode");
+#pragma unroll
+        for (int c = 0; c < NV; c++) {
+            const cf a = ok ? A[((size_t)sys * NV + r) * NV + c] : cmk(0.0f, 0.0f);
+            if (c >= lu_first_unfused_step()) rA[LuRowForm<FUSE>::pos(c)] = a;
+            sq.x = __builtin_fmaf(a.x, a.x, sq.x);
+            sq.y = __builtin_fmaf(a.y, a.y, sq.y);
+        }
+#pragma unroll
+        for (int lv = 0; lv < LU_SLOTS; lv++) {
+            const int mem = (int)((lu_rowtab_lds()[lv * LU_REC_ROWS + r] >> LU_REC_MEMBER_AT) & 31u);
+            rA[lv] = ok && mem != LU_REC_NO_MEMBER ? A[((size_t)sys * NV + r) * NV + mem] : cmk(0.0f, 0.0f);
         }
     }
     bool ent_bad = false;
@@ -81,13 +97,19 @@
     bool redo;
     cf x = lu_solve<false, LAT, STRUCT, ENTCHK, FUSE>(rA, rB, lane, pat, LB, scr, redo, __ballot(sys < n), ent_bad);
     if (__builtin_expect(redo, 0)) {
-#pragma unroll
-        for (int c = 0; c < NV; c++) rA[c] = ok ? A[((size_t)sys * NV + r) * NV + c] : cmk(0.0f, 0.0f);
-        x = lu_solve<true>(rA, rB, lane, pat, LB, scr, redo);
+        if constexpr (!FUSE) {
+#pragma unroll
+            for (int c = 0; c < NV; c++) rA[c] = ok ? A[((size_t)sys * NV + r) * NV + c] : cmk(0.0f, 0.0f);
+            x = lu_solve<true>(rA, rB, lane, pat, LB, scr, redo);
+        } else {
+            cf rD[NV];
+#pragma unroll
+            for (int c = 0; c < NV; c++) rD[c] = ok ? A[((size_t)sys * NV + r) * NV + c] : cmk(0.0f, 0.0f);
+            x = lu_solve<true>(rD, rB, lane, pat, LB, scr, redo);
+        }
     }
     if (ok) X[(size_t)sys * NV + r] = x;
 }
-
 
 __global__ void __launch_bounds__(WG_THREADS) k_eval(int n, const Workspace *ws, const cf *__restrict__ X,
                                                      const cf *__restrict__ P, const cf *__restrict__ D,
@@ -137,7 +159,7 @@
     }
 }
 
-template <bool ABSTAB>
+template <bool ABSTAB, bool CROW = false>
 __global__ void __launch_bounds__(WG_THREADS) k_eval_variant(int n, int redo_vals, const Workspace *ws,
                                                              const cf *__restrict__ X, const cf *__restrict__ TGT,
                                                              const cf *__restrict__ DIF, const cf *__restrict__ SP,
@@ -202,10 +224,11 @@
             if (!pred) rB = t;
         }
     }
-    cf rA[NV];
+    static_assert(ABSTAB || !CROW, "the compact row is gathered through the absolute tables");
+    cf rA[LuRowForm<CROW>::W];
     if constexpr (ABSTAB) {
-        uint4 gmv[ABS_GM_Q];
-        const bool ent_ok = eval_hx_terms_abs(AT->hx[wv], l0, l16, AT->gm[wv], gmv);
+        uint4 gmv[CROW ? ABS_GMC_Q : ABS_GM_Q];
+        const bool ent_ok = eval_hx_terms_abs(AT->hx[wv], l0, l16, CROW ? AT->gmc[wv] : AT->gm[wv], gmv);
         if (act) ENT_OK[pi * 32 + r] = ent_ok ? 1 : 0;
         wave_lds_sync();
         gather_hx_abs(rA, l0, gmv);
@@ -213,6 +236,13 @@
         eval_hx(rA, s_hx, s_hxd, &s_rowc[0][0], S, r_v);
     }
     wave_lds_sync();
+    if constexpr (CROW) {
+        if (act && rl) {
+#pragma unroll
+            for (int c = 0; c < LU_COMPACT_W; c++) HX[(pi * NV + r) * LU_COMPACT_W + c] = rA[c];
+            RHS[pi * NV + r] = rB;
+        }
+    } else {
     if (redo_vals) {
         for (int k = r; k < ENT_CAP - 1; k += 32) S.ent[k] = cmk(__builtin_nanf(""), __builtin_nanf(""));
         wave_lds_sync();
@@ -248,6 +278,7 @@
         for (int c = 0; c < NV; c++) HX[(pi * NV + r) * NV + c] = rA[c];
         RHS[pi * NV + r] = rB;
     }
-}
-
-}
+    }
+}
+
+}
diff --git a/trifocal_pose_estimation_using_improved_gpuhc_amd/csrc/hc_eval.hpp b/trifocal_pose_estimation_using_improved_gpuhc_amd/csrc/hc_eval.hpp
--- a/trifocal_pose_estimation_using_improved_gpuhc_amd/csrc/hc_eval.hpp
+++ b/trifocal_pose_estimation_using_improved_gpuhc_amd/csrc/hc_eval.hpp
@@ -3,6 +3,7 @@
 #include <stddef.h>
 
 #include "hc_slot.hpp"
+#include "hc_lu_struct.hpp"
 
 namespace hc {
 
@@ -315,12 +316,15 @@
 
 constexpr int ABS_WAVES = 4;
 constexpr int ABS_GM_Q = (NV + 3) / 4;
+constexpr int ABS_GMC_Q = LU_COMPACT_W / 4;
+static_assert(LU_COMPACT_W % 4 == 0, "whole words of four positions");
 static_assert(HT_HELP <= 3, "the light terms' x[w] share one word group");
 struct AbsTables {
     uint4 hx[ABS_WAVES][HX_SLOT_CAP][WAVE];
     uint4 ht[ABS_WAVES][HT_FULL + 1][WAVE];
     uint2 htq[ABS_WAVES][HT_FULL][WAVE];
     uint4 gm[ABS_WAVES][ABS_GM_Q][WAVE];
+    uint4 gmc[ABS_WAVES][ABS_GMC_Q][WAVE];
 };
 static_assert(2 * ABS_WAVES * sizeof(SlotLDS) < 65536, "absolute offsets stay in the DS offset range");
 constexpr int EV_TAHEAD = 6;
@@ -334,8 +338,9 @@
 __device__ __forceinline__ HxOps hx_ops_abs(const char *l0, const uint4 &w) {
     return HxOps{ldp(l0, w.x), ldp(l0, w.y), ldp(l0, w.z)};
 }
+template <int GQ>
 __device__ __forceinline__ bool eval_hx_terms_abs(const uint4 (*hxw)[WAVE], char *l0, uint32_t l16,
-                                                  const uint4 (*gmw)[WAVE], uint4 (&g)[ABS_GM_Q]) {
+                                                  const uint4 (*gmw)[WAVE], uint4 (&g)[GQ]) {
     uint4 w[HX_SLOT_CAP];
 #pragma unroll
     for (int k = 0; k < EV_TAHEAD; k++) w[k] = abs_ld(hxw[k], l16);
@@ -348,7 +353,7 @@
         if (k + EV_TAHEAD < HX_SLOT_CAP) w[k + EV_TAHEAD] = abs_ld(hxw[k + EV_TAHEAD], l16);
         if (k == HX_SLOT_CAP - EV_TAHEAD) {
 #pragma unroll
-            for (int q = 0; q < ABS_GM_Q; q++) g[q] = abs_ld(gmw[q], l16);
+            for (int q = 0; q < GQ; q++) g[q] = abs_ld(gmw[q], l16);
         }
         if (k + EV_AHEAD < HX_SLOT_CAP) o[(k + EV_AHEAD) % (EV_AHEAD + 1)] = hx_ops_abs(l0, w[k + EV_AHEAD]);
         const HxOps &q = o[k % (EV_AHEAD + 1)];
@@ -364,9 +369,11 @@
     return sq.x + sq.y < __builtin_inff();
 }
 
-__device__ __forceinline__ void gather_hx_abs(cf (&rA)[NV], const char *l0, const uint4 (&g)[ABS_GM_Q]) {
-#pragma unroll
-    for (int c = 0; c < NV; c++) {
+template <int W, int GQ>
+__device__ __forceinline__ void gather_hx_abs(cf (&rA)[W], const char *l0, const uint4 (&g)[GQ]) {
+    static_assert(W <= 4 * GQ, "a word for every position");
+#pragma unroll
+    for (int c = 0; c < W; c++) {
         const uint4 &gw = g[c / 4];
         const pf2 v = ldp(l0, c % 4 == 0 ? gw.x : c % 4 == 1 ? gw.y : c % 4 == 2 ? gw.z : gw.w);
         rA[c] = cmk(v.x, v.y);
diff --git a/trifocal_pose_estimation_using_improved_gpuhc_amd/csrc/hc_kernels.hip b/trifocal_pose_estimation_using_improved_gpuhc_amd/csrc/hc_kernels.hip
--- a/trifocal_pose_estimation_using_improved_gpuhc_amd/csrc/hc_kernels.hip
+++ b/trifocal_pose_estimation_using_improved_gpuhc_amd/csrc/hc_kernels.hip
@@ -9,6 +9,7 @@
 #include "../../include/p2c/hc_trifocal_p2c.h"
 #include "../../include/lu/hc_lu_testing.h"
 #include "../../include/lu/hc_lu_rowtable_testing.h"
+#include "../../include/lu/hc_lu_compact_testing.h"
 #include "../../include/eval/hc_eval_testing.h"
 #include "../../include/adaptive/hc_trifocal_adaptive.h"
 
@@ -439,11 +440,11 @@
     return hc::launch_status(HC_ERROR_LAUNCH);
 }
 
-hcStatus hc_trifocal_eval_variant_batched(int variant, unsigned flags, int n, const int32_t *unified_index,
-                                          const hcComplex *x, const hcComplex *target, const hcComplex *diff,
-                                          const hcComplex *start_params, const float *t, const uint8_t *kind,
-                                          hcComplex *Hx, hcComplex *rhs, uint8_t *ent_ok, void *workspace,
-                                          size_t workspace_bytes, hcStream stream) {
+static hcStatus eval_variant_run(int variant, bool compact_rows, unsigned flags, int n, const int32_t *unified_index,
+                                 const hcComplex *x, const hcComplex *target, const hcComplex *diff,
+                                 const hcComplex *start_params, const float *t, const uint8_t *kind, hcComplex *Hx,
+                                 hcComplex *rhs, uint8_t *ent_ok, void *workspace, size_t workspace_bytes,
+                                 hcStream stream) {
     if (variant < 0 || variant >= HC_EVAL_VARIANT_COUNT || (flags & ~HC_EVAL_REDO) != 0u) return HC_ERROR_INVALID_VALUE;
     const bool abs_tables = variant == HC_EVAL_VARIANT_ABS;
     if (n < 0 || (n > 0 && (!unified_index || !x || !target || !diff || !start_params || !t || !kind || !Hx || !rhs ||
@@ -460,7 +461,11 @@
     const int per = 2 * hc::WAVES_PER_WG;
     const dim3 grid((n + per - 1) / per), block(hc::WG_THREADS);
     const int redo = (flags & HC_EVAL_REDO) ? 1 : 0;
-    if (abs_tables)
+    if (compact_rows)
+        hipLaunchKernelGGL((hc::k_eval_variant<true, true>), grid, block, 0, s, n, redo, ws, (const hc::cf *)x,
+                           (const hc::cf *)target, (const hc::cf *)diff, (const hc::cf *)start_params, t, kind,
+                           (hc::cf *)Hx, (hc::cf *)rhs, ent_ok);
+    else if (abs_tables)
         hipLaunchKernelGGL(hc::k_eval_variant<true>, grid, block, 0, s, n, redo, ws, (const hc::cf *)x,
                            (const hc::cf *)target, (const hc::cf *)diff, (const hc::cf *)start_params, t, kind,
                            (hc::cf *)Hx, (hc::cf *)rhs, ent_ok);
@@ -479,6 +484,24 @@
     const unsigned status = ctl[offsetof(hc::Workspace, status) / sizeof(unsigned)];
     if (status == 0u) return HC_SUCCESS;
     return status == (unsigned)HC_ERROR_TABLE ? HC_ERROR_TABLE : HC_ERROR_DEVICE;
+}
+
+hcStatus hc_trifocal_eval_variant_batched(int variant, unsigned flags, int n, const int32_t *unified_index,
+                                          const hcComplex *x, const hcComplex *target, const hcComplex *diff,
+                                          const hcComplex *start_params, const float *t, const uint8_t *kind,
+                                          hcComplex *Hx, hcComplex *rhs, uint8_t *ent_ok, void *workspace,
+                                          size_t workspace_bytes, hcStream stream) {
+    return eval_variant_run(variant, false, flags, n, unified_index, x, target, diff, start_params, t, kind, Hx, rhs,
+                            ent_ok, workspace, workspace_bytes, stream);
+}
+
+hcStatus hc_trifocal_compact_rows_batched(int n, const int32_t *unified_index, const hcComplex *x,
+                                          const hcComplex *target, const hcComplex *diff,
+                                          const hcComplex *start_params, const float *t, const uint8_t *kind,
+                                          hcComplex *rows, hcComplex *rhs, uint8_t *ent_ok, void *workspace,
+                                          size_t workspace_bytes) {
+    return eval_variant_run(HC_EVAL_VARIANT_ABS, true, 0u, n, unified_index, x, target, diff, start_params, t, kind,
+                            rows, rhs, ent_ok, workspace, workspace_bytes, nullptr);
 }
 
 hcStatus hc_trifocal_p2c_eval_batched(int n, const int32_t *hx_index, const int32_t *ht_index, const hcComplex *x,
@@ -580,6 +603,11 @@
     if (step < 0 || step >= hc::NV - 1 || group < 0 || group >= hc::LuChunks::count(step)) return -1;
     return hc::lu_group_class(step, group);
 }
+static_assert(HC_LU_COMPACT_WIDTH == hc::LU_COMPACT_W, "the header's row width");
+int hc_lu_compact_column(int row, int position) {
+    if (row < 0 || row >= hc::NV || position < 0 || position >= hc::LU_COMPACT_W) return -2;
+    return hc::lu_compact_col(row, position);
+}
 int hc_lu_row_field(int level, int row, int field) {
     if (level < 0 || level >= hc::LU_REC_LEVELS || row < 0 || row >= hc::LU_REC_ROWS) return -2;
     hc::LuRowRec rec{0u, hc::LU_ROWTAB.w[level * hc::LU_REC_ROWS + row]};
@@ -627,7 +655,8 @@
 void hc_trifocal_set_retry_reuse(int on) { hc::g_retry_reuse.store(on ? 1 : 0, std::memory_order_relaxed); }
 
 const char *hc_trifocal_version(void) {
-    return "hc_trifocal gfx950 v10.12 (2 paths/wave, structurally sparse LDS-broadcast LU with lean pivot steps fused by level, the levels' per-row constants and row labels read from LDS tables, "
+    return "hc_trifocal gfx950 v10.13 (2 paths/wave, structurally sparse LDS-broadcast LU with lean pivot steps fused by level, the levels' per-row constants and row labels read from LDS tables, "
+           "the fused solve's row kept in 16 positions (its column of each level, then columns 18..29), "
            "one exec region per pivot step for the eligible rows with the column groups through scratch windows, "
            "column groups by structural class (never-fillable groups untested, always-live groups unconditional), "
            "pivot search narrowed to the candidate rows' DPP group "
diff --git a/trifocal_pose_estimation_using_improved_gpuhc_amd/csrc/hc_lu.hpp b/trifocal_pose_estimation_using_improved_gpuhc_amd/csrc/hc_lu.hpp
--- a/trifocal_pose_estimation_using_improved_gpuhc_amd/csrc/hc_lu.hpp
+++ b/trifocal_pose_estimation_using_improved_gpuhc_amd/csrc/hc_lu.hpp
@@ -110,22 +110,24 @@
     else return (gb >> J) & 1u;
 }
 
-template <int J, int N>
-__device__ __forceinline__ void grp_store(cf *w, const cf (&rA)[NV]) {
-    if constexpr (N == 1) w[J] = rA[J];
-    else st4(&w[J], rA[J], rA[J + 1]);
+template <int J, int N, int P = J, int W>
+__device__ __forceinline__ void grp_store(cf *w, const cf (&rA)[W]) {
+    static_assert(P >= 0 && P + N <= W, "the group lies inside the row");
+    if constexpr (N == 1) w[J] = rA[P];
+    else st4(&w[J], rA[P], rA[P + 1]);
 }
 template <int J, int N>
 __device__ __forceinline__ void grp_load(const cf *p, cf *u) {
     if constexpr (N == 1) u[0] = p[J];
     else ld4(&p[J], u[0], u[1]);
 }
-template <int J, int N>
-__device__ __forceinline__ void grp_update(cf (&rA)[NV], const pf2 &l, const cf *u) {
+template <int J, int N, int P = J, int W>
+__device__ __forceinline__ void grp_update(cf (&rA)[W], const pf2 &l, const cf *u) {
+    static_assert(P >= 0 && P + N <= W, "the group lies inside the row");
 #pragma unroll
     for (int q = 0; q < N; q++) {
-        const pf2 v = pcmsub(pf2{rA[J + q].x, rA[J + q].y}, l, pf2{u[q].x, u[q].y});
-        rA[J + q] = cmk(v.x, v.y);
+        const pf2 v = pcmsub(pf2{rA[P + q].x, rA[P + q].y}, l, pf2{u[q].x, u[q].y});
+        rA[P + q] = cmk(v.x, v.y);
     }
 }
 
@@ -218,29 +220,29 @@
     }
 }
 
-template <int I, int K, bool STRUCT>
-__device__ __forceinline__ void lu_group_elig(cf (&rA)[NV], const pf2 &l, uint32_t pmw, uint32_t gb, cf *wrow,
-                                              const LUBuf &L HC_LU_WORK_ARG) {
+template <int I, int K, bool STRUCT, bool COMPACT>
+__device__ __forceinline__ void lu_group_elig(cf (&rA)[LuRowForm<COMPACT>::W], const pf2 &l, uint32_t pmw, uint32_t gb,
+                                              cf *wrow, const LUBuf &L HC_LU_WORK_ARG) {
     using C = LuChunks;
     if constexpr (K < C::count(I)) {
-        constexpr int J = C::start(I, K), N = C::len(I, K);
+        constexpr int J = C::start(I, K), N = C::len(I, K), P = LuRowForm<COMPACT>::pos(J);
         constexpr int CLS = STRUCT ? lu_group_class(I, K) : GRP_TESTED;
         if (CLS != GRP_DEAD && (CLS == GRP_ALWAYS || __builtin_expect(group_live<I, K>(pmw, gb), 1))) {
-            grp_store<J, N>(wrow, rA);
+            grp_store<J, N, P>(wrow, rA);
             wave_lds_sync();
             HC_LU_WORK(N);
             HC_DIAG_LIVE_HIT(I, K);
             HC_LU_WORK_GROUP();
             cf u[N];
             grp_load<J, N>(L.row, u);
-            grp_update<J, N>(rA, l, u);
+            grp_update<J, N, P>(rA, l, u);
         }
         __builtin_amdgcn_sched_barrier(0);
-        lu_group_elig<I, K + 1, STRUCT>(rA, l, pmw, gb, wrow, L HC_LU_WORK_PASS);
-    }
-}
-template <int I, bool X1, bool STRUCT>
-__device__ __forceinline__ void lu_step_tested(cf (&rA)[NV], cf &rB, int &rowid, uint32_t &pat, PivF &my, LUBuf &L,
+        lu_group_elig<I, K + 1, STRUCT, COMPACT>(rA, l, pmw, gb, wrow, L HC_LU_WORK_PASS);
+    }
+}
+template <int I, bool X1, bool STRUCT, bool COMPACT>
+__device__ __forceinline__ void lu_step_tested(cf (&rA)[LuRowForm<COMPACT>::W], cf &rB, int &rowid, uint32_t &pat, PivF &my, LUBuf &L,
                                                cf *scr, bool is_piv, int pl0, int pl1, pf2 reg_s, pf2 oo_s,
                                                bool elig HC_LU_WORK_ARG) {
     const uint32_t pp0 = (uint32_t)__builtin_amdgcn_readlane((int)pat, pl0);
@@ -280,12 +282,13 @@
     HC_DIAG_LIVE_HIT(I, LIVE_SOLVES);
     if (elig) {
         HC_ISA_MARK_I("lu_mult", I);
-        const pf2 lq = pcmul(pf2{rA[I].x, rA[I].y}, pf2{reg.x, reg.y});
+        constexpr int PI = LuRowForm<COMPACT>::pos(I);
+        const pf2 lq = pcmul(pf2{rA[PI].x, rA[PI].y}, pf2{reg.x, reg.y});
         const pf2 lp = {is_piv ? 0.0f : lq.x, is_piv ? 0.0f : lq.y};
         const pf2 bp = pcmsub(pf2{rB.x, rB.y}, lp, pf2{sB0.x, sB0.y});
         rB = cmk(bp.x, bp.y);
         pat |= (uint32_t)__builtin_amdgcn_sbfe((int)pat, I, 1) & pmw;
-        lu_group_elig<I, 0, STRUCT>(rA, lp, pmw, gb, wrow, L HC_LU_WORK_PASS);
+        lu_group_elig<I, 0, STRUCT, COMPACT>(rA, lp, pmw, gb, wrow, L HC_LU_WORK_PASS);
     }
 }
 
@@ -343,18 +346,21 @@
 
 namespace hc {
 
-template <int I, bool DENSE, int LAT, bool STRUCT>
-__device__ __forceinline__ void lu_forward(cf (&rA)[NV], cf &rB, int &rowid, uint32_t &pat, int lane, int r, int hb,
+template <int I, bool DENSE, int LAT, bool STRUCT, bool COMPACT = false>
+__device__ __forceinline__ void lu_forward(cf (&rA)[LuRowForm<COMPACT>::W], cf &rB, int &rowid, uint32_t &pat, int lane, int r, int hb,
                                            bool row_lane, PivF &my, LUBuf &L, cf *scr, bool &redo,
                                            unsigned long long elig_m HC_LU_WORK_ARG) {
+    static_assert(!COMPACT || (!DENSE && LAT == 0 && STRUCT && I >= lu_first_unfused_step()),
+                  "the compact row is the fused solve's");
     if constexpr (I < NV) {
         HC_ISA_MARK_I("lu_search", I);
-        const float v = __builtin_fabsf(rA[I].x) + __builtin_fabsf(rA[I].y);
+        constexpr int PI = LuRowForm<COMPACT>::pos(I);
+        const float v = __builtin_fabsf(rA[PI].x) + __builtin_fabsf(rA[PI].y);
         pf2 reg_s, oo_s;
         if constexpr (!DENSE) {
-            reg_s = recip_fast(pf2{rA[I].x, rA[I].y}, v, oo_s);
+            reg_s = recip_fast(pf2{rA[PI].x, rA[PI].y}, v, oo_s);
         } else {
-            const divf f = cdiv_factors(rA[I]);
+            const divf f = cdiv_factors(rA[PI]);
             const cf rg = (v == 0.0f) ? cmk(1.0f, 0.0f) : cdiv_apply(cmk(1.0f, 0.0f), f);
             reg_s = pf2{rg.x, rg.y};
             oo_s = pf2{f.o1, f.o2};
@@ -433,14 +439,14 @@
         HC_ISA_MARK_I("lu_pattern", I);
         if constexpr (DENSE) lu_step_dense<I>(rA, rB, rowid, my, L, is_piv, reg_s, oo_s, elig HC_LU_WORK_PASS);
         else if constexpr (LAT > 0 && STRUCT) lu_step_batched<I, LAT>(rA, rB, rowid, my, L, scr, is_piv, reg_s, oo_s, elig);
-        else lu_step_tested<I, (LAT > 0), STRUCT>(rA, rB, rowid, pat, my, L, scr, is_piv, pl0, pl1, reg_s, oo_s,
-                                                  elig HC_LU_WORK_PASS);
-        lu_forward<I + 1, DENSE, LAT, STRUCT>(rA, rB, rowid, pat, lane, r, hb, row_lane, my, L, scr, redo,
+        else lu_step_tested<I, (LAT > 0), STRUCT, COMPACT>(rA, rB, rowid, pat, my, L, scr, is_piv, pl0, pl1, reg_s, oo_s,
+                                                           elig HC_LU_WORK_PASS);
+        lu_forward<I + 1, DENSE, LAT, STRUCT, COMPACT>(rA, rB, rowid, pat, lane, r, hb, row_lane, my, L, scr, redo,
                                               elig_m & ~piv_m HC_LU_WORK_PASS);
     }
 }
 template <int LV>
-__device__ __forceinline__ void lu_forward_fused(cf (&rA)[NV], cf &rB, int &rowid, uint32_t &pat, int lane, int r, int hb,
+__device__ __forceinline__ void lu_forward_fused(cf (&rA)[LU_COMPACT_W], cf &rB, int &rowid, uint32_t &pat, int lane, int r, int hb,
                                                  bool row_lane, PivF &my, LUBuf &L, cf *scr, bool &redo,
                                                  unsigned long long elig_m HC_LU_WORK_ARG) {
     if constexpr (LV < LU_LEVELS.nlevels) {
@@ -454,19 +460,22 @@
         }
         lu_forward_fused<LV + 1>(rA, rB, rowid, pat, lane, r, hb, row_lane, my, L, scr, redo, elig_m HC_LU_WORK_PASS);
     } else {
-        lu_forward<lu_first_unfused_step(), false, 0, true>(rA, rB, rowid, pat, lane, r, hb, row_lane, my, L, scr, redo,
+        lu_forward<lu_first_unfused_step(), false, 0, true, true>(rA, rB, rowid, pat, lane, r, hb, row_lane, my, L, scr, redo,
                                                            elig_m HC_LU_WORK_PASS);
     }
 }
 
-template <int I, int LAST = 0>
-__device__ __forceinline__ void lu_backward(const cf (&rA)[NV], cf &rB, int rowid, const PivF &my, pf2 &res) {
+template <int I, int LAST = 0, bool COMPACT = false>
+__device__ __forceinline__ void lu_backward(const cf (&rA)[LuRowForm<COMPACT>::W], cf &rB, int rowid, const PivF &my,
+                                            pf2 &res) {
+    static_assert(!COMPACT || LAST >= lu_first_unfused_step(), "the compact row's low positions run level by level");
     if constexpr (I >= LAST) {
         HC_ISA_MARK_I("lu_back", I);
+        constexpr int PI = LuRowForm<COMPACT>::pos(I);
         const unsigned long long own = __builtin_amdgcn_ballot_w64(rowid == I);
         const int o0 = __builtin_ctz((unsigned)own);
         const int o1 = 32 + __builtin_ctz((unsigned)(own >> 32));
-        const pf2 q = pcdiv_apply(pf2{rB.x, rB.y}, pf2{rA[I].x, rA[I].y}, my);
+        const pf2 q = pcdiv_apply(pf2{rB.x, rB.y}, pf2{rA[PI].x, rA[PI].y}, my);
         const float x0 = __int_as_float(__builtin_amdgcn_readlane(__float_as_int(q.x), o0));
         const float y0 = __int_as_float(__builtin_amdgcn_readlane(__float_as_int(q.y), o0));
         const float x1 = __int_as_float(__builtin_amdgcn_readlane(__float_as_int(q.x), o1));
@@ -479,10 +488,10 @@
                      "v_mov_b64 %1, %0\n\ts_mov_b64 exec, %2"
                      : "=&v"(xv), "+v"(res), "=&s"(tmp) : "s"(xs0), "s"(xs1), "i"(1u << I));
         if constexpr (I > 0) {
-            const pf2 w = pcmsub(pf2{rB.x, rB.y}, xv, pf2{rA[I].x, rA[I].y});
+            const pf2 w = pcmsub(pf2{rB.x, rB.y}, xv, pf2{rA[PI].x, rA[PI].y});
             rB = cmk(w.x, w.y);
         }
-        lu_backward<I - 1, LAST>(rA, rB, rowid, my, res);
+        lu_backward<I - 1, LAST, COMPACT>(rA, rB, rowid, my, res);
     }
 }
 
@@ -493,7 +502,7 @@
 }
 
 template <bool DENSE, int LAT = 0, bool STRUCT = false, bool ENTCHK = false, bool FUSE = false>
-__device__ __forceinline__ cf lu_solve(cf (&rA)[NV], cf rB, int lane, uint32_t pattern, LUBuf &L, cf *scratch,
+__device__ __forceinline__ cf lu_solve(cf (&rA)[LuRowForm<FUSE>::W], cf rB, int lane, uint32_t pattern, LUBuf &L, cf *scratch,
                                       bool &redo, unsigned long long count_mask = ~0ull, bool ent_bad = false) {
     static_assert(!FUSE || (!DENSE && LAT == 0 && STRUCT && ENTCHK), "the fused levels belong to the throughput tracker's solve");
     (void)count_mask;
@@ -554,7 +563,7 @@
     HC_ISA_MARK("lu_back_init");
     pf2 res = {0.0f, 0.0f};
     if constexpr (FUSE) {
-        lu_backward<NV - 1, lu_first_unfused_step()>(rA, rB, rowid, my, res);
+        lu_backward<NV - 1, lu_first_unfused_step(), true>(rA, rB, rowid, my, res);
         lu_backward_fused<LU_LEVELS.nlevels - 1>(rA, rB, rowid, my, L, r, res);
         const float nf = __builtin_fmaf(res.y, 0.0f, res.x * 0.0f);
         redo = __builtin_amdgcn_ballot_w64(nf != nf) != 0ull;
diff --git a/trifocal_pose_estimation_using_improved_gpuhc_amd/csrc/hc_lu_levels.hpp b/trifocal_pose_estimation_using_improved_gpuhc_amd/csrc/hc_lu_levels.hpp
--- a/trifocal_pose_estimation_using_improved_gpuhc_amd/csrc/hc_lu_levels.hpp
+++ b/trifocal_pose_estimation_using_improved_gpuhc_amd/csrc/hc_lu_levels.hpp
@@ -11,16 +11,6 @@
 __device__ __forceinline__ void lu_rowtab_fill(int tid) {
     if (tid < LU_REC_WORDS) lu_rowtab_lds()[tid] = LU_ROWTAB.w[tid];
 }
-template <int LV, int K>
-__device__ __forceinline__ void lvl_pick(const cf (&rA)[NV], pf2 &c, int kk) {
-    if constexpr (K < lu_level_count(LV)) {
-        constexpr int I = lu_level_member(LV, K);
-        const bool in = kk == K;
-        c.x = in ? rA[I].x : c.x;
-        c.y = in ? rA[I].y : c.y;
-        lvl_pick<LV, K + 1>(rA, c, kk);
-    }
-}
 
 template <int LV>
 __device__ __forceinline__ void lvl_relabel(int &rowid, int mem, bool is_piv, unsigned long long live_m, const LUBuf &L) {
@@ -33,29 +23,38 @@
     }
     rowid = is_piv ? mem : rowid;
 }
-template <int LV, int J>
-__device__ __forceinline__ void lvl_groups(cf (&rA)[NV], const pf2 &l, cf *wrow, const cf *cw) {
-    if constexpr (J < NV) {
-        if constexpr (((LU_LEVELS.cols[LV] >> J) & 3u) != 0u) {
-            grp_store<J, 2>(wrow, rA);
+constexpr int LVL_SLOT_J0 = 2;
+template <int LV, int P>
+__device__ __forceinline__ void lvl_groups(cf (&rA)[LU_COMPACT_W], const pf2 &l, cf *wrow, const cf *cw) {
+    if constexpr (P < LU_COMPACT_W) {
+        constexpr int C0 = lu_first_unfused_step() + P - LU_SLOTS;
+        constexpr bool RUN = P < LU_SLOTS ? ((lu_level_slots(LV) >> P) & 3u) != 0u : ((LU_LEVELS.cols[LV] >> C0) & 3u) != 0u;
+        if constexpr (RUN) {
+            constexpr int J = P < LU_SLOTS ? LVL_SLOT_J0 + P : C0;
+            grp_store<J, 2, P>(wrow, rA);
             wave_lds_sync();
             cf u[2];
             grp_load<J, 2>(cw, u);
-            grp_update<J, 2>(rA, l, u);
+            grp_update<J, 2, P>(rA, l, u);
             __builtin_amdgcn_sched_barrier(0);
         }
-        lvl_groups<LV, J + 2>(rA, l, wrow, cw);
+        lvl_groups<LV, P + 2>(rA, l, wrow, cw);
     }
 }
+constexpr int lvl_pairs(int lv) {
+    int n = 0;
+    for (int p = 0; p < LU_SLOTS; p += 2) n += ((lu_level_slots(lv) >> p) & 3u) != 0u;
+    for (int j = lu_first_unfused_step(); j < NV; j += 2) n += ((LU_LEVELS.cols[lv] >> j) & 3u) != 0u;
+    return n;
+}
 template <int LV>
-__device__ __forceinline__ bool lu_level(cf (&rA)[NV], cf &rB, int &rowid, uint32_t &pat, int r, int hb, PivF &my,
+__device__ __forceinline__ bool lu_level(cf (&rA)[LU_COMPACT_W], cf &rB, int &rowid, uint32_t &pat, int r, int hb, PivF &my,
                                          LUBuf &L, cf *scr, unsigned long long &elig_m HC_LU_WORK_ARG) {
     constexpr int CNT = lu_level_count(LV), I0 = lu_level_member(LV, 0);
     constexpr uint32_t ROWS = LU_LEVELS.rows[LV];
     HC_ISA_MARK_I("lu_search", I0);
-    pf2 c = {0.0f, 0.0f};
+    const pf2 c = {rA[LV].x, rA[LV].y};
     const uint32_t rec = lu_rowtab_lds()[LV * LU_REC_ROWS + r];
-    lvl_pick<LV, 0>(rA, c, (int)((rec >> LU_REC_CHAIN_AT) & 15u));
     const float v = __builtin_fabsf(c.x) + __builtin_fabsf(c.y);
     pf2 oo_s;
     const pf2 reg_s = recip_fast(c, v, oo_s);
@@ -96,8 +95,7 @@
     HC_ISA_MARK_I("lu_update", I0);
 #ifdef HC_DIAG_LUWORK
     {
-        int pairs = 0;
-        for (int j = 0; j < NV; j += 2) pairs += ((LU_LEVELS.cols[LV] >> j) & 3u) != 0u;
+        constexpr int pairs = lvl_pairs(LV);
         lu_work_acc.acc += 2ull * (unsigned long long)pairs *
                            (unsigned long long)__builtin_popcountll(lv_elig & lu_work_acc.mask & ~m);
         lu_work_acc.groups += (unsigned long long)pairs;
@@ -117,11 +115,11 @@
 }
 
 template <int LV>
-__device__ __forceinline__ void lu_back_level(const cf (&rA)[NV], cf &rB, int rowid, const PivF &my, LUBuf &L, int r) {
+__device__ __forceinline__ void lu_back_level(const cf (&rA)[LU_COMPACT_W], cf &rB, int rowid, const PivF &my, LUBuf &L,
+                                              int r) {
     HC_ISA_MARK_I("lu_back_level", LV);
-    pf2 c = {0.0f, 0.0f};
+    const pf2 c = {rA[LV].x, rA[LV].y};
     const uint32_t rec = lu_rowtab_lds()[LV * LU_REC_ROWS + r];
-    lvl_pick<LV, 0>(rA, c, (int)((rec >> LU_REC_CHAIN_AT) & 15u));
     const int mem = (int)((rec >> LU_REC_MEMBER_AT) & 31u);
     const pf2 q = pcdiv_apply(pf2{rB.x, rB.y}, c, my);
     if (rowid == mem) L.row[mem] = cmk(q.x, q.y);
@@ -135,7 +133,7 @@
     }
 }
 template <int LV>
-__device__ __forceinline__ void lu_backward_fused(const cf (&rA)[NV], cf &rB, int rowid, const PivF &my, LUBuf &L, int r,
+__device__ __forceinline__ void lu_backward_fused(const cf (&rA)[LU_COMPACT_W], cf &rB, int rowid, const PivF &my, LUBuf &L, int r,
                                                   pf2 &res) {
     if constexpr (LV >= 0) {
         lu_back_level<LV>(rA, rB, rowid, my, L, r);
diff --git a/trifocal_pose_estimation_using_improved_gpuhc_amd/csrc/hc_lu_struct.hpp b/trifocal_pose_estimation_using_improved_gpuhc_amd/csrc/hc_lu_struct.hpp
--- a/trifocal_pose_estimation_using_improved_gpuhc_amd/csrc/hc_lu_struct.hpp
+++ b/trifocal_pose_estimation_using_improved_gpuhc_amd/csrc/hc_lu_struct.hpp
@@ -254,4 +254,52 @@
 static_assert(LU_LEVELS.nlevels == LU_REC_LEVELS && lu_row_fields_fit(), "a field of the row records overflows");
 static_assert(LU_REC_WORDS * sizeof(uint32_t) <= 640, "a larger row table may cost the headline kernel its fifth workgroup per CU: measure");
 
-}
+constexpr int LU_SLOTS = LU_REC_LEVELS;
+constexpr int LU_COMPACT_W = LU_SLOTS + NV - lu_first_unfused_step();
+constexpr int lu_slot_col(int row, int lv) {
+    const int k = lu_row_chain(lv, row);
+    return k < 0 ? -1 : lu_level_member(lv, k);
+}
+constexpr int lu_compact_col(int row, int pos) {
+    return pos < LU_SLOTS ? lu_slot_col(row, pos) : lu_first_unfused_step() + pos - LU_SLOTS;
+}
+constexpr uint32_t lu_row_bound(int row) {
+    uint32_t cur[NV] = {};
+    for (int r = 0; r < NV; r++) cur[r] = LU_STRUCT_PAT[r];
+    for (int i = 0; i < NV; i++)
+        for (int r = 0; r < NV; r++)
+            if ((cur[r] >> i) & 1u) cur[r] |= LU_BOUND.s[i];
+    return cur[row];
+}
+constexpr bool lu_slots_hold_the_bound() {
+    for (int r = 0; r < NV; r++) {
+        const uint32_t low = lu_row_bound(r) & ((1u << lu_first_unfused_step()) - 1u);
+        int per_level[LU_SLOTS] = {};
+        for (int c = 0; c < lu_first_unfused_step(); c++) {
+            if (!((low >> c) & 1u)) continue;
+            const int lv = LU_LEVELS.level[c];
+            if (!lu_step_fusable(c) || lv >= LU_SLOTS || ++per_level[lv] > 1 || lu_slot_col(r, lv) != c) return false;
+        }
+        for (int lv = 0; lv < LU_SLOTS; lv++)
+            if (lu_slot_col(r, lv) >= 0 && !((low >> lu_slot_col(r, lv)) & 1u)) return false;
+    }
+    return true;
+}
+static_assert(lu_slots_hold_the_bound(), "a row's bound holds a low column outside its level's slot");
+static_assert(LU_SLOTS % 2 == 0 && lu_first_unfused_step() % 2 == 0 && LU_COMPACT_W == 16,
+              "the columns behind the slots keep their pairs; 4 slots and columns 18..29");
+constexpr uint32_t lu_level_slots(int lv) {
+    uint32_t m = 0u;
+    for (int c = 0; c < lu_first_unfused_step(); c++)
+        if ((LU_LEVELS.cols[lv] >> c) & 1u) m |= 1u << LU_LEVELS.level[c];
+    return m;
+}
+static_assert(lu_level_slots(0) == 0xEu && lu_level_slots(1) == 0xCu && lu_level_slots(2) == 0x8u && lu_level_slots(3) == 0u,
+              "a level changes the slots above its own only");
+template <bool COMPACT>
+struct LuRowForm {
+    static constexpr int W = COMPACT ? LU_COMPACT_W : NV;
+    static constexpr int pos(int c) { return COMPACT ? c - (lu_first_unfused_step() - LU_SLOTS) : c; }
+};
+
+}
diff --git a/trifocal_pose_estimation_using_improved_gpuhc_amd/csrc/hc_prep_body.inc b/trifocal_pose_estimation_using_improved_gpuhc_amd/csrc/hc_prep_body.inc
--- a/trifocal_pose_estimation_using_improved_gpuhc_amd/csrc/hc_prep_body.inc
+++ b/trifocal_pose_estimation_using_improved_gpuhc_amd/csrc/hc_prep_body.inc
@@ -432,6 +432,27 @@
             }
             A->gm[wv][q][l] = make_uint4(g[0], g[1], g[2], g[3]);
         }
+        for (int i = tid; i < ABS_WAVES * ABS_GMC_Q * WAVE; i += PREP_THREADS) {
+            const int l = i & 63, q = (i >> 6) % ABS_GMC_Q, wv = (i >> 6) / ABS_GMC_Q;
+            const uint32_t sb = slot_base(wv * 64 + l);
+            const int row = l & 31;
+            uint32_t g[4];
+            for (int e = 0; e < 4; e++) {
+                const int pos = 4 * q + e;
+                int c = lu_first_unfused_step() + pos - LU_SLOTS;
+                if (pos < LU_SLOTS) {
+                    const int mem = (int)((LU_ROWTAB.w[pos * LU_REC_ROWS + row] >> LU_REC_MEMBER_AT) & 31u);
+                    c = mem == LU_REC_NO_MEMBER ? -1 : mem;
+                }
+                uint32_t off = (uint32_t)SLOT_OFF_ENTZERO;
+                if (c >= 0 && row < NV) {
+                    const uint32_t w = T->gm[c >> 1][row];
+                    off = (c & 1) ? w >> 16 : w & 0xFFFFu;
+                }
+                g[e] = sb + off;
+            }
+            A->gmc[wv][q][l] = make_uint4(g[0], g[1], g[2], g[3]);
+        }
     }
     if (r == 0) {
         for (int q = 0; q < 4; q++) {
diff --git a/trifocal_pose_estimation_using_improved_gpuhc_amd/csrc/hc_track_body.inc b/trifocal_pose_estimation_using_improved_gpuhc_amd/csrc/hc_track_body.inc
--- a/trifocal_pose_estimation_using_improved_gpuhc_amd/csrc/hc_track_body.inc
+++ b/trifocal_pose_estimation_using_improved_gpuhc_amd/csrc/hc_track_body.inc
@@ -445,12 +445,12 @@
             }
         }
         HC_DIAG_MARK(3);
-        cf rA[NV];
+        cf rA[LuRowForm<LUFUSE>::W];
         HC_ISA_MARK("ev_hx");
         bool ent_ok = true;
         if constexpr (ABSTAB) {
-            uint4 gmv[ABS_GM_Q];
-            ent_ok = eval_hx_terms_abs(AT->hx[wv], l0, l16, AT->gm[wv], gmv);
+            uint4 gmv[LUFUSE ? ABS_GMC_Q : ABS_GM_Q];
+            ent_ok = eval_hx_terms_abs(AT->hx[wv], l0, l16, LUFUSE ? AT->gmc[wv] : AT->gm[wv], gmv);
             wave_lds_sync();
             HC_ISA_MARK("ev_gather");
             gather_hx_abs(rA, l0, gmv);
@@ -482,18 +482,19 @@
                                     : eval_rhs<RHS_H>(s_ht, S, r_r, false, rhs_masks(T));
                 if (!pred_r) rb = t;
             }
+            cf rD[NV];
             if constexpr (ABSTAB) {
                 uint4 gmv[ABS_GM_Q];
                 eval_hx_terms_abs(AT->hx[wv], l0, l16_r, AT->gm[wv], gmv);
                 wave_lds_sync();
-                gather_hx_abs(rA, l0, gmv);
+                gather_hx_abs(rD, l0, gmv);
             } else {
                 eval_hx_terms(s_hx, s_hxd, reinterpret_cast<char *>(&S), r_r);
                 wave_lds_sync();
-                gather_hx(rA, &s_rowc[0][0], S, r_r);
+                gather_hx(rD, &s_rowc[0][0], S, r_r);
             }
             wave_lds_sync();
-            k = lu_solve<true>(rA, rb, lane_v, row_pat, LB, S.ent, redo, HC_LU_COUNT(__ballot(act_r)));
+            k = lu_solve<true>(rD, rb, lane_v, row_pat, LB, S.ent, redo, HC_LU_COUNT(__ballot(act_r)));
         }
         wave_lds_sync();
 #ifdef HC_DIAG_PHASES
diff --git a/trifocal_pose_estimation_using_improved_gpuhc_amd/tracker.py b/trifocal_pose_estimation_using_improved_gpuhc_amd/tracker.py
--- a/trifocal_pose_estimation_using_improved_gpuhc_amd/tracker.py
+++ b/trifocal_pose_estimation_using_improved_gpuhc_amd/tracker.py
@@ -512,3 +512,30 @@
               _abi.ptr(torch.cuda.current_stream(dev)))
     torch.cuda.synchronize(dev)
     return HX.cpu().numpy(), RHS.cpu().numpy(), OK.cpu().numpy()
+
+
+def compact_rows_batched(unified: np.ndarray, x: np.ndarray, target: np.ndarray, diff: np.ndarray,
+                         start_params: np.ndarray, t: np.ndarray, kind: np.ndarray, device="cuda:0"):
+    dev = _require_gpu(device)
+    n = x.shape[0]
+    U = torch.from_numpy(np.ascontiguousarray(unified, np.int32)).to(dev)
+    X = torch.from_numpy(np.ascontiguousarray(x, np.float32)).to(dev)
+    TG = torch.from_numpy(np.ascontiguousarray(target, np.float32)).to(dev)
+    DF = torch.from_numpy(np.ascontiguousarray(diff, np.float32)).to(dev)
+    SP = torch.from_numpy(np.ascontiguousarray(start_params, np.float32)).to(dev)
+    T = torch.from_numpy(np.ascontiguousarray(t, np.float32)).to(dev)
+    K = torch.from_numpy(np.ascontiguousarray(kind, np.uint8)).to(dev)
+    if tuple(X.shape) != (n, 31, 2) or tuple(TG.shape) != (n, 34, 2) or tuple(DF.shape) != (n, 34, 2) or \
+            tuple(SP.shape) != (34, 2) or tuple(T.shape) != (n,) or tuple(K.shape) != (n,) or U.numel() != 38880:
+        raise _abi.HCError("compact_rows_batched: x (n, 31, 2), target and diff (n, 34, 2), start_params (34, 2), "
+                           "t and kind (n,), a unified index of 38880 values")
+    ROWS = torch.full((n, 30, _abi.LU_COMPACT_WIDTH, 2), float("nan"), dtype=torch.float32, device=dev)
+    RHS = torch.empty((n, 30, 2), dtype=torch.float32, device=dev)
+    OK = torch.full((n, 32), 255, dtype=torch.uint8, device=dev)
+    wsb = int(_abi.lib().hc_trifocal_workspace_size())
+    ws = torch.zeros(wsb, dtype=torch.uint8, device=dev)
+    torch.cuda.synchronize(dev)
+    _abi.call("hc_trifocal_compact_rows_batched", n, *(_abi.ptr(v) for v in (U, X, TG, DF, SP, T, K, ROWS, RHS, OK, ws)),
+              wsb)
+    torch.cuda.synchronize(dev)
+    return ROWS.cpu().numpy(), RHS.cpu().numpy()
```

New measurement: 1.792 million, median of 6. 9.0% higher.
